# Rose-STL-Lab/spherical-dyffusion

Hardware: AMD Instinct MI355X
Metric: forecast-steps/sec (180x360, 63ch), 25-member ensemble DYffusion sampling, whole job (higher is better)
Workload: dtype f32 tensors; every GEMM-class kernel (1x1 convs, fused MLP, Legendre analysis/synthesis, dhconv) as 3-pass split-f16 MFMA with f32 accumulation; FFT / norms / pointwise in f32 (statistics f64); 1 GPU; 25-member ensemble x horizon-6 DYffusion sampling pass (6 forecaster + 10 interpolator SFNO forwards, dropout stream on, AR feedback), 180x360, 63 state + 2 forcing channels, embed 256, 8 blocks; horizon=6, relayed_members=0, parallelism=members of one initial condition sharded over GPUs, no data-path collective

## Files before the change

### include/sdy_amd.h

```cpp
#ifndef SDY_AMD_H
#define SDY_AMD_H

#include <stddef.h>
#include <stdint.h>

#ifdef __cplusplus
extern "C" {
#endif
#pragma GCC visibility push(default)

#define SDY_OK 0
#define SDY_ERR_ARG (-1)
#define SDY_ERR_UNSUPPORTED (-2)
#define SDY_ERR_ALIGN (-3)
#define SDY_ERR_WORKSPACE (-4)
#define SDY_ERR_NAME (-5)
#define SDY_ERR_SHAPE (-6)
#define SDY_ERR_STATE (-7)

#define SDY_GRID_EQUIANGULAR 0
#define SDY_GRID_LEGENDRE_GAUSS 1

int sdy_version(void);
const char* sdy_error_string(int code);
// ... 13 lines not shown

int sdy_sht_forward(const sdy_sht_plan* plan, const float* x, float* out_c64, int B, int C, float* ws,
                    size_t ws_floats, void* stream);
int sdy_sht_inverse(const sdy_sht_plan* plan, const float* in_c64, float* y, int B, int C, float* ws,
                    size_t ws_floats, void* stream);

int sdy_rfft_lon(const sdy_sht_plan* plan, const float* x, const float* a, const float* d, float* xn_out,
                 float* Xf, int B, int C, void* stream);
int sdy_legendre_fwd(const sdy_sht_plan* plan, const float* Xf, float* Cs, int B, int C, void* stream);
int sdy_legendre_inv(const sdy_sht_plan* plan, const float* Cs, float* Yf, int B, int C, void* stream);
int sdy_irfft_lon(const sdy_sht_plan* plan, const float* Yf, const float* bias, float* y, int B, int C,
                  void* stream);

int sdy_dhconv_pack_weight(const float* w_host, int Ci, int Co, int L, float* w_packed_dev, void* stream);
int sdy_dhconv(const float* Cs_in, const float* w_packed, float* Cs_out, int L, int mtr, int B, int Ci, int Co,
               void* stream);
size_t sdy_dhconv_h3_pack_bytes(int Ci, int Co, int L);
int sdy_dhconv_h3_pack_weight(const float* w_host, int Ci, int Co, int L, void* packed_dev, float* scale);
int sdy_dhconv_h3(const float* Cs_in, const void* packed, float scale, float* Cs_out, int L, int mtr, int B, int Ci,
                  int Co, void* stream);

int sdy_dhconv_frag_supported(int Ci, int Co);
size_t sdy_dhconv_frag_pack_bytes(int L);
int sdy_dhconv_frag_pack(const float* w_host, int L, void* packed_dev, float* scale);
int sdy_dhconv_frag(const float* Cs_in, const void* packed, float scale, float* Cs_out, int L, int mtr, int B,
                    void* stream);

int sdy_instnorm_coeffs(const float* x, int B, int C, int HW, const float* gamma, const float* beta,
                        const float* scale_shift, long ss_stride, float eps, float* a, float* d, void* stream);

typedef struct sdy_conv_args {
  const float* x;  long x_bstride;
  const float* wt; int ldw;
  float* out;      long out_bstride;
  int B, Cin, Cout, HW;
  const float* pa; const float* pd;
  const float* bias;
  const float* add; long add_bstride;
  int add_mode;
  int act;
  float drop_p;
  const float* keep_mask;
  uint64_t seed; uint32_t call; uint32_t stream_id; uint32_t batch_offset;
  int rows_per_call;
  const float* batch_scale;
  int kernel_tag;
  const void* w_h3;
  float w_h3_scale;
  const void* w_frag;
  float w_frag_scale;
  double* stats;
  int out_tiled;
  const unsigned char* x_rows;
} sdy_conv_args;
int sdy_conv1x1(const sdy_conv_args* args, void* stream);

int sdy_conv256_h3_supported(int Cin, int Cout);
size_t sdy_conv256_h3_pack_bytes(void);
size_t sdy_conv256_h3_pack_bytes_cin(int Cin);
int sdy_conv256_h3_pack(const float* w_host, void* packed_dev, float* scale);
int sdy_conv256_h3_pack_cin(const float* w_host, int Cin, void* packed_dev, float* scale);
size_t sdy_h3_pack_bytes(int Cout, int Cin);
int sdy_h3_pack_weight(const float* w_host, int Cout, int Cin, void* packed_dev, float* scale);

typedef struct sdy_mlp_args {
  const float* x;  long x_bstride;
  const float* pa; const float* pd;
  const void* w; float w1_scale; float w2_scale;
  const float* b1; const float* b2;
  float* out;      long out_bstride;
  const float* add; long add_bstride;
  const float* add_a; const float* add_d;
  int B, E, hidden, HW;
  float drop_p;
  uint64_t seed; uint32_t call; uint32_t stream_fc1; uint32_t stream_fc2; uint32_t batch_offset;
  int rows_per_call;
  const float* batch_scale;
  double* stats;
  int x_tiled;
  const float* keep_hidden;
  const float* keep_out;
  const unsigned char* out_rows;
  int add_by_launch_row;
} sdy_mlp_args;
int sdy_instnorm_from_stats(double* stats, int B, int C, int HW, const float* gamma, const float* beta,
                            const float* scale_shift, long ss_bstride, float eps, float* a_out, float* d_out, void* stream);
int sdy_mlp_h3_supported(int E, int hidden);
size_t sdy_mlp_h3_pack_bytes(int E, int hidden);
int sdy_mlp_h3_pack(const float* w1_host, const float* w2_host, int E, int hidden, void* packed_dev, float* scale1,
                    float* scale2);
int sdy_mlp_h3(const sdy_mlp_args* args, void* stream);

typedef struct sdy_pair_args {
  const float* x;  long x_bstride;
  const void* w; float w1_scale; float w2_scale;
  const float* b1;
  float* out;      long out_bstride;
  const float* add; long add_bstride;
  int B, Cin, hidden, Cout, HW;
  double* stats;
} sdy_pair_args;
int sdy_pair_h3_supported(int Cin, int hidden, int Cout);
size_t sdy_pair_h3_pack_bytes(int Cin, int hidden, int Cout);
int sdy_pair_h3_pack(const float* w1_host, const float* w2_host, int Cin, int hidden, int Cout, void* packed_dev,
                     float* scale1, float* scale2);
int sdy_pair_h3(const sdy_pair_args* args, void* stream);

typedef struct sdy_sfno_config {
  int nlat, nlon;
  int in_chans;
  int out_chans;
  int embed_dim;
  int num_layers;
  int mlp_hidden;
  int lmax, mmax;
  int data_grid;
  int with_time_emb;
  int time_dim;
  float dropout_mlp;
  float drop_path_rate;
  int big_skip, pos_embed;
  int gemm_mode;
} sdy_sfno_config;

typedef struct sdy_sfno sdy_sfno;
int sdy_sfno_create(const sdy_sfno_config* cfg, sdy_sfno** out);
void sdy_sfno_destroy(sdy_sfno* net);
int sdy_sfno_set_param(sdy_sfno* net, const char* name, const float* host, size_t numel);
int sdy_sfno_ready(const sdy_sfno* net);
const char* sdy_sfno_missing(const sdy_sfno* net);
size_t sdy_sfno_workspace_floats(const sdy_sfno* net, int B);
int sdy_sfno_max_batch(const sdy_sfno* net);

typedef struct sdy_sfno_fwd_args {
  const float* in[3]; int in_chans[3];
  const float* time;
  float* out;
  int B;
  int enable_dropout;
  uint64_t seed; uint32_t call; uint32_t batch_offset;
  int rows_per_call;
  const float* const* keep_masks;
  const float* drop_path_keep;
  float* ws; size_t ws_floats;
  int reuse_encoder;
  int shared_inputs;
  const float* gen_src;
  int gen_chans;
  int gen_pos;
  const float* gen_coef;
  const float* gen_noise;
} sdy_sfno_fwd_args;
int sdy_sfno_forward(sdy_sfno* net, const sdy_sfno_fwd_args* args, void* stream);

int sdy_sfno_time_embed(sdy_sfno* net, const float* time, int B, float* t_repr, float* ss, void* stream);

int sdy_cold_update(const float* x_s, const float* x_ip_next, const float* x_ip_s, float* out, size_t n,
                    void* stream);
int sdy_concat_channels(const float* const* src, const int* chans, int nsrc, float* out, int B, int HW,
                        void* stream);

#define SDY_MAX_VARS 96
typedef struct sdy_var_table {
  int nvars;
  const float* data[SDY_MAX_VARS];
  float mean[SDY_MAX_VARS];
  float std[SDY_MAX_VARS];
} sdy_var_table;
int sdy_norm_pack(const sdy_var_table* vars, int t, int T1, int B, int HW, float* out, void* stream);

typedef struct sdy_step_finish_args {
  int B, HW, T1, t;
  const float* gen; int n_out;
  const float* prev_in; float* next_in; int n_in;
  int n_entries;
  int out_idx[SDY_MAX_VARS];
  int in_idx[SDY_MAX_VARS];
  float* gen_norm_tl[SDY_MAX_VARS];
  float* gen_tl[SDY_MAX_VARS];
  float mean[SDY_MAX_VARS], std[SDY_MAX_VARS];
  int presc_entry;
  const float* presc_target;
  const float* presc_mask;
  int mask_value, interpolate;
  const float* ar_init;
} sdy_step_finish_args;
int sdy_step_finish(const sdy_step_finish_args* args, void* stream);
int sdy_init_timeline(const sdy_var_table* vars, int T1, int B, int HW, float* const* tl_norm, float* const* tl_denorm,
                      void* stream);
int sdy_lp_rel_terms(const float* gen, const sdy_var_table* targets, int t, int T1, int B, int HW, double* terms,
                     void* stream);

int sdy_ensemble_metrics(const float* pred, const float* truth, const float* weights, int M, long member_stride,
                         int n_planes, int HW, double* out, void* stream);

int sdy_ensemble_series(const float* pred, int M, long member_stride, long sample_stride, const float* truth,
                        long truth_sample_stride, const float* weights, int n_sample, int T, int HW, double* out,
                        void* stream);

int sdy_ensemble_series_grad(const float* pred, int M, long member_stride, long sample_stride, const float* truth,
                             long truth_sample_stride, const float* weights, int n_sample, int T, int nlat, int nlon,
                             double* out, void* stream);

#define SDY_DERIVED_MAX_LEVELS 16
typedef struct {
  const float* q[SDY_DERIVED_MAX_LEVELS];
  const float* ps;
  const float* lhf;
  const float* prate;
  const float* adv;
  long s0, s1;
  int n0, n1, T, HW, K;
  float ak[SDY_DERIVED_MAX_LEVELS + 1], bk[SDY_DERIVED_MAX_LEVELS + 1];
  float* dry;
  float* twp;
  float* resid;
} sdy_derived_args;
int sdy_derived_water(const sdy_derived_args* args, void* stream);

#define SDY_CORRECTOR_DRY_AIR 1
#define SDY_CORRECTOR_ZERO_ADV 2
typedef struct sdy_corrector_var {
  const float* base;
  long stride;
  int channel;
  float mean, std;
} sdy_corrector_var;
typedef struct sdy_corrector_out {
  float* base;
  long stride;
  int channel;
} sdy_corrector_out;
typedef struct sdy_corrector_args {
  int B, HW, K;
  int flags;
  int budget;
// ... 130 lines not shown
```

### spherical-dyffusion_amd/_lib.py

```python
from __future__ import annotations

import ctypes as C
import os

_HERE = os.path.dirname(os.path.abspath(__file__))
LIB_PATH = os.environ.get("SDY_AMD_LIB") or os.path.join(_HERE, "libsdy_amd.so")

SDY_GRID = {"equiangular": 0, "legendre-gauss": 1}


class SdyError(RuntimeError):
    pass


class SdyConvArgs(C.Structure):
    _fields_ = [
        ("x", C.c_void_p), ("x_bstride", C.c_long),
        ("wt", C.c_void_p), ("ldw", C.c_int),
        ("out", C.c_void_p), ("out_bstride", C.c_long),
        ("B", C.c_int), ("Cin", C.c_int), ("Cout", C.c_int), ("HW", C.c_int),
        ("pa", C.c_void_p), ("pd", C.c_void_p),
        ("bias", C.c_void_p),
        ("add", C.c_void_p), ("add_bstride", C.c_long),
        ("add_mode", C.c_int),
        ("act", C.c_int),
        ("drop_p", C.c_float),
        ("keep_mask", C.c_void_p),
        ("seed", C.c_uint64), ("call", C.c_uint32), ("stream_id", C.c_uint32), ("batch_offset", C.c_uint32),
        ("rows_per_call", C.c_int),
        ("batch_scale", C.c_void_p),
        ("kernel_tag", C.c_int),
        ("w_h3", C.c_void_p),
        ("w_h3_scale", C.c_float),
        ("w_frag", C.c_void_p),
        ("w_frag_scale", C.c_float),
        ("stats", C.c_void_p),
        ("out_tiled", C.c_int),
        ("x_rows", C.c_void_p),
    ]


class SdyMlpArgs(C.Structure):
    _fields_ = [
        ("x", C.c_void_p), ("x_bstride", C.c_long),
        ("pa", C.c_void_p), ("pd", C.c_void_p),
        ("w", C.c_void_p), ("w1_scale", C.c_float), ("w2_scale", C.c_float),
        ("b1", C.c_void_p), ("b2", C.c_void_p),
        ("out", C.c_void_p), ("out_bstride", C.c_long),
        ("add", C.c_void_p), ("add_bstride", C.c_long),
        ("add_a", C.c_void_p), ("add_d", C.c_void_p),
        ("B", C.c_int), ("E", C.c_int), ("hidden", C.c_int), ("HW", C.c_int),
        ("drop_p", C.c_float),
        ("seed", C.c_uint64), ("call", C.c_uint32), ("stream_fc1", C.c_uint32), ("stream_fc2", C.c_uint32),
        ("batch_offset", C.c_uint32),
        ("rows_per_call", C.c_int),
        ("batch_scale", C.c_void_p),
        ("stats", C.c_void_p),
        ("x_tiled", C.c_int),
        ("keep_hidden", C.c_void_p), ("keep_out", C.c_void_p),
        ("out_rows", C.c_void_p),
        ("add_by_launch_row", C.c_int),
    ]


class SdyPairArgs(C.Structure):
    _fields_ = [
        ("x", C.c_void_p), ("x_bstride", C.c_long),
        ("w", C.c_void_p), ("w1_scale", C.c_float), ("w2_scale", C.c_float),
        ("b1", C.c_void_p),
        ("out", C.c_void_p), ("out_bstride", C.c_long),
        ("add", C.c_void_p), ("add_bstride", C.c_long),
        ("B", C.c_int), ("Cin", C.c_int), ("hidden", C.c_int), ("Cout", C.c_int), ("HW", C.c_int),
        ("stats", C.c_void_p),
    ]


SDY_MAX_VARS = 96


class SdyVarTable(C.Structure):
    _fields_ = [("nvars", C.c_int), ("data", C.c_void_p * SDY_MAX_VARS), ("mean", C.c_float * SDY_MAX_VARS),
                ("std", C.c_float * SDY_MAX_VARS)]


class SdyStepFinishArgs(C.Structure):
    _fields_ = [
        ("B", C.c_int), ("HW", C.c_int), ("T1", C.c_int), ("t", C.c_int),
        ("gen", C.c_void_p), ("n_out", C.c_int),
        ("prev_in", C.c_void_p), ("next_in", C.c_void_p), ("n_in", C.c_int),
        ("n_entries", C.c_int),
        ("out_idx", C.c_int * SDY_MAX_VARS), ("in_idx", C.c_int * SDY_MAX_VARS),
        ("gen_norm_tl", C.c_void_p * SDY_MAX_VARS), ("gen_tl", C.c_void_p * SDY_MAX_VARS),
        ("mean", C.c_float * SDY_MAX_VARS), ("std", C.c_float * SDY_MAX_VARS),
        ("presc_entry", C.c_int),
        ("presc_target", C.c_void_p), ("presc_mask", C.c_void_p),
        ("mask_value", C.c_int), ("interpolate", C.c_int),
        ("ar_init", C.c_void_p),
    ]


class SdySfnoConfig(C.Structure):
    _fields_ = [
        ("nlat", C.c_int), ("nlon", C.c_int),
        ("in_chans", C.c_int), ("out_chans", C.c_int),
        ("embed_dim", C.c_int), ("num_layers", C.c_int), ("mlp_hidden", C.c_int),
        ("lmax", C.c_int), ("mmax", C.c_int),
        ("data_grid", C.c_int),
        ("with_time_emb", C.c_int), ("time_dim", C.c_int),
        ("dropout_mlp", C.c_float), ("drop_path_rate", C.c_float),
        ("big_skip", C.c_int), ("pos_embed", C.c_int),
        ("gemm_mode", C.c_int),
    ]


class SdySfnoFwdArgs(C.Structure):
    _fields_ = [
        ("in_", C.c_void_p * 3), ("in_chans", C.c_int * 3),
        ("time", C.c_void_p),
        ("out", C.c_void_p),
        ("B", C.c_int),
        ("enable_dropout", C.c_int),
        ("seed", C.c_uint64), ("call", C.c_uint32), ("batch_offset", C.c_uint32),
        ("rows_per_call", C.c_int),
        ("keep_masks", C.POINTER(C.c_void_p)),
        ("drop_path_keep", C.c_void_p),
        ("ws", C.c_void_p), ("ws_floats", C.c_size_t),
        ("reuse_encoder", C.c_int),
        ("shared_inputs", C.c_int),
        ("gen_src", C.c_void_p), ("gen_chans", C.c_int), ("gen_pos", C.c_int),
        ("gen_coef", C.c_void_p), ("gen_noise", C.c_void_p),
    ]


SDY_DERIVED_MAX_LEVELS = 16


class SdyDerivedArgs(C.Structure):
    _fields_ = [
        ("q", C.c_void_p * SDY_DERIVED_MAX_LEVELS), ("ps", C.c_void_p),
        ("lhf", C.c_void_p), ("prate", C.c_void_p), ("adv", C.c_void_p),
        ("s0", C.c_long), ("s1", C.c_long),
        ("n0", C.c_int), ("n1", C.c_int), ("T", C.c_int), ("HW", C.c_int), ("K", C.c_int),
        ("ak", C.c_float * (SDY_DERIVED_MAX_LEVELS + 1)), ("bk", C.c_float * (SDY_DERIVED_MAX_LEVELS + 1)),
        ("dry", C.c_void_p), ("twp", C.c_void_p), ("resid", C.c_void_p),
    ]


SDY_CORRECTOR_DRY_AIR = 1
SDY_CORRECTOR_ZERO_ADV = 2
SDY_CORRECTOR_BUDGET = {None: 0, "precipitation": 1, "evaporation": 2, "advection_and_precipitation": 3,
                        "advection_and_evaporation": 4}


class SdyCorrectorVar(C.Structure):
    _fields_ = [("base", C.c_void_p), ("stride", C.c_long), ("channel", C.c_int), ("mean", C.c_float), ("std", C.c_float)]


class SdyCorrectorOut(C.Structure):
    _fields_ = [("base", C.c_void_p), ("stride", C.c_long), ("channel", C.c_int)]


class SdyCorrectorArgs(C.Structure):
    _fields_ = [
        ("B", C.c_int), ("HW", C.c_int), ("K", C.c_int), ("flags", C.c_int), ("budget", C.c_int),
        ("ak", C.c_float * (SDY_DERIVED_MAX_LEVELS + 1)), ("bk", C.c_float * (SDY_DERIVED_MAX_LEVELS + 1)),
        ("area", C.c_void_p),
        ("gen_q", SdyCorrectorVar * SDY_DERIVED_MAX_LEVELS), ("in_q", SdyCorrectorVar * SDY_DERIVED_MAX_LEVELS),
        ("gen_ps", SdyCorrectorVar), ("in_ps", SdyCorrectorVar), ("gen_lhf", SdyCorrectorVar),
        ("gen_prate", SdyCorrectorVar), ("gen_adv", SdyCorrectorVar),
        ("out_ps", SdyCorrectorOut), ("out_lhf", SdyCorrectorOut), ("out_prate", SdyCorrectorOut),
        ("out_adv", SdyCorrectorOut),
        ("ws", C.c_void_p), ("ws_bytes", C.c_size_t),
    ]


class SdyDryAirVar(C.Structure):
    _fields_ = [("base", C.c_void_p), ("stride_b", C.c_long), ("stride_t", C.c_long), ("channel", C.c_int),
                ("mean", C.c_float), ("std", C.c_float)]


class SdyDryAirArgs(C.Structure):
    _fields_ = [
        ("B", C.c_int), ("T", C.c_int), ("HW", C.c_int), ("K", C.c_int), ("accumulate", C.c_int),
        ("ak", C.c_float * (SDY_DERIVED_MAX_LEVELS + 1)), ("bk", C.c_float * (SDY_DERIVED_MAX_LEVELS + 1)),
        ("area", C.c_void_p),
        ("q", SdyDryAirVar * SDY_DERIVED_MAX_LEVELS), ("ps", SdyDryAirVar),
        ("gm", C.c_void_p), ("absdiff", C.c_void_p), ("mean_absdiff", C.c_void_p),
        ("ws", C.c_void_p), ("ws_bytes", C.c_size_t),
    ]


SDY_HIST_MAX_BINS = 2048
SDY_HIST_FLAG_RANGE = 1


class SdyHistArgs(C.Structure):
    _fields_ = [
        ("nvars", C.c_int), ("data", C.c_void_p * SDY_MAX_VARS),
        ("s0", C.c_long * SDY_MAX_VARS), ("s1", C.c_long * SDY_MAX_VARS),
        ("n0", C.c_int), ("n1", C.c_int), ("T", C.c_int), ("HW", C.c_int),
        ("t_start", C.c_int), ("n_times", C.c_int), ("n_bins", C.c_int),
        ("state", C.c_void_p), ("counts", C.c_void_p),
    ]


class SdyCoarsenArgs(C.Structure):
    _fields_ = [
        ("nvars", C.c_int), ("data", C.c_void_p * SDY_MAX_VARS),
        ("s0", C.c_long * SDY_MAX_VARS), ("s1", C.c_long * SDY_MAX_VARS),
        ("out", C.c_void_p * SDY_MAX_VARS),
        ("n0", C.c_int), ("n1", C.c_int), ("T", C.c_int), ("HW", C.c_int),
# ... 1 lines not shown
    ]


class SdyVideoArgs(C.Structure):
    _fields_ = [
        ("nvars", C.c_int), ("gen", C.c_void_p * SDY_MAX_VARS), ("target", C.c_void_p * SDY_MAX_VARS),
        ("gs0", C.c_long), ("gs1", C.c_long), ("ts1", C.c_long),
        ("n0", C.c_int), ("n1", C.c_int), ("T", C.c_int), ("HW", C.c_int),
        ("t_start", C.c_int), ("n_timesteps", C.c_int),
        ("gen_mean", C.c_void_p), ("target_mean", C.c_void_p), ("gen_sq", C.c_void_p), ("target_sq", C.c_void_p),
        ("err_var", C.c_void_p), ("err_min", C.c_void_p), ("err_max", C.c_void_p),
    ]


class SdyZonalArgs(C.Structure):
    _fields_ = [
        ("nvars", C.c_int), ("gen", C.c_void_p * SDY_MAX_VARS), ("target", C.c_void_p * SDY_MAX_VARS),
        ("gs0", C.c_long), ("gs1", C.c_long), ("ts1", C.c_long),
        ("n0", C.c_int), ("n1", C.c_int), ("T", C.c_int), ("H", C.c_int), ("W", C.c_int),
        ("t_start", C.c_int), ("n_timesteps", C.c_int),
        ("gen_acc", C.c_void_p), ("target_acc", C.c_void_p),
    ]


SIGNATURES = {
    "sdy_version": (C.c_int, []),
    "sdy_error_string": (C.c_char_p, [C.c_int]),
    "sdy_abi_check": (C.c_int, [C.POINTER(C.c_size_t), C.c_int]),
    "sdy_sht_tables_host": (C.c_int, [C.c_int, C.c_int, C.c_int, C.c_int, C.c_int, C.c_void_p, C.c_void_p, C.c_void_p]),
    "sdy_sht_plan_create": (C.c_int, [C.c_int, C.c_int, C.c_int, C.c_int, C.c_int, C.POINTER(C.c_void_p)]),
    "sdy_sht_plan_create_ex": (C.c_int, [C.c_int, C.c_int, C.c_int, C.c_int, C.c_int, C.c_int, C.POINTER(C.c_void_p)]),
    "sdy_sht_plan_destroy": (None, [C.c_void_p]),
    "sdy_sht_plan_dims": (C.c_int, [C.c_void_p, C.POINTER(C.c_int * 6)]),
    "sdy_sht_plan_kernels": (C.c_int, [C.c_void_p, C.POINTER(C.c_int * 2)]),
    "sdy_sht_workspace_floats": (C.c_size_t, [C.c_void_p, C.c_int, C.c_int]),
    "sdy_sht_forward": (C.c_int, [C.c_void_p, C.c_void_p, C.c_void_p, C.c_int, C.c_int, C.c_void_p, C.c_size_t, C.c_void_p]),
    "sdy_sht_inverse": (C.c_int, [C.c_void_p, C.c_void_p, C.c_void_p, C.c_int, C.c_int, C.c_void_p, C.c_size_t, C.c_void_p]),
    "sdy_rfft_lon": (C.c_int, [C.c_void_p, C.c_void_p, C.c_void_p, C.c_void_p, C.c_void_p, C.c_void_p, C.c_int, C.c_int, C.c_void_p]),
    "sdy_legendre_fwd": (C.c_int, [C.c_void_p, C.c_void_p, C.c_void_p, C.c_int, C.c_int, C.c_void_p]),
    "sdy_legendre_inv": (C.c_int, [C.c_void_p, C.c_void_p, C.c_void_p, C.c_int, C.c_int, C.c_void_p]),
    "sdy_irfft_lon": (C.c_int, [C.c_void_p, C.c_void_p, C.c_void_p, C.c_void_p, C.c_int, C.c_int, C.c_void_p]),
    "sdy_dhconv_pack_weight": (C.c_int, [C.c_void_p, C.c_int, C.c_int, C.c_int, C.c_void_p, C.c_void_p]),
    "sdy_dhconv": (C.c_int, [C.c_void_p, C.c_void_p, C.c_void_p, C.c_int, C.c_int, C.c_int, C.c_int, C.c_int, C.c_void_p]),
    "sdy_dhconv_h3_pack_bytes": (C.c_size_t, [C.c_int, C.c_int, C.c_int]),
    "sdy_dhconv_h3_pack_weight": (C.c_int, [C.c_void_p, C.c_int, C.c_int, C.c_int, C.c_void_p, C.POINTER(C.c_float)]),
    "sdy_dhconv_h3": (C.c_int, [C.c_void_p, C.c_void_p, C.c_float, C.c_void_p, C.c_int, C.c_int, C.c_int, C.c_int, C.c_int,
                                C.c_void_p]),
    "sdy_dhconv_frag_supported": (C.c_int, [C.c_int, C.c_int]),
    "sdy_dhconv_frag_pack_bytes": (C.c_size_t, [C.c_int]),
    "sdy_dhconv_frag_pack": (C.c_int, [C.c_void_p, C.c_int, C.c_void_p, C.POINTER(C.c_float)]),
    "sdy_dhconv_frag": (C.c_int, [C.c_void_p, C.c_void_p, C.c_float, C.c_void_p, C.c_int, C.c_int, C.c_int, C.c_void_p]),
    "sdy_instnorm_coeffs": (C.c_int, [C.c_void_p, C.c_int, C.c_int, C.c_int, C.c_void_p, C.c_void_p, C.c_void_p, C.c_long,
                                      C.c_float, C.c_void_p, C.c_void_p, C.c_void_p]),
    "sdy_conv1x1": (C.c_int, [C.POINTER(SdyConvArgs), C.c_void_p]),
    "sdy_ensemble_metrics": (C.c_int, [C.c_void_p, C.c_void_p, C.c_void_p, C.c_int, C.c_long, C.c_int, C.c_int, C.c_void_p,
                                       C.c_void_p]),
    "sdy_instnorm_from_stats": (C.c_int, [C.c_void_p, C.c_int, C.c_int, C.c_int, C.c_void_p, C.c_void_p, C.c_void_p,
                                          C.c_long, C.c_float, C.c_void_p, C.c_void_p, C.c_void_p]),
    "sdy_mlp_h3_supported": (C.c_int, [C.c_int, C.c_int]),
    "sdy_mlp_h3_pack_bytes": (C.c_size_t, [C.c_int, C.c_int]),
    "sdy_mlp_h3_pack": (C.c_int, [C.c_void_p, C.c_void_p, C.c_int, C.c_int, C.c_void_p, C.POINTER(C.c_float),
                                  C.POINTER(C.c_float)]),
    "sdy_mlp_h3": (C.c_int, [C.POINTER(SdyMlpArgs), C.c_void_p]),
    "sdy_pair_h3_supported": (C.c_int, [C.c_int, C.c_int, C.c_int]),
    "sdy_pair_h3_pack_bytes": (C.c_size_t, [C.c_int, C.c_int, C.c_int]),
    "sdy_pair_h3_pack": (C.c_int, [C.c_void_p, C.c_void_p, C.c_int, C.c_int, C.c_int, C.c_void_p, C.POINTER(C.c_float),
                                   C.POINTER(C.c_float)]),
    "sdy_pair_h3": (C.c_int, [C.POINTER(SdyPairArgs), C.c_void_p]),
    "sdy_conv256_h3_supported": (C.c_int, [C.c_int, C.c_int]),
    "sdy_conv256_h3_pack_bytes": (C.c_size_t, []),
    "sdy_conv256_h3_pack_bytes_cin": (C.c_size_t, [C.c_int]),
    "sdy_conv256_h3_pack": (C.c_int, [C.c_void_p, C.c_void_p, C.POINTER(C.c_float)]),
    "sdy_conv256_h3_pack_cin": (C.c_int, [C.c_void_p, C.c_int, C.c_void_p, C.POINTER(C.c_float)]),
    "sdy_h3_pack_bytes": (C.c_size_t, [C.c_int, C.c_int]),
    "sdy_h3_pack_weight": (C.c_int, [C.c_void_p, C.c_int, C.c_int, C.c_void_p, C.POINTER(C.c_float)]),
    "sdy_sfno_create": (C.c_int, [C.POINTER(SdySfnoConfig), C.POINTER(C.c_void_p)]),
    "sdy_sfno_destroy": (None, [C.c_void_p]),
    "sdy_sfno_set_param": (C.c_int, [C.c_void_p, C.c_char_p, C.c_void_p, C.c_size_t]),
    "sdy_sfno_ready": (C.c_int, [C.c_void_p]),
    "sdy_sfno_missing": (C.c_char_p, [C.c_void_p]),
    "sdy_sfno_workspace_floats": (C.c_size_t, [C.c_void_p, C.c_int]),
    "sdy_sfno_max_batch": (C.c_int, [C.c_void_p]),
    "sdy_sfno_forward": (C.c_int, [C.c_void_p, C.POINTER(SdySfnoFwdArgs), C.c_void_p]),
    "sdy_sfno_time_embed": (C.c_int, [C.c_void_p, C.c_void_p, C.c_int, C.c_void_p, C.c_void_p, C.c_void_p]),
    "sdy_norm_pack": (C.c_int, [C.POINTER(SdyVarTable), C.c_int, C.c_int, C.c_int, C.c_int, C.c_void_p, C.c_void_p]),
    "sdy_step_finish": (C.c_int, [C.POINTER(SdyStepFinishArgs), C.c_void_p]),
    "sdy_init_timeline": (C.c_int, [C.POINTER(SdyVarTable), C.c_int, C.c_int, C.c_int, C.POINTER(C.c_void_p),
                                    C.POINTER(C.c_void_p), C.c_void_p]),
    "sdy_lp_rel_terms": (C.c_int, [C.c_void_p, C.POINTER(SdyVarTable), C.c_int, C.c_int, C.c_int, C.c_int, C.c_void_p,
                                   C.c_void_p]),
    "sdy_cold_update": (C.c_int, [C.c_void_p, C.c_void_p, C.c_void_p, C.c_void_p, C.c_size_t, C.c_void_p]),
    "sdy_concat_channels": (C.c_int, [C.POINTER(C.c_void_p), C.POINTER(C.c_int), C.c_int, C.c_void_p, C.c_int, C.c_int,
                                      C.c_void_p]),
    "sdy_time_mean_accumulate": (C.c_int, [C.c_void_p, C.c_int, C.c_long, C.c_int, C.c_long, C.c_int, C.c_int, C.c_int,
                                          C.c_float, C.c_void_p, C.c_void_p]),
    "sdy_status_flags": (C.c_int, [C.POINTER(C.c_uint), C.c_int, C.c_void_p]),
    "sdy_status_flags_async": (C.c_int, [C.c_void_p, C.c_int, C.c_void_p]),
    "sdy_range_headroom_enable": (C.c_int, [C.c_int]),
    "sdy_range_headroom": (C.c_int, [C.POINTER(C.c_float), C.c_int, C.c_void_p]),
    "sdy_dropout_stream_rounds": (C.c_int, []),
    "sdy_dropout_stream_words": (C.c_int, [C.c_uint32, C.c_uint32, C.c_uint32, C.c_uint32, C.c_uint32, C.c_uint32,
                                           C.POINTER(C.c_uint32)]),
    "sdy_cond_noise_fill": (C.c_int, [C.c_uint64, C.c_uint32, C.c_uint32, C.c_int, C.c_int, C.c_int, C.c_int, C.c_void_p,
                                      C.c_void_p]),
    "sdy_ensemble_series": (C.c_int, [C.c_void_p, C.c_int, C.c_long, C.c_long, C.c_void_p, C.c_long, C.c_void_p, C.c_int,
                                     C.c_int, C.c_int, C.c_void_p, C.c_void_p]),
    "sdy_ensemble_series_grad": (C.c_int, [C.c_void_p, C.c_int, C.c_long, C.c_long, C.c_void_p, C.c_long, C.c_void_p,
                                          C.c_int, C.c_int, C.c_int, C.c_int, C.c_void_p, C.c_void_p]),
    "sdy_derived_water": (C.c_int, [C.POINTER(SdyDerivedArgs), C.c_void_p]),
    "sdy_corrector": (C.c_int, [C.POINTER(SdyCorrectorArgs), C.c_void_p]),
    "sdy_corrector_host": (C.c_int, [C.POINTER(SdyCorrectorArgs)]),
    "sdy_corrector_workspace_bytes": (C.c_size_t, [C.c_int, C.c_int]),
    "sdy_corrector_args_bytes": (C.c_size_t, []),
    "sdy_dry_air_series": (C.c_int, [C.POINTER(SdyDryAirArgs), C.c_void_p]),
    "sdy_dry_air_series_host": (C.c_int, [C.POINTER(SdyDryAirArgs)]),
    "sdy_dry_air_workspace_bytes": (C.c_size_t, [C.c_int, C.c_int, C.c_int]),
    "sdy_dry_air_args_bytes": (C.c_size_t, []),
    "sdy_hist_add": (C.c_int, [C.POINTER(SdyHistArgs), C.c_void_p]),
    "sdy_hist_args_bytes": (C.c_size_t, []),
    "sdy_hist_state_bytes": (C.c_size_t, [C.c_int]),
    "sdy_hist_state_unpack_host": (C.c_int, [C.c_void_p, C.c_int, C.POINTER(C.c_float), C.POINTER(C.c_float),
                                             C.POINTER(C.c_int), C.POINTER(C.c_uint), C.POINTER(C.c_ulonglong)]),
    "sdy_hist_plan_host": (C.c_int, [C.c_float, C.c_float, C.c_int, C.c_float, C.c_float, C.c_int, C.POINTER(C.c_float),
                                     C.POINTER(C.c_float), C.POINTER(C.c_int), C.POINTER(C.c_int), C.POINTER(C.c_uint)]),
    "sdy_hist_edges_host": (C.c_int, [C.c_float, C.c_float, C.c_int, C.c_void_p]),
    "sdy_hist_bins_host": (C.c_int, [C.c_void_p, C.c_long, C.c_float, C.c_float, C.c_int, C.c_void_p]),
    "sdy_time_coarsen": (C.c_int, [C.POINTER(SdyCoarsenArgs), C.c_void_p]),
    "sdy_time_coarsen_host": (C.c_int, [C.POINTER(SdyCoarsenArgs)]),
    "sdy_coarsen_args_bytes": (C.c_size_t, []),
    "sdy_video_accumulate": (C.c_int, [C.POINTER(SdyVideoArgs), C.c_void_p]),
    "sdy_video_accumulate_host": (C.c_int, [C.POINTER(SdyVideoArgs)]),
    "sdy_video_args_bytes": (C.c_size_t, []),
    "sdy_zonal_accumulate": (C.c_int, [C.POINTER(SdyZonalArgs), C.c_void_p]),
    "sdy_zonal_accumulate_host": (C.c_int, [C.POINTER(SdyZonalArgs)]),
    "sdy_zonal_args_bytes": (C.c_size_t, []),
    "sdy_profile_enable": (C.c_int, [C.c_int]),
    "sdy_profile_stage_count": (C.c_int, []),
    "sdy_profile_stage_name": (C.c_char_p, [C.c_int]),
    "sdy_profile_read": (C.c_int, [C.POINTER(C.c_double), C.POINTER(C.c_long), C.c_int]),
    "sdy_profile_read_rows": (C.c_int, [C.POINTER(C.c_double), C.POINTER(C.c_long), C.POINTER(C.c_long), C.c_int]),
    "sdy_relay_pool_create": (C.c_int, [C.c_size_t, C.c_int, C.POINTER(C.c_void_p), C.POINTER(C.c_ubyte)]),
    "sdy_relay_pool_destroy": (C.c_int, [C.c_void_p]),
    "sdy_ipc_open": (C.c_int, [C.POINTER(C.c_ubyte), C.POINTER(C.c_void_p)]),
    "sdy_ipc_close": (C.c_int, [C.c_void_p]),
    "sdy_copy_nocu": (C.c_int, [C.c_void_p, C.c_void_p, C.c_size_t, C.c_void_p]),
}


def _load():
    import torch

    if not os.path.exists(LIB_PATH):
        raise ImportError(
            f"{LIB_PATH} not found: the HIP library is required (no CPU/PyTorch fallback exists). "
            "Build it with `make -C spherical-dyffusion_amd/csrc` or `__graft_entry__.build()`."
        )
    lib = C.CDLL(LIB_PATH)
    for name, (res, args) in SIGNATURES.items():
        fn = getattr(lib, name)
        fn.restype = res
        fn.argtypes = args
    structs = (SdyConvArgs, SdyMlpArgs, SdyPairArgs, SdySfnoConfig, SdySfnoFwdArgs, SdyVarTable, SdyStepFinishArgs)
    sizes = (C.c_size_t * len(structs))(*[C.sizeof(t) for t in structs])
    if lib.sdy_abi_check(sizes, len(structs)) != 0:
        raise ImportError(f"{LIB_PATH}: argument structures of the bindings and of the library differ in size "
                          f"({[C.sizeof(t) for t in structs]}): rebuild the library (make -C spherical-dyffusion_amd/csrc)")
# ... 45 lines not shown
```

### spherical-dyffusion_amd/csrc/capi.hip

```cpp
#include <cmath>
#include <cstdio>
#include <cstdlib>
#include <cstring>
#include <mutex>
#include <string>
#include <vector>

#include "common.h"
#include "fft.h"
#include "pointwise.h"

static inline int round_up(int v, int m) { return (v + m - 1) / m * m; }
static inline size_t round_up_sz(size_t v, size_t m) { return (v + m - 1) / m * m; }

template <class F>
static float h3_pack_host(std::vector<_Float16>& buf, int nb, int rows, int K, int rows_pad, int Kpad, F value) {
  float mx = 0.f;
  for (int b = 0; b < nb; ++b)
    for (int r = 0; r < rows; ++r)
      for (int k = 0; k < K; ++k) mx = std::fmax(mx, std::fabs(value(b, r, k)));
  const float s = sdy_h3_scale(mx);
  const size_t plane = (size_t)nb * rows_pad * Kpad;
  buf.assign(2 * plane, (_Float16)0.0f);
  for (int b = 0; b < nb; ++b)
// ... 492 lines not shown
  return sdy_cond_noise_launch(seed, call, batch_offset, rows_per_call, B, C, HW, out, (hipStream_t)stream);
}

namespace {

struct DevBuf {
  float* p = nullptr;
  size_t n = 0;
  bool set = false;
  void* h3 = nullptr;
  float h3_scale = 1.0f;
  void* frag = nullptr;
  float frag_scale = 1.0f;
};

struct BlockW {
  DevBuf n0w, n0b, n1w, n1b;
  DevBuf tw, tb;
  DevBuf fw;
  DevBuf fb;
  DevBuf skw, skb;
  DevBuf w1, b1, w2, b2;
  std::vector<float> w1_host, w2_host;
  void* mlp = nullptr;
  float mlp_s1 = 1.0f, mlp_s2 = 1.0f;
  std::vector<float> fw_host, skw_host, fb_host, skb_host;
  DevBuf fbs;
};

}

static int spec_ilv(const sdy_sfno_config& c) { return (c.gemm_mode == 1 && c.embed_dim % 16 == 0) ? 1 : 0; }

static bool skip_foldable(const sdy_sfno_config& c, int i) {
  const bool first = i == 0, last = i == c.num_layers - 1;
  return c.gemm_mode == 1 && c.data_grid != SDY_GRID_LEGENDRE_GAUSS && first != last;
}

enum DhKind { DH_FOLDED, DH_FRAG, DH_GEMM_H3, DH_GEMM_F32 };
static DhKind dhconv_kind(const sdy_sfno_config& c, int i) {
  if (c.gemm_mode != 1) return DH_GEMM_F32;
  if (!sdy_dhconv_frag_supported(c.embed_dim, c.embed_dim) || sw().no_dh_frag) return DH_GEMM_H3;
  return skip_foldable(c, i) && !sw().no_skip_fold ? DH_FOLDED : DH_FRAG;
}

namespace {
struct XfSide {
  const sdy_sht_plan* plan;
  bool polar;
  bool tiled;
  int ilv;
  const int* mcut;
};

struct BlockPath {
  XfSide in, out;
  bool scale_residual;
  bool fused_mlp;
  bool lazy_norm;
  bool cs_tiled;
  DhKind dh;
  enum Skip { SKIP_CONV, SKIP_GELU, SKIP_IN_FFT } skip;
  bool stats1;
  bool z_tiled;
  bool drop_skip;
};
}

struct sdy_sfno {
  sdy_sfno_config cfg;
  int HW, catC, decC, ldo;
  sdy_sht_plan* plan_data = nullptr;
  sdy_sht_plan* plan_lg = nullptr;
  DevBuf pos, e0w, e0b, e2w, d0w, d0b, d2w;
  struct Pair { std::vector<float> w1_host, w2_host; void* w = nullptr; float s1 = 1.0f, s2 = 1.0f; } enc, dec;
  DevBuf t1w, t1b, t3w, t3b, freq, wbt, bb;
  std::vector<BlockW> blk;
  std::vector<BlockPath> path;
  SdyTimeMlp tm;
  std::string missing;
  const float* enc_ws = nullptr;
  int enc_B = 0;
  bool enc_has_stats = false;
};

static int dev_alloc(DevBuf& b, size_t n) {
  if (b.p && b.n == n) return SDY_OK;
  if (b.p) (void)hipFree(b.p);
  b.p = nullptr;
  SDY_HIP_TRY(hipMalloc((void**)&b.p, n * sizeof(float)));
  b.n = n;
  return SDY_OK;
}
static int dev_upload(DevBuf& b, const float* host, size_t n) {
  SDY_TRY(dev_alloc(b, n));
  SDY_HIP_TRY(hipMemcpy(b.p, host, n * sizeof(float), hipMemcpyHostToDevice));
  b.set = true;
  return SDY_OK;
}
static int dev_upload_T(DevBuf& b, const float* host, int out, int in, int ld) {
  std::vector<float> t((size_t)in * ld, 0.0f);
  for (int o = 0; o < out; ++o)
    for (int i = 0; i < in; ++i) t[(size_t)i * ld + o] = host[(size_t)o * in + i];
  return dev_upload(b, t.data(), t.size());
}
static void dev_free(DevBuf& b) {
  if (b.p) (void)hipFree(b.p);
  if (b.h3) (void)hipFree(b.h3);
  if (b.frag) (void)hipFree(b.frag);
  b.p = nullptr;
  b.h3 = nullptr;
  b.frag = nullptr;
  b.set = false;
}
static int dev_upload_conv(DevBuf& b, const float* host, int out, int in, int ld, bool want_h3) {
  SDY_TRY(dev_upload_T(b, host, out, in, ld));
  if (want_h3) {
    if (b.h3) (void)hipFree(b.h3);
    b.h3 = nullptr;
    SDY_HIP_TRY(hipMalloc(&b.h3, sdy_h3_pack_bytes(out, in)));
    SDY_TRY(sdy_h3_pack_weight(host, out, in, b.h3, &b.h3_scale));
    if (sdy_conv256_h3_supported(in, out)) {
      if (b.frag) (void)hipFree(b.frag);
      b.frag = nullptr;
      SDY_HIP_TRY(hipMalloc(&b.frag, sdy_conv256_h3_pack_bytes_cin(in)));
      SDY_TRY(sdy_conv256_h3_pack_cin(host, in, b.frag, &b.frag_scale));
    }
  }
  return SDY_OK;
}

extern "C" int sdy_sfno_create(const sdy_sfno_config* c, sdy_sfno** out) {
  if (!c || !out) return SDY_ERR_ARG;
  if (c->nlat < 2 || c->nlon < 4 || c->in_chans < 1 || c->out_chans < 1 || c->embed_dim < 4 || c->num_layers < 1 ||
      c->num_layers > 32 || c->mlp_hidden < 4)
    return SDY_ERR_ARG;
  if ((c->embed_dim & 3) || (c->mlp_hidden & 3) || ((c->nlat * c->nlon) & 3)) return SDY_ERR_ALIGN;
  if (c->with_time_emb && (c->time_dim < 4 || (c->embed_dim & 1))) return SDY_ERR_ARG;
  if (c->dropout_mlp < 0.f || c->dropout_mlp >= 1.f || c->drop_path_rate < 0.f || c->drop_path_rate >= 1.f)
    return SDY_ERR_ARG;
  sdy_sfno* n = new sdy_sfno();
  n->cfg = *c;
  n->HW = c->nlat * c->nlon;
  n->catC = c->embed_dim + c->in_chans;
  n->decC = c->embed_dim + (c->big_skip ? c->in_chans : 0);
  n->ldo = round_up(c->out_chans, 4);
  n->blk.resize(c->num_layers);
  if (c->gemm_mode != 0 && c->gemm_mode != 1) { delete n; return SDY_ERR_ARG; }
  int r = sdy_sht_plan_create_ex(c->nlat, c->nlon, c->lmax, c->mmax, c->data_grid, c->gemm_mode, &n->plan_data);
  if (r != SDY_OK) { delete n; return r; }
  if (c->data_grid == SDY_GRID_LEGENDRE_GAUSS) {
    n->plan_lg = n->plan_data;
  } else {
    r = sdy_sht_plan_create_ex(c->nlat, c->nlon, c->lmax, c->mmax, SDY_GRID_LEGENDRE_GAUSS, c->gemm_mode, &n->plan_lg);
    if (r != SDY_OK) { sdy_sfno_destroy(n); return r; }
  }
  std::memset(&n->tm, 0, sizeof(n->tm));
  n->tm.num_layers = c->num_layers;
  for (int i = 0; i < c->num_layers; ++i) {
    const float rate = c->num_layers > 1 ? c->drop_path_rate * (float)i / (float)(c->num_layers - 1) : 0.0f;
    n->tm.dp_rate[i] = rate;
    n->tm.dp_thr[i] = sdy_drop_threshold(rate);
  }
  if (c->with_time_emb) {
    const int E = c->embed_dim, T = c->time_dim, L = c->num_layers, half = E / 2;
    std::vector<float> f(half);
    const float e = (float)(-std::log(10000.0) / (half - 1));
    for (int i = 0; i < half; ++i) f[i] = expf((float)i * e);
    r = dev_upload(n->freq, f.data(), half);
    if (r == SDY_OK) r = dev_alloc(n->wbt, (size_t)L * T * 2 * E);
    if (r == SDY_OK) r = dev_alloc(n->bb, (size_t)L * 2 * E);
    if (r != SDY_OK) { sdy_sfno_destroy(n); return r; }
  }
  *out = n;
  return SDY_OK;
}

extern "C" void sdy_sfno_destroy(sdy_sfno* n) {
  if (!n) return;
  if (n->plan_lg && n->plan_lg != n->plan_data) sdy_sht_plan_destroy(n->plan_lg);
  if (n->plan_data) sdy_sht_plan_destroy(n->plan_data);
  DevBuf* top[] = {&n->pos, &n->e0w, &n->e0b, &n->e2w, &n->d0w, &n->d0b, &n->d2w, &n->t1w, &n->t1b,
                   &n->t3w, &n->t3b, &n->freq, &n->wbt, &n->bb};
  for (DevBuf* b : top) dev_free(*b);
  for (BlockW& w : n->blk) {
    DevBuf* bs[] = {&w.n0w, &w.n0b, &w.n1w, &w.n1b, &w.fw, &w.fb, &w.skw, &w.skb, &w.w1, &w.b1, &w.w2, &w.b2, &w.fbs};
    for (DevBuf* b : bs) dev_free(*b);
    if (w.mlp) (void)hipFree(w.mlp);
  }
  if (n->enc.w) (void)hipFree(n->enc.w);
  if (n->dec.w) (void)hipFree(n->dec.w);
  delete n;
}

#define EXPECT_NUMEL(n_expected)                      \
  do {                                                \
    if (numel != (size_t)(n_expected)) return SDY_ERR_SHAPE; \
  } while (0)

extern "C" int sdy_sfno_set_param(sdy_sfno* n, const char* name_c, const float* host, size_t numel) {
  if (!n || !name_c || !host) return SDY_ERR_ARG;
  const sdy_sfno_config& c = n->cfg;
  const int E = c.embed_dim, T = c.time_dim, L = c.num_layers, H = c.mlp_hidden, Cin = c.in_chans;
  const std::string name(name_c);
  const bool h3 = c.gemm_mode == 1;
  n->enc_ws = nullptr;
  n->path.clear();
  if (name.find("trans") != std::string::npos && (name.find(".weights") != std::string::npos ||
                                                   name.find(".pct") != std::string::npos))
    return SDY_OK;
  if (name == "@time_freq") { EXPECT_NUMEL(E / 2); return dev_upload(n->freq, host, numel); }
  if (name == "@drop_path_rates") {
    EXPECT_NUMEL(L);
    for (int i = 0; i < L; ++i) {
      if (host[i] < 0.f || host[i] >= 1.f) return SDY_ERR_ARG;
      n->tm.dp_rate[i] = host[i];
      n->tm.dp_thr[i] = sdy_drop_threshold(host[i]);
    }
    return SDY_OK;
  }
  if (name == "pos_embed") { EXPECT_NUMEL((size_t)E * n->HW); return dev_upload(n->pos, host, numel); }
  auto pack_pair = [&](sdy_sfno::Pair& pr, int cin, int cout) -> int {
    if (!h3 || !sdy_pair_h3_supported(cin, E, cout) || pr.w1_host.empty() || pr.w2_host.empty()) return SDY_OK;
    if (!pr.w) SDY_HIP_TRY(hipMalloc(&pr.w, sdy_pair_h3_pack_bytes(cin, E, cout)));
    return sdy_pair_h3_pack(pr.w1_host.data(), pr.w2_host.data(), cin, E, cout, pr.w, &pr.s1, &pr.s2);
  };
  if (name == "encoder.0.weight") {
    EXPECT_NUMEL((size_t)E * Cin);
    n->enc.w1_host.assign(host, host + numel);
    SDY_TRY(pack_pair(n->enc, Cin, E));
    return dev_upload_conv(n->e0w, host, E, Cin, E, h3);
  }
  if (name == "encoder.0.bias") { EXPECT_NUMEL(E); return dev_upload(n->e0b, host, numel); }
  if (name == "encoder.2.weight") {
    EXPECT_NUMEL((size_t)E * E);
    n->enc.w2_host.assign(host, host + numel);
    SDY_TRY(pack_pair(n->enc, Cin, E));
    return dev_upload_conv(n->e2w, host, E, E, E, h3);
  }
  if (name == "decoder.0.weight") {
    EXPECT_NUMEL((size_t)E * n->decC);
    n->dec.w1_host.assign(host, host + numel);
    SDY_TRY(pack_pair(n->dec, n->decC, c.out_chans));
    return dev_upload_conv(n->d0w, host, E, n->decC, E, h3);
  }
  if (name == "decoder.0.bias") { EXPECT_NUMEL(E); return dev_upload(n->d0b, host, numel); }
  if (name == "decoder.2.weight") {
    EXPECT_NUMEL((size_t)c.out_chans * E);
    n->dec.w2_host.assign(host, host + numel);
    SDY_TRY(pack_pair(n->dec, n->decC, c.out_chans));
    return dev_upload_conv(n->d2w, host, c.out_chans, E, n->ldo, h3);
  }
  if (c.with_time_emb) {
    if (name == "time_emb_mlp.1.weight") { EXPECT_NUMEL((size_t)T * E); return dev_upload_T(n->t1w, host, T, E, T); }
    if (name == "time_emb_mlp.1.bias") { EXPECT_NUMEL(T); return dev_upload(n->t1b, host, numel); }
    if (name == "time_emb_mlp.3.weight") { EXPECT_NUMEL((size_t)T * T); return dev_upload_T(n->t3w, host, T, T, T); }
    if (name == "time_emb_mlp.3.bias") { EXPECT_NUMEL(T); return dev_upload(n->t3b, host, numel); }
  }
  if (name.rfind("blocks.", 0) == 0) {
    const size_t dot = name.find('.', 7);
    if (dot == std::string::npos) return SDY_ERR_NAME;
    const int i = std::atoi(name.substr(7, dot - 7).c_str());
    if (i < 0 || i >= L) return SDY_ERR_NAME;
    const std::string rest = name.substr(dot + 1);
    BlockW& w = n->blk[i];
    if (rest == "norm0.weight") { EXPECT_NUMEL(E); return dev_upload(w.n0w, host, numel); }
    if (rest == "norm0.bias") { EXPECT_NUMEL(E); return dev_upload(w.n0b, host, numel); }
    if (rest == "norm1.weight") { EXPECT_NUMEL(E); return dev_upload(w.n1w, host, numel); }
    if (rest == "norm1.bias") { EXPECT_NUMEL(E); return dev_upload(w.n1b, host, numel); }
    if (c.with_time_emb && rest == "time_mlp.1.weight") {
      EXPECT_NUMEL((size_t)2 * E * T);
      std::vector<float> t((size_t)T * 2 * E);
      for (int o = 0; o < 2 * E; ++o)
        for (int k = 0; k < T; ++k) t[(size_t)k * 2 * E + o] = host[(size_t)o * T + k];
      SDY_HIP_TRY(hipMemcpy(n->wbt.p + (size_t)i * T * 2 * E, t.data(), t.size() * sizeof(float), hipMemcpyHostToDevice));
      w.tw.set = true;
      return SDY_OK;
    }
    if (c.with_time_emb && rest == "time_mlp.1.bias") {
      EXPECT_NUMEL((size_t)2 * E);
      SDY_HIP_TRY(hipMemcpy(n->bb.p + (size_t)i * 2 * E, host, numel * sizeof(float), hipMemcpyHostToDevice));
      w.tb.set = true;
      return SDY_OK;
    }
    auto pack_folded = [&]() -> int {
      if (w.fw_host.empty() || w.skw_host.empty()) return SDY_OK;
      std::vector<float> sum(w.fw_host);
      for (int ii = 0; ii < E; ++ii)
        for (int oo = 0; oo < E; ++oo) {
// ... 71 lines not shown
      return SDY_OK;
    }
    if (rest == "mlp.fwd.2.bias" || rest == "mlp.fwd.3.bias") { EXPECT_NUMEL(E); return dev_upload(w.b2, host, numel); }
  }
  return SDY_ERR_NAME;
}

static BlockPath resolve_path(const sdy_sfno* n, int i) {
  const sdy_sfno_config& c = n->cfg;
  const BlockW& w = n->blk[i];
  const int E = c.embed_dim, ilv = spec_ilv(c);
  auto side = [&](const sdy_sht_plan* p) {
    const bool polar = plan_polar_ok(p, E), tiled = plan_tiled_ok(p, E, ilv);
    return XfSide{p, polar, tiled, tiled ? 2 : ilv, polar ? p->d_mcut : nullptr};
  };
  BlockPath b;
  b.in = side(i == 0 ? n->plan_data : n->plan_lg);
  b.out = side(i == c.num_layers - 1 ? n->plan_data : n->plan_lg);
  b.scale_residual = b.in.plan != b.out.plan;
  b.fused_mlp = w.mlp && !sw().no_fused_mlp;
  b.lazy_norm = b.fused_mlp && !b.scale_residual;
  b.dh = dhconv_kind(c, i);
  const bool dh_frag = b.dh == DH_FOLDED || b.dh == DH_FRAG;
  b.cs_tiled = b.in.tiled && b.out.tiled && dh_frag && b.in.plan->lmax == b.out.plan->lmax && b.in.plan->mtr == b.out.plan->mtr;
  b.stats1 = c.gemm_mode == 1 && w.skw.frag && sdy_conv256_h3_supported(E, E);
  b.z_tiled = b.stats1 && b.fused_mlp;
  b.skip = b.dh != DH_FOLDED ? BlockPath::SKIP_CONV : (b.out.tiled && b.z_tiled) ? BlockPath::SKIP_IN_FFT : BlockPath::SKIP_GELU;
  b.drop_skip = b.fused_mlp && b.z_tiled && b.cs_tiled && !sw().no_drop_skip;
  return b;
}

extern "C" int sdy_sfno_ready(const sdy_sfno* n_c) {
  sdy_sfno* n = const_cast<sdy_sfno*>(n_c);
  if (!n) return SDY_ERR_ARG;
  if (!n->path.empty()) return SDY_OK;
  const sdy_sfno_config& c = n->cfg;
  n->missing.clear();
  auto need = [&](const DevBuf& b, const std::string& nm) {
    if (!b.set && n->missing.empty()) n->missing = nm;
  };
  if (c.pos_embed) need(n->pos, "pos_embed");
  need(n->e0w, "encoder.0.weight"); need(n->e0b, "encoder.0.bias"); need(n->e2w, "encoder.2.weight");
  need(n->d0w, "decoder.0.weight"); need(n->d0b, "decoder.0.bias"); need(n->d2w, "decoder.2.weight");
  if (c.with_time_emb) {
    need(n->t1w, "time_emb_mlp.1.weight"); need(n->t1b, "time_emb_mlp.1.bias");
    need(n->t3w, "time_emb_mlp.3.weight"); need(n->t3b, "time_emb_mlp.3.bias");
  }
  for (int i = 0; i < c.num_layers; ++i) {
    const BlockW& w = n->blk[i];
    const std::string p = "blocks." + std::to_string(i) + ".";
    need(w.n0w, p + "norm0.weight"); need(w.n0b, p + "norm0.bias");
    need(w.n1w, p + "norm1.weight"); need(w.n1b, p + "norm1.bias");
    if (c.with_time_emb) { need(w.tw, p + "time_mlp.1.weight"); need(w.tb, p + "time_mlp.1.bias"); }
    need(w.fw, p + "filter.filter.weight"); need(w.fb, p + "filter.filter.bias");
    need(w.skw, p + "inner_skip.weight"); need(w.skb, p + "inner_skip.bias");
    need(w.w1, p + "mlp.fwd.0.weight"); need(w.b1, p + "mlp.fwd.0.bias");
    need(w.w2, p + "mlp.fwd.{2|3}.weight"); need(w.b2, p + "mlp.fwd.{2|3}.bias");
  }
  if (!n->missing.empty()) return SDY_ERR_STATE;
  if (c.with_time_emb) {
    n->tm.E = c.embed_dim; n->tm.T = c.time_dim;
    n->tm.freq = n->freq.p; n->tm.w1t = n->t1w.p; n->tm.b1 = n->t1b.p; n->tm.w2t = n->t3w.p; n->tm.b2 = n->t3b.p;
    n->tm.wbt = n->wbt.p; n->tm.bb = n->bb.p;
  } else {
    n->tm.E = 0;
  }
  std::vector<BlockPath> path;
  for (int i = 0; i < c.num_layers; ++i) {
    const BlockW& w = n->blk[i];
    const BlockPath b = resolve_path(n, i);
    const void* packed = b.dh == DH_GEMM_F32 ? (const void*)w.fw.p : b.dh == DH_GEMM_H3 ? w.fw.h3 : w.fw.frag;
    if (!packed) return SDY_ERR_STATE;
    if (b.dh == DH_FOLDED && !(b.scale_residual && w.fbs.set)) return SDY_ERR_STATE;
    path.push_back(b);
  }
  n->path = std::move(path);
  return SDY_OK;
}

extern "C" const char* sdy_sfno_missing(const sdy_sfno* n) { return n ? n->missing.c_str() : ""; }

namespace {
struct WsLayout {
  size_t cat, xa, xb, xe, xn, y, zt, hid, xf, cs, cs2, ca, cd, ca1, cd1, st0, st1, ste, ss, dp, trep, sp, total;
};
WsLayout ws_layout(const sdy_sfno* n, int B) {
  const sdy_sfno_config& c = n->cfg;
  const size_t HW = n->HW, E = c.embed_dim;
  WsLayout w;
  size_t off = 0;
  auto take = [&](size_t floats) { size_t o = off; off += round_up_sz(floats, 64); return o; };
  w.cat = take((size_t)B * n->catC * HW);
  const size_t img = (size_t)B * E * HW;
  w.xa = take(img); w.xb = take(img);
  w.xe = take(img);
  w.xn = take(img); w.y = take(img);
  w.zt = take((size_t)B * ((HW + 63) / 64) * E * 64);
  w.hid = take((size_t)B * c.mlp_hidden * HW);
  w.xf = take(xf_floats(n->plan_data, B, (int)E));
  w.cs = take(cs_floats(n->plan_data, B, (int)E)); w.cs2 = take(cs_floats(n->plan_data, B, (int)E));
  w.ca = take((size_t)B * E); w.cd = take((size_t)B * E); w.ca1 = take((size_t)B * E); w.cd1 = take((size_t)B * E);
  w.st1 = take((size_t)B * E * 4);
  w.st0 = take((size_t)B * E * 4);
  w.ste = take((size_t)B * E * 4);
  w.ss = take((size_t)B * c.num_layers * 2 * E);
  w.dp = take((size_t)B * c.num_layers);
  w.trep = take((size_t)2 * B * (c.with_time_emb ? c.time_dim : 1));
  w.sp = take((size_t)B * E * c.nlat * 4);
  w.total = off;
  return w;
}
}

extern "C" size_t sdy_sfno_workspace_floats(const sdy_sfno* n, int B) {
  if (!n || B <= 0) return 0;
  return ws_layout(n, B).total;
}

extern "C" int sdy_sfno_max_batch(const sdy_sfno* n) {
  if (!n) return 0;
  const sdy_sfno_config& c = n->cfg;
  const int mtr = c.mmax < c.lmax ? c.mmax : c.lmax;
  bool all_tiled = sdy_sfno_ready(n) == SDY_OK;
  for (const BlockPath& p : n->path) all_tiled = all_tiled && p.cs_tiled;
  long b;
  if (all_tiled) {
    b = ((1L << 32) - 1) / ((long)mtr * 8 * c.lmax * 64);
  } else {
    const long per_row = 192L * mtr * 2 * c.embed_dim * 4 + 2L * c.embed_dim * 4;
    b = ((1L << 32) - 1) / per_row;
  }
  if (b > SDY_MAP_MAX) b = SDY_MAP_MAX;
  return b < 1 ? 1 : (int)b;
}

extern "C" int sdy_sfno_time_embed(sdy_sfno* n, const float* time, int B, float* t_repr, float* ss, void* stream) {
  if (!n || !time || B <= 0) return SDY_ERR_ARG;
  SDY_TRY(sdy_sfno_ready(n));
  if (!n->cfg.with_time_emb) return SDY_ERR_UNSUPPORTED;
  if (!ss) return SDY_ERR_ARG;
  float* scratch = nullptr;
  SDY_HIP_TRY(hipMallocAsync(reinterpret_cast<void**>(&scratch), (size_t)2 * B * n->cfg.time_dim * sizeof(float), (hipStream_t)stream));
  const int rc = sdy_time_mlp_launch(n->tm, time, B, t_repr, ss, nullptr, nullptr, 0, 0, 0, 0, 0, (hipStream_t)stream, scratch);
  SDY_HIP_TRY(hipFreeAsync(scratch, (hipStream_t)stream));
  return rc;
}

namespace {
enum SdyStage {
  ST_CONCAT, ST_TIME_MLP, ST_ENC0, ST_ENC2, ST_NORM_COEFFS, ST_FFT_FWD, ST_LEG_FWD, ST_LEG_INV, ST_FFT_INV, ST_DHCONV,
  ST_SKIP_CONV, ST_MLP_FUSED, ST_MLP_FUSED_DROP, ST_FC1, ST_FC2, ST_DEC0, ST_DEC2, ST_ENC_PAIR, ST_DEC_PAIR, ST_DROP_COPY,
  ST_SKIP_GELU, ST_COUNT
};
const char* const kStageNames[ST_COUNT] = {
  "concat", "time_mlp", "encoder.0 conv", "encoder.2 conv", "instnorm coefficients", "rfft (lon)", "legendre analysis",
  "legendre synthesis", "irfft (lon)", "dhconv", "inner-skip conv", "mlp fused", "mlp fused (dropout)", "mlp fc1", "mlp fc2",
  "decoder.0 conv", "decoder.2 conv", "encoder (fused pair)", "decoder (fused pair)", "drop-path copy",
  "inner skip folded (gelu)"};
struct SdyProfiler {
  bool on = false;
  struct Rec { int stage; int rows; hipEvent_t e0, e1; bool closed; };
  std::vector<Rec> recs;
  std::vector<hipEvent_t> pool;
  std::mutex mu;
  int get_event(hipEvent_t* e) {
    if (!pool.empty()) { *e = pool.back(); pool.pop_back(); return SDY_OK; }
    SDY_HIP_TRY(hipEventCreate(e));
    return SDY_OK;
  }
  int begin(int stage, int rows, hipStream_t s, int* idx) {
    std::lock_guard<std::mutex> g(mu);
    Rec r{stage, rows, nullptr, nullptr, false};
    SDY_TRY(get_event(&r.e0));
    int rc = get_event(&r.e1);
    if (rc == SDY_OK) {
      hipError_t e = hipEventRecord(r.e0, s);
      if (e != hipSuccess) rc = (int)e;
    }
    if (rc != SDY_OK) {
      pool.push_back(r.e0);
      if (r.e1) pool.push_back(r.e1);
      return rc;
    }
    recs.push_back(r);
    *idx = (int)recs.size() - 1;
    return SDY_OK;
  }
  int end(int idx, hipStream_t s) {
    std::lock_guard<std::mutex> g(mu);
    if (idx < 0 || idx >= (int)recs.size()) return SDY_ERR_STATE;
    SDY_HIP_TRY(hipEventRecord(recs[idx].e1, s));
    recs[idx].closed = true;
    return SDY_OK;
  }
} g_prof;
}

#define SDY_STAGE_N(stage, rows, call)                                          \
  do {                                                                          \
    int prof_idx_ = -1;                                                         \
    if (g_prof.on) SDY_TRY(g_prof.begin((stage), (rows), stream, &prof_idx_));  \
    SDY_TRY(call);                                                              \
    if (prof_idx_ >= 0) (void)g_prof.end(prof_idx_, stream);                    \
  } while (0)
#define SDY_STAGE(stage, call) SDY_STAGE_N(stage, B, call)

extern "C" int sdy_profile_enable(int on) {
  g_prof.on = on != 0;
  return SDY_OK;
}
extern "C" int sdy_profile_stage_count(void) { return ST_COUNT; }
extern "C" const char* sdy_profile_stage_name(int stage) {
  return (stage >= 0 && stage < ST_COUNT) ? kStageNames[stage] : "";
}
extern "C" int sdy_profile_read(double* total_ms, long* launches, int n) {
  return sdy_profile_read_rows(total_ms, launches, nullptr, n);
}
extern "C" int sdy_profile_read_rows(double* total_ms, long* launches, long* rows, int n) {
  if (!total_ms || !launches || n < ST_COUNT) return SDY_ERR_ARG;
  for (int i = 0; i < n; ++i) { total_ms[i] = 0.0; launches[i] = 0; if (rows) rows[i] = 0; }
  std::lock_guard<std::mutex> g(g_prof.mu);
  int rc = SDY_OK;
  for (auto& r : g_prof.recs) {
    if (r.closed) {
      float ms = 0.f;
      hipError_t e = hipEventSynchronize(r.e1);
      if (e == hipSuccess) e = hipEventElapsedTime(&ms, r.e0, r.e1);
      if (e != hipSuccess) rc = (int)e;
      else { total_ms[r.stage] += ms; launches[r.stage] += 1; if (rows) rows[r.stage] += r.rows; }
    }
    g_prof.pool.push_back(r.e0);
    g_prof.pool.push_back(r.e1);
  }
  g_prof.recs.clear();
  return rc;
}

namespace {
struct SfnoCall {
  sdy_sfno* n;
  const sdy_sfno_config& c;
  const sdy_sfno_fwd_args* a;
  hipStream_t stream;
  const int B, E = c.embed_dim, HW = n->HW, ilv = spec_ilv(c);
  const int rpc = a->rows_per_call > 0 ? a->rows_per_call : B;
  const bool drop = a->enable_dropout != 0, reuse = a->reuse_encoder != 0, shared = a->shared_inputs != 0, gen = a->gen_src;
  const bool enc_once = shared && n->enc.w && n->path[0].scale_residual && n->path[0].in.tiled;
  const int Be = enc_once ? rpc : B;
  const float pm = (drop && c.dropout_mlp > 0.f) ? c.dropout_mlp : 0.f;
  const WsLayout w = ws_layout(n, B);
  float* const ws = a->ws;
  const long xbs = (long)E * HW, cat_bs = (long)n->catC * HW;
  const long zt_bs = (long)((HW + 63) / 64) * E * 64;
  float *cat = ws + w.cat, *xa = ws + w.xa, *xb = ws + w.xb, *xe = ws + w.xe, *xn = ws + w.xn, *y = ws + w.y, *zt = ws + w.zt;
  float *hid = ws + w.hid, *Xf = ws + w.xf, *Cs = ws + w.cs, *Cs2 = ws + w.cs2, *ss = ws + w.ss, *dp = ws + w.dp;
  float *ca = ws + w.ca, *cd = ws + w.cd, *ca1 = ws + w.ca1, *cd1 = ws + w.cd1, *trep = ws + w.trep;
  float* cat_in = cat + (size_t)(n->catC - c.in_chans) * HW;
  double *st0 = reinterpret_cast<double*>(ws + w.st0), *st1 = reinterpret_cast<double*>(ws + w.st1);
  double *ste = reinterpret_cast<double*>(ws + w.ste), *sp = reinterpret_cast<double*>(ws + w.sp);
  const float* srcs[4];
  int chans[4], ns = 0;
  float *cur = xe, *nxt = xa;
  double* cur_stats = nullptr;

  struct Blk {
    int i;
    const BlockPath& P;
    const BlockW& w;
    float* dst; long dst_bs;
    float* z; long z_bs;
    double* st_out;
    unsigned char perm[SDY_MAP_MAX];
    int Bp, nD, Bf;
    const unsigned char* rows;
  };

  SfnoCall(sdy_sfno* n_, const sdy_sfno_fwd_args* a_, hipStream_t s) : n(n_), c(n_->cfg), a(a_), stream(s), B(a_->B) {}

  int check() {
    if (c.with_time_emb && !a->time) return SDY_ERR_ARG;
    if (a->ws_floats < w.total) return SDY_ERR_WORKSPACE;
    if (reuse && (n->enc_ws != ws || n->enc_B != B)) return SDY_ERR_STATE;
    int ctot = 0;
    for (int i = 0; i < 3; ++i)
      if (a->in[i] && a->in_chans[i] > 0) { srcs[ns] = a->in[i]; chans[ns] = a->in_chans[i]; ctot += a->in_chans[i]; ++ns; }
    if (gen) {
      if (a->gen_chans <= 0 || !a->gen_coef || a->gen_pos < 0 || a->gen_pos > ns) return SDY_ERR_ARG;
      if (reuse || shared) return SDY_ERR_ARG;
      for (int i = ns; i > a->gen_pos; --i) { srcs[i] = srcs[i - 1]; chans[i] = chans[i - 1]; }
      srcs[a->gen_pos] = a->gen_src; chans[a->gen_pos] = a->gen_chans; ctot += a->gen_chans; ++ns;
    }
    if (ns == 0 || ctot != c.in_chans) return SDY_ERR_SHAPE;
    if (a->rows_per_call < 0 || (a->rows_per_call > 0 && B % a->rows_per_call)) return SDY_ERR_ARG;
    if (shared && (reuse || rpc >= B)) return SDY_ERR_ARG;
    return SDY_OK;
  }

  int inputs() {
    if (!reuse) n->enc_ws = nullptr;
    SDY_HIP_TRY(hipMemsetAsync(st1, 0, (size_t)B * E * 2 * sizeof(double), stream));
    SDY_HIP_TRY(hipMemsetAsync(st0, 0, (size_t)B * E * 2 * sizeof(double), stream));
    if (gen) {
      SdyConcatGen g;
      g.gen = a->gen_pos; g.coef = a->gen_coef; g.noise = a->gen_noise;
      g.seed = a->seed; g.call = a->call; g.batch_offset = a->batch_offset; g.rows_per_call = rpc;
      SDY_STAGE(ST_CONCAT, sdy_concat_gen_launch(srcs, chans, ns, g, cat_in, cat_bs, B, HW, stream));
    } else if (!reuse) {
      SDY_STAGE(ST_CONCAT, sdy_concat_launch(srcs, chans, ns, cat_in, cat_bs, B, HW, stream, shared ? rpc : 0));
    }
    return SDY_OK;
  }

  int time_mlp() {
    SDY_STAGE(ST_TIME_MLP, sdy_time_mlp_launch(n->tm, a->time, B, trep, ss, dp, a->drop_path_keep, drop ? 1 : 0, a->seed, a->call,
                                               a->batch_offset, rpc, stream, trep + (size_t)B * (c.with_time_emb ? c.time_dim : 1)));
    return SDY_OK;
  }

  sdy_conv_args conv_args(const DevBuf& wb, int rows) const {
    sdy_conv_args cv;
    std::memset(&cv, 0, sizeof(cv));
    cv.B = rows; cv.HW = HW; cv.seed = a->seed; cv.call = a->call; cv.batch_offset = a->batch_offset; cv.rows_per_call = rpc;
    cv.wt = wb.p;
    if (c.gemm_mode == 1) { cv.w_h3 = wb.h3; cv.w_h3_scale = wb.h3_scale; cv.w_frag = wb.frag; cv.w_frag_scale = wb.frag_scale; }
    return cv;
  }

  int encoder() {
    bool have_ste = false;
    if (reuse) {
      have_ste = n->enc_has_stats;
    } else if (n->enc.w) {
      sdy_pair_args pa{};
      pa.x = cat_in; pa.x_bstride = cat_bs; pa.w = n->enc.w; pa.w1_scale = n->enc.s1; pa.w2_scale = n->enc.s2;
      pa.b1 = n->e0b.p; pa.out = xe; pa.out_bstride = xbs;
      if (c.pos_embed) { pa.add = n->pos.p; pa.add_bstride = 0; }
      pa.B = Be; pa.Cin = c.in_chans; pa.hidden = E; pa.Cout = E; pa.HW = HW;
      SDY_HIP_TRY(hipMemsetAsync(ste, 0, (size_t)Be * E * 2 * sizeof(double), stream));
      pa.stats = ste; have_ste = true;
      SDY_STAGE_N(ST_ENC_PAIR, Be, sdy_pair_h3(&pa, stream));
    } else {
      sdy_conv_args cv = conv_args(n->e0w, B);
      cv.x = cat_in; cv.x_bstride = cat_bs; cv.ldw = E; cv.out = xa; cv.out_bstride = xbs;
      cv.Cin = c.in_chans; cv.Cout = E; cv.bias = n->e0b.p; cv.act = 1;
      SDY_STAGE(ST_ENC0, sdy_conv1x1(&cv, stream));
      cv = conv_args(n->e2w, B);
      cv.x = xa; cv.x_bstride = xbs; cv.ldw = E; cv.out = xe; cv.out_bstride = xbs; cv.Cin = E; cv.Cout = E;
      if (c.pos_embed) { cv.add = n->pos.p; cv.add_bstride = 0; cv.add_mode = 2; }
      if (cv.w_frag && sdy_conv256_h3_supported(E, E)) {
        SDY_HIP_TRY(hipMemsetAsync(ste, 0, (size_t)B * E * 2 * sizeof(double), stream));
        cv.stats = ste; have_ste = true;
      }
      SDY_STAGE(ST_ENC2, sdy_conv1x1(&cv, stream));
    }
    n->enc_ws = enc_once ? nullptr : ws; n->enc_B = B; n->enc_has_stats = have_ste;
    if (have_ste) {
      for (int b0 = 0; b0 < B; b0 += Be)
        SDY_HIP_TRY(hipMemcpyAsync(st0 + (size_t)b0 * E * 2, ste, (size_t)Be * E * 2 * sizeof(double), hipMemcpyDeviceToDevice,
                                   stream));
      cur_stats = st0;
    }
    return SDY_OK;
  }

  int block(int i) {
    const bool last = i == c.num_layers - 1;
    Blk k{i, n->path[i], n->blk[i], last ? cat : nxt, last ? cat_bs : xbs};
    k.z = k.P.z_tiled ? zt : y;
    k.z_bs = k.P.z_tiled ? zt_bs : xbs;
    k.st_out = (k.P.fused_mlp && !last) ? st0 : nullptr;
    SDY_TRY(norm0(k));
    drop_rows(k);
    SDY_TRY(spectral(k));
    if (k.Bp > 0) {
      SDY_TRY(inner_skip(k));
      SDY_TRY(mlp(k));
    }
    if (k.nD > 0) SDY_TRY(drop_copy(k));
    cur_stats = k.st_out;
    cur = k.dst;
    nxt = (k.dst == xa) ? xb : xa;
    return SDY_OK;
  }

  int norm0(const Blk& k) {
    const float* ssk = c.with_time_emb ? ss + (size_t)k.i * 2 * E : nullptr;
    const long ss_bs = (long)c.num_layers * 2 * E;
    if (cur_stats)
      SDY_STAGE(ST_NORM_COEFFS, sdy_instnorm_from_stats(cur_stats, B, E, HW, k.w.n0w.p, k.w.n0b.p, ssk, ss_bs, 1e-6f, ca, cd, stream));
    else
      SDY_STAGE(ST_NORM_COEFFS, sdy_instnorm_coeffs_launch(cur, B, E, HW, k.w.n0w.p, k.w.n0b.p, ssk, ss_bs, 1e-6f, ca, cd, stream));
    return SDY_OK;
  }

  void drop_rows(Blk& k) const {
    k.Bp = B;
    k.nD = 0;
    if (drop && !a->drop_path_keep && B <= SDY_MAP_MAX && n->tm.dp_rate[k.i] > 0.f && k.P.drop_skip) {
      unsigned char drp[SDY_MAP_MAX];
      k.Bp = 0;
      for (int b = 0; b < B; ++b) {
        const int bq = b / rpc;
        const philox4 wd = philox4x32((uint32_t)(b - bq * rpc) + a->batch_offset, 0xFFFFFFFFu, 0x1000u + (uint32_t)k.i,
                                      a->call + (uint32_t)bq, (uint32_t)(a->seed & 0xFFFFFFFFu), (uint32_t)(a->seed >> 32));
        if (wd.x >= n->tm.dp_thr[k.i]) k.perm[k.Bp++] = (unsigned char)b;
        else drp[k.nD++] = (unsigned char)b;
      }
      for (int j = 0; j < k.nD; ++j) k.perm[k.Bp + j] = drp[j];
    }
    k.rows = k.nD > 0 ? k.perm : nullptr;
    k.Bf = k.P.scale_residual ? B : k.Bp;
  }

  int spectral(const Blk& k) {
    const BlockPath& P = k.P;
    const sdy_sht_plan *pin = P.in.plan, *pout = P.out.plan;
    if (k.Bf > 0) {
      float* xn_out = (P.scale_residual || P.lazy_norm) ? nullptr : xn;
      SDY_STAGE_N(ST_FFT_FWD, k.Bf, sdy_fft_launch_fwd(pin->fft, cur, ca, cd, xn_out, Xf, k.Bf, E, pin->nlat, pin->mtr, P.in.ilv,
                                                       P.in.mcut, stream, k.rows, (k.i == 0 && enc_once) ? Be : 0));
      SDY_STAGE_N(ST_LEG_FWD, k.Bf, legendre_fwd_impl(pin, Xf, Cs, k.Bf, E, P.in.polar, stream, P.in.tiled, P.cs_tiled));
      if (P.scale_residual) {
        SDY_STAGE(ST_LEG_INV, legendre_inv_impl(pout, Cs, Xf, B, E, P.out.polar, stream, P.out.tiled, P.cs_tiled));
        SDY_STAGE(ST_FFT_INV, sdy_fft_launch_inv(pout->fft, Xf, nullptr, xn, B, E, pout->nlat, pout->mtr, P.out.ilv, P.out.mcut,
                                                 stream));
      }
    }
    if (k.Bp == 0) return SDY_OK;
    if (P.dh == DH_FOLDED || P.dh == DH_FRAG)
      SDY_STAGE_N(ST_DHCONV, k.Bp, sdy_dh_h3_launch(Cs, k.w.fw.frag, k.w.fw.frag_scale, Cs2, c.lmax, pin->mtr, k.Bp, ilv, stream,
                                                    P.cs_tiled ? 1 : 0, k.Bf));
    else if (P.dh == DH_GEMM_H3)
      SDY_STAGE(ST_DHCONV, sdy_dhconv_h3(Cs, k.w.fw.h3, k.w.fw.h3_scale, Cs2, c.lmax, pin->mtr, B, E, E, stream));
    else
      SDY_STAGE(ST_DHCONV, sdy_dhconv(Cs, k.w.fw.p, Cs2, c.lmax, pin->mtr, B, E, E, stream));
    SDY_STAGE_N(ST_LEG_INV, k.Bp, legendre_inv_impl(pout, Cs2, Xf, k.Bp, E, P.out.polar, stream, P.out.tiled, P.cs_tiled));
    const float* bias = P.dh == DH_FOLDED ? k.w.fbs.p : k.w.fb.p;
    if (P.skip == BlockPath::SKIP_IN_FFT)
      SDY_STAGE_N(ST_FFT_INV, k.Bp, sdy_fft360_launch_inv(pout->fft, Xf, bias, nullptr, k.Bp, E, pout->nlat, pout->mtr, P.out.ilv,
                                                          P.out.mcut, stream, zt, zt_bs, sp));
    else
      SDY_STAGE_N(ST_FFT_INV, k.Bp, sdy_fft_launch_inv(pout->fft, Xf, bias, y, k.Bp, E, pout->nlat, pout->mtr, P.out.ilv,
                                                       P.out.mcut, stream));
    return SDY_OK;
  }

  int inner_skip(const Blk& k) {
    const BlockPath& P = k.P;
    const BlockW& bw = k.w;
    if (P.skip == BlockPath::SKIP_IN_FFT) {
      SDY_STAGE_N(ST_NORM_COEFFS, k.Bp, sdy_instnorm_from_partials_launch(sp, P.out.plan->nlat, k.Bp, E, HW, bw.n1w.p, bw.n1b.p,
                                                                          1e-6f, ca1, cd1, stream));
      return SDY_OK;
    }
    if (P.skip == BlockPath::SKIP_GELU) {
      SDY_STAGE_N(ST_SKIP_GELU, k.Bp, sdy_gelu_stats_launch(y, xbs, k.z, k.z_bs, P.z_tiled ? 1 : 0, st1, k.Bp, E, HW, stream));
    } else {
      sdy_conv_args cv = conv_args(bw.skw, k.Bp);
      cv.x_rows = P.lazy_norm ? k.rows : nullptr;
      cv.x = P.lazy_norm ? cur : xn; cv.x_bstride = xbs;
      if (P.lazy_norm) { cv.pa = ca; cv.pd = cd; }
      cv.ldw = E; cv.out = k.z; cv.out_bstride = k.z_bs; cv.out_tiled = P.z_tiled ? 1 : 0;
      cv.Cin = E; cv.Cout = E; cv.bias = bw.skb.p; cv.add = y; cv.add_bstride = xbs; cv.add_mode = 1; cv.act = 1; cv.kernel_tag = 3;
      if (P.stats1) cv.stats = st1;
      SDY_STAGE_N(ST_SKIP_CONV, k.Bp, sdy_conv1x1(&cv, stream));
    }
    if (P.skip == BlockPath::SKIP_GELU || P.stats1)
      SDY_STAGE_N(ST_NORM_COEFFS, k.Bp, sdy_instnorm_from_stats(st1, k.Bp, E, HW, bw.n1w.p, bw.n1b.p, nullptr, 0, 1e-6f, ca1, cd1,
                                                                stream));
    else
      SDY_STAGE(ST_NORM_COEFFS, sdy_instnorm_coeffs_launch(y, B, E, HW, bw.n1w.p, bw.n1b.p, nullptr, 0, 1e-6f, ca1, cd1, stream));
    return SDY_OK;
  }

  int mlp(const Blk& k) {
    const BlockW& bw = k.w;
    const int i = k.i, Hd = c.mlp_hidden;
    const float* dps = (drop && n->tm.dp_rate[i] > 0.f) ? dp + (size_t)i * B : nullptr;
    const float* keep1 = (pm > 0.f && a->keep_masks) ? a->keep_masks[2 * i] : nullptr;
    const float* keep2 = (pm > 0.f && a->keep_masks) ? a->keep_masks[2 * i + 1] : nullptr;
    if (k.P.fused_mlp) {
      sdy_mlp_args ma;
      std::memset(&ma, 0, sizeof(ma));
      ma.x = k.z; ma.x_bstride = k.z_bs; ma.x_tiled = k.P.z_tiled ? 1 : 0; ma.pa = ca1; ma.pd = cd1;
      ma.w = bw.mlp; ma.w1_scale = bw.mlp_s1; ma.w2_scale = bw.mlp_s2; ma.b1 = bw.b1.p; ma.b2 = bw.b2.p;
      ma.out = k.dst; ma.out_bstride = k.dst_bs;
      if (k.P.lazy_norm) { ma.add = cur; ma.add_bstride = xbs; ma.add_a = ca; ma.add_d = cd; }
      else { ma.add = xn; ma.add_bstride = xbs; ma.add_by_launch_row = k.rows ? 1 : 0; }
      ma.B = k.Bp; ma.out_rows = k.rows; ma.E = E; ma.hidden = Hd; ma.HW = HW;
      ma.drop_p = pm; ma.seed = a->seed; ma.call = a->call; ma.stream_fc1 = 2u * i; ma.stream_fc2 = 2u * i + 1u;
      ma.batch_offset = a->batch_offset; ma.rows_per_call = rpc;
      ma.batch_scale = dps; ma.keep_hidden = keep1; ma.keep_out = keep2; ma.stats = k.st_out;
      SDY_STAGE_N(pm > 0.f ? ST_MLP_FUSED_DROP : ST_MLP_FUSED, k.Bp, sdy_mlp_h3(&ma, stream));
      return SDY_OK;
    }
    sdy_conv_args cv = conv_args(bw.w1, B);
    cv.x = y; cv.x_bstride = xbs; cv.ldw = Hd; cv.out = hid; cv.out_bstride = (long)Hd * HW;
    cv.Cin = E; cv.Cout = Hd; cv.pa = ca1; cv.pd = cd1; cv.bias = bw.b1.p; cv.act = 1; cv.kernel_tag = 1;
    cv.drop_p = pm; cv.stream_id = 2u * i; cv.keep_mask = keep1;
    SDY_STAGE(ST_FC1, sdy_conv1x1(&cv, stream));
    cv = conv_args(bw.w2, B);
    cv.x = hid; cv.x_bstride = (long)Hd * HW; cv.ldw = E; cv.out = k.dst; cv.out_bstride = k.dst_bs;
    cv.Cin = Hd; cv.Cout = E; cv.bias = bw.b2.p; cv.kernel_tag = 2;
    cv.drop_p = pm; cv.stream_id = 2u * i + 1u; cv.keep_mask = keep2; cv.batch_scale = dps;
    cv.add = xn; cv.add_bstride = xbs; cv.add_mode = 2;
    SDY_STAGE(ST_FC2, sdy_conv1x1(&cv, stream));
    return SDY_OK;
  }

  int drop_copy(const Blk& k) {
    if (k.P.lazy_norm)
      SDY_STAGE_N(ST_DROP_COPY, k.nD, sdy_affine_copy_stats_launch(cur, xbs, ca, cd, k.dst, k.dst_bs, k.st_out, E, HW,
                                                                   k.perm + k.Bp, k.nD, stream));
    else
      SDY_STAGE_N(ST_DROP_COPY, k.nD, sdy_affine_copy_stats_launch(xn, xbs, nullptr, nullptr, k.dst, k.dst_bs, k.st_out, E, HW,
                                                                   k.perm + k.Bp, k.nD, stream, k.Bp));
    return SDY_OK;
  }

  int decoder() {
    if (n->dec.w) {
      sdy_pair_args pa{};
      pa.x = cat; pa.x_bstride = cat_bs; pa.w = n->dec.w; pa.w1_scale = n->dec.s1; pa.w2_scale = n->dec.s2;
      pa.b1 = n->d0b.p; pa.out = a->out; pa.out_bstride = (long)c.out_chans * HW;
      pa.B = B; pa.Cin = n->decC; pa.hidden = E; pa.Cout = c.out_chans; pa.HW = HW;
      SDY_STAGE(ST_DEC_PAIR, sdy_pair_h3(&pa, stream));
      return SDY_OK;
    }
    sdy_conv_args cv = conv_args(n->d0w, B);
    cv.x = cat; cv.x_bstride = cat_bs; cv.ldw = E;
    cv.out = xa; cv.out_bstride = xbs; cv.Cin = n->decC; cv.Cout = E; cv.bias = n->d0b.p; cv.act = 1;
    SDY_STAGE(ST_DEC0, sdy_conv1x1(&cv, stream));
    cv = conv_args(n->d2w, B);
    cv.x = xa; cv.x_bstride = xbs; cv.ldw = n->ldo; cv.out = a->out; cv.out_bstride = (long)c.out_chans * HW;
    cv.Cin = E; cv.Cout = c.out_chans;
    SDY_STAGE(ST_DEC2, sdy_conv1x1(&cv, stream));
    return SDY_OK;
  }
};
}

extern "C" int sdy_sfno_forward(sdy_sfno* n, const sdy_sfno_fwd_args* a, void* stream) {
  if (!n || !a || !a->out || !a->ws || a->B <= 0) return SDY_ERR_ARG;
  SDY_TRY(sdy_sfno_ready(n));
  SfnoCall f(n, a, (hipStream_t)stream);
  SDY_TRY(f.check());
  SDY_TRY(f.inputs());
  SDY_TRY(f.time_mlp());
  SDY_TRY(f.encoder());
  for (int i = 0; i < n->cfg.num_layers; ++i) SDY_TRY(f.block(i));
  return f.decoder();
}
```

### spherical-dyffusion_amd/csrc/mlp_h3.hip

```cpp
#include <cstdlib>
#include <vector>
#include <cmath>
#include <type_traits>

#include "common.h"

typedef const sdy_f16x8 __attribute__((address_space(1)))* wptr_t;
typedef _Float16 f16x4 __attribute__((ext_vector_type(4)));

namespace {

constexpr int ME = 256;
constexpr int MH = 512;
constexpr int TN = 64;
constexpr int HC = 128;
constexpr int NCH = MH / HC;
constexpr int KS1 = ME / 16;
constexpr int KSC = HC / 16;
constexpr int RING = 16;
constexpr int NGROUPS = NCH * 2 * RING;
static_assert(KS1 == RING && 2 * KSC == RING, "ring slot = index inside a block");
constexpr float SX = SDY_ACT_SX;

struct MlpParams {
  const float* x; long x_bs;
  int x_tiled;
  const float* pa; const float* pd;
  const sdy_f16x8* w;
  const float* b1; const float* b2;
  float* out; long out_bs;
  const float* add; long add_bs;
  const float* add_a; const float* add_d;
  int HW, B;
  float s1, s2;
  uint32_t drop_thr; float drop_scale;
  uint32_t seed_lo, seed_hi, stream1, stream2, call, batch_offset;
  int rows_per_call;
  const float* batch_scale;
  double* stats;
  const float* keep_h; const float* keep_o;
  unsigned* flags;
  unsigned* head;
  unsigned long long* stamps;
  SdyImgMap omap;
  int add_local;
};

__device__ __forceinline__ int px_swz(int px) { return (px & 15) ^ (((px >> 4) & 1) * 3); }
__device__ __forceinline__ int xs_off(int px, int c) { return px * ME + (((c & 16) | ((c ^ px_swz(px)) & 15)) << 3); }
__device__ __forceinline__ int hs_off(int px, int c) { return px * HC + (((c ^ px_swz(px)) & 15) << 3); }

template <bool DROP, bool INJECT = false>
__global__ __launch_bounds__(256, 1) void mlp_h3_kernel(const MlpParams p) {
  extern __shared__ __attribute__((aligned(16))) unsigned char smem[];
  _Float16* Xs_hi = reinterpret_cast<_Float16*>(smem);
  _Float16* Xs_lo = Xs_hi + TN * ME;
  _Float16* Hs = Xs_lo + TN * ME;
  float* Cf = reinterpret_cast<float*>(Hs + 4 * TN * HC);
  float* Cb2 = Cf + 4 * ME;

  const int tid = threadIdx.x, lane = tid & 63;
  const int wave = __builtin_amdgcn_readfirstlane(tid >> 6);
  int h = lane >> 5, l31 = lane & 31;
  const int tpi = (p.HW + TN - 1) / TN;
  const int ntiles = tpi * p.B;
  const int t_per = (ntiles + (int)gridDim.x - 1) / (int)gridDim.x;
  const int t_begin = (int)blockIdx.x * t_per;
  const int t_end = (t_begin + t_per < ntiles) ? t_begin + t_per : ntiles;
  int z = 0, zo = 0, n0 = 0;
  bool full = true;

  sdy_f16x8 r_hi[RING], r_lo[RING];
  auto wbase_of = [&](int ln) { return (wptr_t)(p.w + (size_t)wave * (NGROUPS + RING) * SDY_GROUP + ln); };
  wptr_t wp = wbase_of(lane);
#pragma unroll
  for (int s = 0; s < RING; ++s) {
    r_hi[s] = wp[s * SDY_GROUP];
    r_lo[s] = wp[s * SDY_GROUP + 64];
  }
  wp += RING * SDY_GROUP;

  int q0 = tid & 15, o0 = tid >> 4;
  f32x4 xr[2][8];
  const float* pf_base = nullptr;
  const float* res_base = nullptr;
  unsigned pf_off = 0u;
  int pf_rs = 0;
  auto prefetch_setup = [&](int t) {
    const int zz = t / tpi, nn = (t - zz * tpi) * TN;
    const bool ok = nn + 4 * q0 < p.HW;
    pf_base = p.x + (long)zz * p.x_bs + (p.x_tiled ? (long)(t - zz * tpi) * (ME * TN) : 0L);
    pf_rs = p.x_tiled ? TN : p.HW;
    pf_off = p.x_tiled ? (unsigned)(8 * o0 * TN + 4 * q0) * 4u : (unsigned)(8 * o0 * p.HW + (ok ? nn + 4 * q0 : 0)) * 4u;
  };
  auto prefetch_piece = [&](int piece) {
    const int oc = piece >> 3, e = piece & 7;
    xr[oc][e] = sdy_ld16s(pf_base + (long)(8 * 16 * oc + e) * pf_rs, pf_off);
  };
  auto prefetch_x = [&](int t) {
    const int zz = t / tpi, nn = (t - zz * tpi) * TN;
    const bool ok = nn + 4 * q0 < p.HW;
    const float* xz = p.x + (long)zz * p.x_bs + (p.x_tiled ? (long)(t - zz * tpi) * (ME * TN) : 0L);
    const int rs = p.x_tiled ? TN : p.HW;
    const unsigned xo = p.x_tiled ? (unsigned)(8 * o0 * TN + 4 * q0) * 4u : (unsigned)(8 * o0 * p.HW + (ok ? nn + 4 * q0 : 0)) * 4u;
#pragma unroll
    for (int oc = 0; oc < 2; ++oc)
#pragma unroll
      for (int e = 0; e < 8; ++e) xr[oc][e] = sdy_ld16s(xz + (long)(8 * 16 * oc + e) * rs, xo);
  };
  auto load_coeffs = [&](int zz) {
    const int t = 64 * wave + (int)__builtin_amdgcn_mbcnt_hi(~0u, __builtin_amdgcn_mbcnt_lo(~0u, 0u));
    const long c = (long)zz * ME + t, co = (long)sdy_img(p.omap, zz) * ME + t;
    Cf[t] = p.pa ? p.pa[c] * SX : SX;
    Cf[ME + t] = p.pa ? p.pd[c] * SX : 0.0f;
    Cf[2 * ME + t] = p.add_a ? p.add_a[co] : 1.0f;
    Cf[3 * ME + t] = p.add_a ? p.add_d[co] : 0.0f;
  };
  Cb2[tid] = DROP ? p.b2[tid] * p.drop_scale : p.b2[tid];
  if (t_begin < t_end) load_coeffs(t_begin / tpi);
  __syncthreads();
  if (t_begin < t_end) prefetch_x(t_begin);
  double psum[16], psq[16];
#pragma unroll
  for (int i = 0; i < 16; ++i) { psum[i] = 0.0; psq[i] = 0.0; }

  for (int tile = t_begin; tile < t_end; ++tile) {
  asm volatile("" : "+v"(l31), "+v"(h), "+v"(q0), "+v"(o0));
  const int tile_it = tile - t_begin;
// ... 366 lines not shown
    };
    auto ldb1 = [&](int set, int t, int part) {
      const int j = part & 1;
      const int off = hs_off(32 * j + l31, 2 * t + h);
      if (part < 2) bh[set][j] = *reinterpret_cast<const sdy_f16x8*>(Hh + off);
      else bl[set][j] = *reinterpret_cast<const sdy_f16x8*>(Hl + off);
    };
    ldb(0, 0);
#pragma unroll
    for (int t = 0; t < KSC; ++t) {
      const int c = t & 1;
      if (!SDY_MLP_PINNED && t + 1 < KSC) ldb(c ^ 1, t + 1);
      __builtin_amdgcn_sched_barrier(0);
      Piece ps;
#pragma unroll
      for (int mi = 0; mi < 2; ++mi) {
        const int s = 2 * t + mi;
#pragma unroll
        for (int k = 0; k < 6; ++k) {
          const int j = k & 1;
          const sdy_f16x8 a = (k < 2) ? r_lo[s] : r_hi[s];
          const sdy_f16x8 b = (k >= 2 && k < 4) ? bl[c][j] : bh[c][j];
          if (SDY_H3_PASSES == 3 || k >= 4) oacc[mi][j] = __builtin_amdgcn_mfma_f32_32x32x16_f16(a, b, oacc[mi][j], 0, 0, 0);
          if (SDY_MLP_PINNED && mi == 0 && k < 4 && t + 1 < KSC) ldb1(c ^ 1, t + 1, k);
          if (SDY_MLP_PINNED && !CHAIN) __builtin_amdgcn_sched_barrier(0);
          if constexpr (CHAIN) {
            if (SDY_MLP_SCALAR_CHAIN) chain_slot(ps, 6 * mi + k, hc2 + 1, t & 1, t >> 1);
            else chain_stage(ps, 6 * mi + k, hc2 + 1, t & 1, t >> 1);
            __builtin_amdgcn_sched_barrier(0);
          }
        }
        r_hi[s] = wp[s * SDY_GROUP];
        r_lo[s] = wp[s * SDY_GROUP + 64];
        __builtin_amdgcn_sched_barrier(0);
      }
    }
    wp += RING * SDY_GROUP;
  };
  using T_ = std::integral_constant<bool, true>;
  using F_ = std::integral_constant<bool, false>;

  stamp(1);
  load_bias(0);
  fc1(0);
  stamp(2);
#pragma unroll
  for (int pc = 0; pc < 8; ++pc) chain_piece(0, pc & 1, pc >> 1);
  stamp(3);
  __syncthreads();
  stamp(4);
  load_bias(1);
  fc1(1);
  stamp(5);
#pragma unroll
  for (int mi = 0; mi < 2; ++mi)
#pragma unroll
    for (int j = 0; j < 2; ++j)
#pragma unroll
      for (int r = 0; r < 16; ++r) oacc[mi][j][r] = 0.0f;
#pragma unroll 1
  for (int hc = 1; hc < NCH; ++hc) {
    fc2(hc - 1, T_{});
    stamp(4 + 2 * hc);
    __syncthreads();
    if (hc < NCH - 1) {
      load_bias(hc + 1);
      fc1(hc + 1);
    }
    stamp(5 + 2 * hc);
  }
  {
    int ln = lane;
    asm volatile("" : "+v"(ln));
    wp = wbase_of(ln);
  }
  asm volatile("" : "+v"(wp));
  {
    const int nt = tile + 1;
    prefetch_setup(nt < t_end ? nt : tile);
  }
  fc2(NCH - 1, F_{});
  stamp(12);
  {
    res_base = p.add ? p.add + (long)(p.add_local ? z : zo) * p.add_bs : p.x + (long)z * p.x_bs;
  }

  {
    const float bscale = p.batch_scale ? p.batch_scale[zo] : 1.0f;
    const float s2e = do_drop ? p.s2 * p.drop_scale * p.drop_scale : p.s2;
    const uint32_t c1_base2 = (uint32_t)(((uint64_t)(zt + p.batch_offset) * (uint64_t)(ME >> 2)) & 0xFFFFFFFFu);
    float* Os = reinterpret_cast<float*>(smem);
#pragma unroll
    for (int mi = 0; mi < 2; ++mi) {
      const int row0 = 64 * wave + 32 * mi + 4 * h;
      f32x4 bv[4];
#pragma unroll
      for (int g4 = 0; g4 < 4; ++g4) bv[g4] = *reinterpret_cast<const f32x4*>(Cb2 + row0 + 8 * g4);
#pragma unroll
      for (int g4 = 0; g4 < 4; ++g4) {
        uint32_t words[4] = {0xFFFFFFFFu, 0xFFFFFFFFu, 0xFFFFFFFFu, 0xFFFFFFFFu};
        if (do_drop && !INJECT) {
          const philox4 w = philox4x32((uint32_t)(n0 + l31), c1_base2 + (uint32_t)((row0 + 8 * g4) >> 2), p.stream2,
                                          call_z, p.seed_lo, p.seed_hi);
          words[0] = w.x; words[1] = w.y; words[2] = w.z; words[3] = w.w;
        }
#pragma unroll
        for (int j = 0; j < 2; ++j) {
          const int px = 32 * j + l31;
#pragma unroll
          for (int r4 = 0; r4 < 4; r4 += 2) {
            sdy_gf2 o = sdy_gf2{oacc[mi][j][4 * g4 + r4], oacc[mi][j][4 * g4 + r4 + 1]} * s2e +
                        sdy_gf2{bv[g4][r4], bv[g4][r4 + 1]};
            if (do_drop) {
              if constexpr (INJECT) {
                const int pix = (n0 + px < p.HW) ? n0 + px : p.HW - 1;
                const float* km = p.keep_o + ((long)zo * ME + row0 + 8 * g4 + r4) * p.HW + pix;
                o = sdy_gf2{km[0] != 0.0f ? o.x : 0.0f, km[p.HW] != 0.0f ? o.y : 0.0f};
              } else {
                o = sdy_gf2{sdy_keep16(words[r4], j, p.drop_thr) ? o.x : 0.0f,
                            sdy_keep16(words[r4 + 1], j, p.drop_thr) ? o.y : 0.0f};
              }
            }
            o = o * bscale;
            Os[(row0 + 8 * g4 + r4) * TN + px] = o.x;
            Os[(row0 + 8 * g4 + r4 + 1) * TN + px] = o.y;
          }
        }
        {
          const int i0 = 2 * (4 * mi + g4);
          rres[i0] = sdy_ld16s(res_base + (long)(16 * i0) * p.HW, e_ro);
          rres[i0 + 1] = sdy_ld16s(res_base + (long)(16 * (i0 + 1)) * p.HW, e_ro);
          prefetch_piece(i0);
          prefetch_piece(i0 + 1);
        }
      }
    }
    stamp(13);
    __syncthreads();
    stamp(14);
    if (e_ok) {
      float* oz = p.out + (long)zo * p.out_bs;
      const float* os = Os + (tid >> 4) * TN + 4 * (tid & 15);
#pragma unroll
      for (int i = 0; i < 16; ++i) {
        const int row = (tid >> 4) + 16 * i;
        f32x4 v = *reinterpret_cast<const f32x4*>(os + 16 * i * TN);
        if (p.add) v += rres[i] * Cf[2 * ME + row] + Cf[3 * ME + row];
        sdy_st16s(oz + (long)(16 * i) * p.HW, e_ro, v);
        if (p.stats) {
          psum[i] += (double)sdy_quad_sum(v);
          psq[i] += (double)sdy_quad_sumsq(v);
        }
      }
    }
    if (p.stats) {
      const int nt = tile + 1;
      if (nt >= t_end || nt / tpi != z) {
#pragma unroll
        for (int i = 0; i < 16; ++i) {
          double s1 = psum[i], s2 = psq[i];
#pragma unroll
          for (int m = 1; m < 16; m <<= 1) {
            s1 += __shfl_xor(s1, m, 64);
            s2 += __shfl_xor(s2, m, 64);
          }
          if ((tid & 15) == 0) {
            double* st = p.stats + ((long)zo * ME + (tid >> 4) + 16 * i) * 2;
// ... 41 lines not shown
                               float* scale1, float* scale2) {
  if (!w1_host || !w2_host || !packed_dev || !scale1 || !scale2) return SDY_ERR_ARG;
  if (!sdy_mlp_h3_supported(E, hidden)) return SDY_ERR_UNSUPPORTED;
  const float s1 = sdy_h3_scale(sdy_h3_absmax(w1_host, (size_t)E * hidden));
  const float s2 = sdy_h3_scale(sdy_h3_absmax(w2_host, (size_t)E * hidden));
  const size_t gh = (size_t)SDY_GROUP * 8;
  std::vector<_Float16> buf((size_t)4 * (NGROUPS + RING) * gh, (_Float16)0.0f);
  for (int w = 0; w < 4; ++w) {
    _Float16* d = buf.data() + (size_t)w * (NGROUPS + RING) * gh;
    auto put_fc1 = [&](int hc) {
      for (int ks = 0; ks < KS1; ++ks, d += gh) {
        const float* blk = w1_host + (size_t)(128 * hc + 32 * w) * ME + 16 * ks;
        sdy_h3_put_group(d, s1, [&](int r, int k) { return blk[(size_t)r * ME + k]; });
      }
    };
    auto put_fc2 = [&](int hc) {
      for (int t = 0; t < KSC; ++t)
        for (int mi = 0; mi < 2; ++mi, d += gh) {
          const float* blk = w2_host + (size_t)(64 * w + 32 * mi) * MH + 16 * (KSC * hc + t);
          sdy_h3_put_group(d, s2, [&](int r, int k) { return blk[(size_t)r * MH + k]; });
        }
    };
    put_fc1(0);
    put_fc1(1);
    for (int hc = 1; hc < NCH; ++hc) {
      put_fc2(hc - 1);
      if (hc < NCH - 1) put_fc1(hc + 1);
    }
    put_fc2(NCH - 1);
  }
  SDY_HIP_TRY(hipMemcpy(packed_dev, buf.data(), buf.size() * sizeof(_Float16), hipMemcpyHostToDevice));
  *scale1 = s1;
  *scale2 = s2;
  return SDY_OK;
}

#endif

int sdy_mlp_h3_inject(const sdy_mlp_args* a, void* stream);

#ifdef SDY_MLP_INJECT_TU
int sdy_mlp_h3_inject(const sdy_mlp_args* a, void* stream) {
#else
extern "C" int sdy_mlp_h3(const sdy_mlp_args* a, void* stream) {
  if (a && (a->keep_hidden || a->keep_out)) {
    if (!a->keep_hidden || !a->keep_out || !(a->drop_p > 0.0f)) return SDY_ERR_ARG;
    return sdy_mlp_h3_inject(a, stream);
  }
#endif
  if (!a || !a->x || !a->w || !a->b1 || !a->b2 || !a->out) return SDY_ERR_ARG;
  if (a->B <= 0 || a->HW <= 0) return SDY_ERR_ARG;
  if (!sdy_mlp_h3_supported(a->E, a->hidden)) return SDY_ERR_UNSUPPORTED;
  if ((a->pa == nullptr) != (a->pd == nullptr) || (a->add_a == nullptr) != (a->add_d == nullptr)) return SDY_ERR_ARG;
  if ((a->HW & 3) || (a->x_bstride & 3) || (a->out_bstride & 3) || (a->add && (a->add_bstride & 3))) return SDY_ERR_ALIGN;
  if ((long)a->HW * ME * 4 >= (1L << 32)) return SDY_ERR_UNSUPPORTED;
  if (a->drop_p < 0.0f || a->drop_p >= 1.0f) return SDY_ERR_ARG;
  if (a->B > 65535) return SDY_ERR_UNSUPPORTED;
  MlpParams p{};
  p.x = a->x; p.x_bs = a->x_bstride; p.x_tiled = a->x_tiled; p.pa = a->pa; p.pd = a->pd;
  if (a->x_tiled && !a->add) return SDY_ERR_ARG;
  p.w = reinterpret_cast<const sdy_f16x8*>(a->w);
  p.b1 = a->b1; p.b2 = a->b2;
  p.out = a->out; p.out_bs = a->out_bstride; p.add = a->add; p.add_bs = a->add_bstride;
  p.add_a = a->add ? a->add_a : nullptr; p.add_d = a->add ? a->add_d : nullptr;
  p.HW = a->HW; p.B = a->B;
  p.s1 = 1.0f / (a->w1_scale * SX);
  p.s2 = 1.0f / (a->w2_scale * SX);
  if (a->drop_p > 0.0f) {
    p.drop_thr = sdy_drop_threshold16(a->drop_p);
    if (p.drop_thr == 0u) p.drop_thr = 1u;
    p.drop_scale = 1.0f / (1.0f - a->drop_p);
  }
  p.seed_lo = (uint32_t)(a->seed & 0xFFFFFFFFu); p.seed_hi = (uint32_t)(a->seed >> 32);
  p.stream1 = a->stream_fc1; p.stream2 = a->stream_fc2; p.call = a->call; p.batch_offset = a->batch_offset;
  if (a->rows_per_call < 0 || (!a->out_rows && a->rows_per_call > 0 && a->B % a->rows_per_call)) return SDY_ERR_ARG;
  if (a->out_rows && a->rows_per_call == 0) return SDY_ERR_ARG;
  p.rows_per_call = a->rows_per_call > 0 ? a->rows_per_call : a->B;
  p.batch_scale = a->batch_scale;
  p.stats = a->stats;
  p.keep_h = a->keep_hidden; p.keep_o = a->keep_out;
  if (a->out_rows && !a->add) return SDY_ERR_ARG;
  if (a->add_by_launch_row && (!a->out_rows || a->add_a)) return SDY_ERR_ARG;
  p.add_local = a->add_by_launch_row ? 1 : 0;
  SDY_TRY(sdy_img_map_fill(p.omap, a->out_rows, a->B));
  SDY_TRY(sdy_flags_ptr(&p.flags));
  SDY_TRY(sdy_headroom_ptr(SDY_RANGE_MLP, &p.head));
  p.stamps = nullptr;
#if SDY_STAMPS_ON && !defined(SDY_MLP_INJECT_TU)
  if (std::getenv("SDY_MLP_STAMPS")) {
    if (!g_stamps) SDY_HIP_TRY(hipMalloc(&g_stamps, 64 * sizeof(unsigned long long)));
    p.stamps = g_stamps;
  }
#endif
  int n_cu = 0;
  SDY_TRY(sdy_cu_count(&n_cu));
  const long ntiles = (long)((a->HW + TN - 1) / TN) * a->B;
  dim3 grid((unsigned)(ntiles < n_cu ? ntiles : n_cu));
  constexpr size_t smem = (size_t)(2 * TN * ME + 4 * TN * HC) * sizeof(_Float16) + 5 * ME * sizeof(float);
  static SdyOncePerDevice once;
  std::atomic<bool>* attr_done = nullptr;
  SDY_TRY(once.slot(&attr_done));
#ifdef SDY_MLP_INJECT_TU
  if (!*attr_done) {
    SDY_HIP_TRY(hipFuncSetAttribute(reinterpret_cast<const void*>(&mlp_h3_kernel<true, true>),
                                    hipFuncAttributeMaxDynamicSharedMemorySize, (int)smem));
    *attr_done = true;
  }
  hipLaunchKernelGGL((mlp_h3_kernel<true, true>), grid, dim3(256), smem, (hipStream_t)stream, p);
#else
  if (!*attr_done) {
    SDY_HIP_TRY(hipFuncSetAttribute(reinterpret_cast<const void*>(&mlp_h3_kernel<false>),
                                    hipFuncAttributeMaxDynamicSharedMemorySize, (int)smem));
    SDY_HIP_TRY(hipFuncSetAttribute(reinterpret_cast<const void*>(&mlp_h3_kernel<true>),
                                    hipFuncAttributeMaxDynamicSharedMemorySize, (int)smem));
    *attr_done = true;
  }
  if (p.drop_thr != 0u)
    hipLaunchKernelGGL(mlp_h3_kernel<true>, grid, dim3(256), smem, (hipStream_t)stream, p);
  else
    hipLaunchKernelGGL(mlp_h3_kernel<false>, grid, dim3(256), smem, (hipStream_t)stream, p);
#endif
  return sdy_launch_status();
}
```

### spherical-dyffusion_amd/csrc/pointwise.h

```cpp
#pragma once
#include <hip/hip_runtime.h>
#include <stdint.h>

struct SdyTimeMlp {
  int E;
  int T;
  int num_layers;
  const float* freq;
  const float* w1t;
  const float* b1;
  const float* w2t;
  const float* b2;
  const float* wbt;
  const float* bb;
  float dp_rate[32];
  uint32_t dp_thr[32];
};

int sdy_instnorm_coeffs_launch(const float* x, int B, int C, int HW, const float* gamma, const float* beta,
                               const float* ss, long ss_stride, float eps, float* a, float* d, hipStream_t stream);
int sdy_concat_launch(const float* const* src, const int* chans, int nsrc, float* out, long out_bstride, int B, int HW,
                      hipStream_t stream, int src_rows = 0);
struct SdyConcatGen {
  int gen;
  const float* coef;
  const float* noise;
  uint64_t seed;
  uint32_t call, batch_offset;
  int rows_per_call;
};
int sdy_concat_gen_launch(const float* const* src, const int* chans, int nsrc, const SdyConcatGen& g, float* out,
                          long out_bstride, int B, int HW, hipStream_t stream);
int sdy_cond_noise_launch(uint64_t seed, uint32_t call, uint32_t batch_offset, int rows_per_call, int B, int C, int HW, float* out,
                          hipStream_t stream);
int sdy_cold_update_launch(const float* xs, const float* xn, const float* xi, float* out, size_t n, hipStream_t stream);
int sdy_time_mlp_launch(const SdyTimeMlp& t, const float* time, int B, float* trep, float* ss, float* dp,
                        const float* dp_keep_in, int enable_dropout, uint64_t seed, uint32_t call,
                        uint32_t batch_offset, int rows_per_call, hipStream_t stream, float* scratch);
int sdy_spec_to_torch_launch(const float* Cs, float* out, int B, int C, int L, int mtr, int Mfull, hipStream_t stream);
int sdy_spec_zero_upper_launch(float* Cs, int L, int mtr, int N, hipStream_t stream);
int sdy_torch_to_spec_launch(const float* in, float* Cs, int B, int C, int L, int mtr, int Mfull, hipStream_t stream);
int sdy_instnorm_from_partials_launch(const double* part, int K, int B, int C, int HW, const float* gamma, const float* beta,
                                      float eps, float* a, float* d, hipStream_t stream);
int sdy_gelu_stats_launch(const float* y, long y_bs, float* out, long out_bs, int out_tiled, double* stats, int B, int C,
                          int HW, hipStream_t stream);
int sdy_affine_copy_stats_launch(const float* x, long x_bs, const float* a, const float* d, float* out, long out_bs,
                                 double* stats, int C, int HW, const unsigned char* rows, int n_rows, hipStream_t stream,
                                 int src_row0 = -1);
```

### spherical-dyffusion_amd/csrc/pointwise.hip

```cpp
#include <cmath>
#include <atomic>
#include <mutex>
#include <vector>
#include "common.h"
#include "pointwise.h"

namespace {

inline bool al16(const void* p) { return ((uintptr_t)p & 15) == 0; }

__global__ __launch_bounds__(256) void instnorm_coeffs_kernel(const float* __restrict__ x, int C, int HW,
                                                               const float* __restrict__ gamma,
                                                               const float* __restrict__ beta,
                                                               const float* __restrict__ ss, long ss_stride, float eps,
                                                               float* __restrict__ a_out, float* __restrict__ d_out,
                                                               unsigned* __restrict__ flags) {
  const int c = blockIdx.x, b = blockIdx.y;
  const float* px = x + ((long)b * C + c) * HW;
  double s = 0.0, s2 = 0.0;
  const int n4 = HW >> 2;
  const f32x4* p4 = reinterpret_cast<const f32x4*>(px);
  for (int i = threadIdx.x; i < n4; i += 256) {
    const f32x4 v = p4[i];
    s += (double)v.x + (double)v.y + (double)v.z + (double)v.w;
// ... 103 lines not shown
  const float a = gamma[c] * rstd;
  a_out[i] = a;
  d_out[i] = beta[c] - (float)mean * a;
}

__global__ __launch_bounds__(256) void affine_copy_stats_kernel(const float* __restrict__ x, long x_bs,
                                                                 const float* __restrict__ a, const float* __restrict__ d,
                                                                 float* __restrict__ out, long out_bs,
                                                                 double* __restrict__ stats, int C, int HW,
                                                                 const SdyImgMap rows, int src_row0) {
  const int c = blockIdx.x, b = sdy_img(rows, blockIdx.y), bs = src_row0 >= 0 ? src_row0 + (int)blockIdx.y : b;
  const f32x4* p4 = reinterpret_cast<const f32x4*>(x + (long)bs * x_bs + (long)c * HW);
  f32x4* o4 = reinterpret_cast<f32x4*>(out + (long)b * out_bs + (long)c * HW);
  const float av = a ? a[b * C + c] : 1.0f, dv = a ? d[b * C + c] : 0.0f;
  double s = 0.0, s2 = 0.0;
  const int n4 = HW >> 2;
  for (int i = threadIdx.x; i < n4; i += 256) {
    const f32x4 r = p4[i];
    f32x4 v;
#pragma unroll
    for (int e = 0; e < 4; ++e) v[e] = __builtin_fmaf(r[e], av, dv);
    o4[i] = v;
    s += (double)sdy_quad_sum(v);
    s2 += (double)sdy_quad_sumsq(v);
  }
  if (!stats) return;
#pragma unroll
  for (int off = 32; off > 0; off >>= 1) {
    s += __shfl_down(s, off, 64);
    s2 += __shfl_down(s2, off, 64);
  }
  __shared__ double sh[8];
  const int lane = threadIdx.x & 63, wave = threadIdx.x >> 6;
  if (lane == 0) {
    sh[wave] = s;
    sh[4 + wave] = s2;
  }
  __syncthreads();
  if (threadIdx.x == 0) {
    stats[((long)b * C + c) * 2] += (sh[0] + sh[1]) + (sh[2] + sh[3]);
    stats[((long)b * C + c) * 2 + 1] += (sh[4] + sh[5]) + (sh[6] + sh[7]);
  }
}

__global__ __launch_bounds__(256) void gelu_stats_kernel(const float* __restrict__ y, long y_bs, float* __restrict__ out,
                                                          long out_bs, int out_tiled, double* __restrict__ stats, int C,
                                                          int HW) {
  const int c = blockIdx.x, b = blockIdx.y;
  const f32x4* p4 = reinterpret_cast<const f32x4*>(y + (long)b * y_bs + (long)c * HW);
  float* ob = out + (long)b * out_bs + (out_tiled ? (long)c * 64 : (long)c * HW);
  const long tile_stride = (long)C * 64;
  double s = 0.0, s2 = 0.0;
  const int n4 = HW >> 2;
  for (int i = threadIdx.x; i < n4; i += 256) {
    const f32x4 r = p4[i];
    f32x4 v;
#pragma unroll
    for (int e = 0; e < 4; ++e) v[e] = gelu_erf_exact(r[e]);
    const int px = 4 * i;
    float* o = out_tiled ? ob + (long)(px >> 6) * tile_stride + (px & 63) : ob + px;
    *reinterpret_cast<f32x4*>(o) = v;
    s += (double)sdy_quad_sum(v);
    s2 += (double)sdy_quad_sumsq(v);
  }
  if (!stats) return;
#pragma unroll
  for (int off = 32; off > 0; off >>= 1) {
    s += __shfl_down(s, off, 64);
    s2 += __shfl_down(s2, off, 64);
  }
  __shared__ double sh[8];
  const int lane = threadIdx.x & 63, wave = threadIdx.x >> 6;
  if (lane == 0) {
    sh[wave] = s;
    sh[4 + wave] = s2;
  }
  __syncthreads();
  if (threadIdx.x == 0) {
    stats[((long)b * C + c) * 2] += (sh[0] + sh[1]) + (sh[2] + sh[3]);
    stats[((long)b * C + c) * 2 + 1] += (sh[4] + sh[5]) + (sh[6] + sh[7]);
  }
}

struct ConcatArgs {
  const float* src[4];
  int chans[4];
  int nsrc;
};
__global__ __launch_bounds__(256) void concat_kernel(const ConcatArgs a, float* __restrict__ out, long out_bstride,
                                                      int HW4, int src_rows) {
  const int i = blockIdx.x * 256 + threadIdx.x;
  if (i >= HW4) return;
  int c = blockIdx.y;
  const int b = blockIdx.z;
  const int bs = src_rows > 0 ? b % src_rows : b;
  int s = 0, coff = 0;
  while (s < a.nsrc - 1 && c >= a.chans[s]) {
    c -= a.chans[s];
    coff += a.chans[s];
    ++s;
  }
  const f32x4* src = reinterpret_cast<const f32x4*>(a.src[s] + ((long)bs * a.chans[s] + c) * HW4 * 4);
  f32x4* dst = reinterpret_cast<f32x4*>(out + (long)b * out_bstride + (long)(coff + c) * HW4 * 4);
  dst[i] = src[i];
}

struct ConcatGenArgs {
  ConcatArgs cat;
  int gen;
  const float* coef;
  const float* noise;
  uint32_t seed_lo, seed_hi, call, batch_offset;
  int rows_per_call;
};
__global__ __launch_bounds__(256) void concat_gen_kernel(const ConcatGenArgs g, float* __restrict__ out, long out_bstride,
                                                          int HW4) {
  const int i = blockIdx.x * 256 + threadIdx.x;
  if (i >= HW4) return;
  int c = blockIdx.y;
  const int b = blockIdx.z;
  int s = 0, coff = 0;
  while (s < g.cat.nsrc - 1 && c >= g.cat.chans[s]) {
    c -= g.cat.chans[s];
    coff += g.cat.chans[s];
    ++s;
  }
  const int C = g.cat.chans[s];
  const long plane = ((long)b * C + c) * HW4 * 4;
  const f32x4 x = reinterpret_cast<const f32x4*>(g.cat.src[s] + plane)[i];
  f32x4* dst = reinterpret_cast<f32x4*>(out + (long)b * out_bstride + (long)(coff + c) * HW4 * 4);
  if (s != g.gen) {
    dst[i] = x;
    return;
  }
  const float a = g.coef[2 * b], sc = g.coef[2 * b + 1];
  f32x4 v;
  if (sc == 0.0f) {
    v.x = __fmul_rn(a, x.x); v.y = __fmul_rn(a, x.y); v.z = __fmul_rn(a, x.z); v.w = __fmul_rn(a, x.w);
  } else {
    f32x4 e;
    if (g.noise) {
      e = reinterpret_cast<const f32x4*>(g.noise + plane)[i];
    } else {
      const int bq = b / g.rows_per_call;
      e = sdy_cond_noise4((uint32_t)i, (uint32_t)(b - bq * g.rows_per_call) + g.batch_offset, (uint32_t)C, (uint32_t)c,
                          g.call + (uint32_t)bq, g.seed_lo, g.seed_hi);
    }
    v.x = __fadd_rn(__fmul_rn(a, x.x), __fmul_rn(sc, e.x));
    v.y = __fadd_rn(__fmul_rn(a, x.y), __fmul_rn(sc, e.y));
    v.z = __fadd_rn(__fmul_rn(a, x.z), __fmul_rn(sc, e.z));
    v.w = __fadd_rn(__fmul_rn(a, x.w), __fmul_rn(sc, e.w));
  }
  dst[i] = v;
}

__global__ __launch_bounds__(256) void cond_noise_kernel(float* __restrict__ out, int HW4, uint32_t seed_lo, uint32_t seed_hi,
                                                          uint32_t call, uint32_t batch_offset, int rows_per_call) {
  const int i = blockIdx.x * 256 + threadIdx.x;
  if (i >= HW4) return;
  const int c = blockIdx.y, C = gridDim.y, b = blockIdx.z;
  const int bq = b / rows_per_call;
  reinterpret_cast<f32x4*>(out + ((long)b * C + c) * HW4 * 4)[i] =
      sdy_cond_noise4((uint32_t)i, (uint32_t)(b - bq * rows_per_call) + batch_offset, (uint32_t)C, (uint32_t)c,
                      call + (uint32_t)bq, seed_lo, seed_hi);
}

// ... 579 lines not shown
  if (!words[dev]) {
    SDY_HIP_TRY(hipMalloc(&words[dev], 64));
    SDY_HIP_TRY(hipMemset(words[dev], 0, 64));
  }
  *flags = words[dev];
  return SDY_OK;
}
int sdy_gelu_table_ptr(const float** table_dev) {
  static float* tabs[SDY_MAX_DEVICES] = {};
  static std::mutex mu;
  int dev = 0;
  SDY_TRY(sdy_current_device(&dev));
  std::lock_guard<std::mutex> g(mu);
  if (!tabs[dev]) {
    std::vector<float> h((size_t)SDY_GELU_NODES * 4);
    const double hstep = 1.0 / 32.0, sx = (double)SDY_GELU_SX / (double)SDY_GELU_WS, inv_sqrt_2pi = 0.39894228040143267794;
    for (int n = 0; n < SDY_GELU_NODES; ++n) {
      const double x = -6.0 + n * hstep;
      const double Phi = 0.5 * std::erfc(-x * 0.70710678118654752440), phi = inv_sqrt_2pi * std::exp(-0.5 * x * x);
      double c0 = sx * Phi, c1 = sx * phi * hstep, c2 = -sx * x * phi * hstep * hstep / 2.0,
             c3 = sx * (x * x - 1.0) * phi * hstep * hstep * hstep / 6.0;
      if (n == 0) { c0 = 0.0; c1 = c2 = c3 = 0.0; }
      if (n == SDY_GELU_NODES - 1) { c0 = sx; c1 = c2 = c3 = 0.0; }
      h[4 * n] = (float)c0; h[4 * n + 1] = (float)c1; h[4 * n + 2] = (float)c2; h[4 * n + 3] = (float)c3;
    }
    float* d = nullptr;
    SDY_HIP_TRY(hipMalloc(&d, h.size() * sizeof(float)));
    SDY_HIP_TRY(hipMemcpy(d, h.data(), h.size() * sizeof(float), hipMemcpyHostToDevice));
    tabs[dev] = d;
  }
  *table_dev = tabs[dev];
  return SDY_OK;
}

static std::atomic<bool> g_headroom_on{false};
int sdy_headroom_ptr(int slot, unsigned** word) {
  *word = nullptr;
  if (!g_headroom_on.load(std::memory_order_relaxed) || slot < 0 || slot >= SDY_RANGE_SLOTS) return SDY_OK;
  unsigned* d = nullptr;
  SDY_TRY(sdy_flags_ptr(&d));
  *word = d + 1 + slot;
  return SDY_OK;
}
extern "C" int sdy_range_headroom_enable(int on) {
  g_headroom_on.store(on != 0);
  return SDY_OK;
}
extern "C" int sdy_range_headroom(float* max_staged, int reset, void* stream) {
  if (!max_staged) return SDY_ERR_ARG;
  unsigned* d = nullptr;
  SDY_TRY(sdy_flags_ptr(&d));
  SDY_HIP_TRY(hipMemcpyAsync(max_staged, d + 1, SDY_RANGE_SLOTS * sizeof(float), hipMemcpyDeviceToHost, (hipStream_t)stream));
  if (reset) SDY_HIP_TRY(hipMemsetAsync(d + 1, 0, SDY_RANGE_SLOTS * sizeof(unsigned), (hipStream_t)stream));
  SDY_HIP_TRY(hipStreamSynchronize((hipStream_t)stream));
  return SDY_OK;
}
extern "C" int sdy_dropout_stream_rounds(void) { return SDY_PHILOX_ROUNDS; }
extern "C" int sdy_dropout_stream_words(uint32_t c0, uint32_t c1, uint32_t c2, uint32_t c3, uint32_t key_lo, uint32_t key_hi,
                                        uint32_t* out4) {
  if (!out4) return SDY_ERR_ARG;
  const philox4 w = philox4x32(c0, c1, c2, c3, key_lo, key_hi);
  out4[0] = w.x; out4[1] = w.y; out4[2] = w.z; out4[3] = w.w;
  return SDY_OK;
}

extern "C" int sdy_status_flags(unsigned* flags, int reset, void* stream) {
  if (!flags) return SDY_ERR_ARG;
  unsigned* d = nullptr;
  SDY_TRY(sdy_flags_ptr(&d));
  SDY_HIP_TRY(hipMemcpyAsync(flags, d, sizeof(unsigned), hipMemcpyDeviceToHost, (hipStream_t)stream));
  if (reset) SDY_HIP_TRY(hipMemsetAsync(d, 0, sizeof(unsigned), (hipStream_t)stream));
  SDY_HIP_TRY(hipStreamSynchronize((hipStream_t)stream));
  return SDY_OK;
}
extern "C" int sdy_status_flags_async(unsigned* flags_host, int reset, void* stream) {
  if (!flags_host) return SDY_ERR_ARG;
  unsigned* d = nullptr;
  SDY_TRY(sdy_flags_ptr(&d));
  SDY_HIP_TRY(hipMemcpyAsync(flags_host, d, sizeof(unsigned), hipMemcpyDeviceToHost, (hipStream_t)stream));
  if (reset) SDY_HIP_TRY(hipMemsetAsync(d, 0, sizeof(unsigned), (hipStream_t)stream));
  return SDY_OK;
}

int sdy_instnorm_coeffs_launch(const float* x, int B, int C, int HW, const float* gamma, const float* beta,
                               const float* ss, long ss_stride, float eps, float* a, float* d, hipStream_t stream) {
  if (!x || !gamma || !beta || !a || !d || B <= 0 || C <= 0 || HW <= 0) return SDY_ERR_ARG;
  if (HW & 3) return SDY_ERR_ALIGN;
  unsigned* flags = nullptr;
  SDY_TRY(sdy_flags_ptr(&flags));
  hipLaunchKernelGGL(instnorm_coeffs_kernel, dim3(C, B), dim3(256), 0, stream, x, C, HW, gamma, beta, ss, ss_stride,
                     eps, a, d, flags);
  return sdy_launch_status();
}

extern "C" int sdy_instnorm_from_stats(double* stats, int B, int C, int HW, const float* gamma, const float* beta,
                                       const float* ss, long ss_stride, float eps, float* a, float* d, void* stream) {
  if (!stats || !gamma || !beta || !a || !d || B <= 0 || C <= 0 || HW <= 0) return SDY_ERR_ARG;
  const int BC = B * C;
  unsigned* flags = nullptr;
  SDY_TRY(sdy_flags_ptr(&flags));
  hipLaunchKernelGGL(instnorm_from_stats_kernel, dim3((BC + 255) / 256), dim3(256), 0, (hipStream_t)stream, stats, BC, C, HW,
                     gamma, beta, ss, ss_stride, eps, a, d, flags);
  return sdy_launch_status();
}

int sdy_instnorm_from_partials_launch(const double* part, int K, int B, int C, int HW, const float* gamma, const float* beta,
                                      float eps, float* a, float* d, hipStream_t stream) {
  if (!part || !gamma || !beta || !a || !d || K <= 0 || B <= 0 || C <= 0 || HW <= 0) return SDY_ERR_ARG;
  const int BC = B * C;
  unsigned* flags = nullptr;
  SDY_TRY(sdy_flags_ptr(&flags));
  hipLaunchKernelGGL(instnorm_from_partials_kernel, dim3((BC + 255) / 256), dim3(256), 0, stream, part, K, BC, C, HW, gamma, beta, eps,
                     a, d, flags);
  return sdy_launch_status();
}

int sdy_gelu_stats_launch(const float* y, long y_bs, float* out, long out_bs, int out_tiled, double* stats, int B, int C,
                          int HW, hipStream_t stream) {
  if (!y || !out || B <= 0 || C <= 0 || HW <= 0) return SDY_ERR_ARG;
  if ((HW & 3) || (y_bs & 3) || (out_bs & 3)) return SDY_ERR_ALIGN;
  hipLaunchKernelGGL(gelu_stats_kernel, dim3(C, B), dim3(256), 0, stream, y, y_bs, out, out_bs, out_tiled, stats, C, HW);
  return sdy_launch_status();
}

int sdy_affine_copy_stats_launch(const float* x, long x_bs, const float* a, const float* d, float* out, long out_bs,
                                 double* stats, int C, int HW, const unsigned char* rows, int n_rows, hipStream_t stream,
                                 int src_row0) {
  if (!x || (a == nullptr) != (d == nullptr) || !out || !rows || C <= 0 || HW <= 0 || n_rows <= 0) return SDY_ERR_ARG;
  if ((HW & 3) || (x_bs & 3) || (out_bs & 3)) return SDY_ERR_ALIGN;
  SdyImgMap m;
  SDY_TRY(sdy_img_map_fill(m, rows, n_rows));
  hipLaunchKernelGGL(affine_copy_stats_kernel, dim3(C, n_rows), dim3(256), 0, stream, x, x_bs, a, d, out, out_bs, stats, C, HW, m,
                     src_row0);
  return sdy_launch_status();
}

int sdy_concat_launch(const float* const* src, const int* chans, int nsrc, float* out, long out_bstride, int B, int HW,
                      hipStream_t stream, int src_rows) {
  if (!src || !chans || !out || nsrc < 1 || nsrc > 4 || B <= 0 || HW <= 0) return SDY_ERR_ARG;
  if ((HW & 3) || (out_bstride & 3) || !al16(out)) return SDY_ERR_ALIGN;
  ConcatArgs a;
  int total = 0;
  for (int i = 0; i < 4; ++i) {
    a.src[i] = i < nsrc ? src[i] : nullptr;
    a.chans[i] = i < nsrc ? chans[i] : 0;
    if (i < nsrc) {
      if (!src[i] || chans[i] <= 0) return SDY_ERR_ARG;
      total += chans[i];
    }
  }
  for (int i = 0; i < nsrc; ++i)
    if (!al16(src[i])) return SDY_ERR_ALIGN;
  a.nsrc = nsrc;
  const int HW4 = HW / 4;
  hipLaunchKernelGGL(concat_kernel, dim3((HW4 + 255) / 256, total, B), dim3(256), 0, stream, a, out, out_bstride, HW4, src_rows);
  return sdy_launch_status();
}

int sdy_concat_gen_launch(const float* const* src, const int* chans, int nsrc, const SdyConcatGen& gen, float* out,
                          long out_bstride, int B, int HW, hipStream_t stream) {
  if (!src || !chans || !out || nsrc < 1 || nsrc > 4 || B <= 0 || HW <= 0) return SDY_ERR_ARG;
  if (gen.gen < 0 || gen.gen >= nsrc || !gen.coef || gen.rows_per_call <= 0 || B % gen.rows_per_call) return SDY_ERR_ARG;
  if ((HW & 3) || (out_bstride & 3) || !al16(out) || !al16(gen.noise)) return SDY_ERR_ALIGN;
  ConcatGenArgs g;
  int total = 0;
  for (int i = 0; i < 4; ++i) {
// ... 84 lines not shown
```

### spherical-dyffusion_amd/csrc/tables.cpp

```cpp
#include <cmath>
#include <cstring>
#include <vector>

#include "../../include/sdy_amd.h"

namespace {

const long double PI_L = 3.141592653589793238462643383279502884L;

void leggauss(int n, std::vector<double>& x, std::vector<double>& w) {
  x.assign(n, 0.0);
  w.assign(n, 0.0);
  for (int i = 0; i < (n + 1) / 2; ++i) {
    long double z = cosl(PI_L * (i + 0.75L) / (n + 0.5L));
    long double pp = 0.0L;
    for (int it = 0; it < 100; ++it) {
      long double p1 = 1.0L, p2 = 0.0L;
      for (int j = 1; j <= n; ++j) {
        long double p3 = p2;
        p2 = p1;
        p1 = ((2.0L * j - 1.0L) * z * p2 - (j - 1.0L) * p3) / j;
      }
      pp = n * (z * p1 - p2) / (z * z - 1.0L);
      long double z1 = z;
// ... 18 lines not shown
    x[i] = std::cos(t);
  }
  if (n == 2) {
    w[0] = w[1] = 1.0;
    return;
  }
  const int n1 = n - 1;
  std::vector<long double> Nn;
  for (int k = 1; k < n1; k += 2) Nn.push_back((long double)k);
  const int l = (int)Nn.size();
  const int m = n1 - l;
  std::vector<long double> v0(l + 1 + m, 0.0L);
  for (int i = 0; i < l; ++i) v0[i] = 2.0L / Nn[i] / (Nn[i] - 2.0L);
  v0[l] = 1.0L / Nn[l - 1];
  std::vector<long double> v(n1);
  const int len = l + 1 + m;
  for (int i = 0; i < n1; ++i) v[i] = 0.0L - v0[i] - v0[len - 1 - i];
  std::vector<long double> g(n1, -1.0L);
  g[l] += n1;
  g[m] += n1;
  const long double den = (long double)n1 * n1 - 1.0L + (n1 % 2);
  for (int i = 0; i < n1; ++i) g[i] /= den;
  for (int j = 0; j < n1; ++j) {
    long double acc = 0.0L;
    for (int k = 0; k < n1; ++k) {
      long long jk = ((long long)j * k) % n1;
      acc += (v[k] + g[k]) * cosl(2.0L * PI_L * jk / n1);
    }
    w[j] = (double)(acc / n1);
  }
  w[n1] = w[0];
}

}

extern "C" int sdy_sht_tables_host(int nlat, int nlon, int lmax, int mmax, int grid, double* pct, double* wq,
                                   double* theta_out) {
  if (nlat < 2 || nlon < 2 || lmax < 1 || mmax < 1) return SDY_ERR_ARG;
  std::vector<double> cost, w;
  if (grid == SDY_GRID_LEGENDRE_GAUSS)
    leggauss(nlat, cost, w);
  else if (grid == SDY_GRID_EQUIANGULAR)
    clenshaw_curtiss(nlat, cost, w);
  else
    return SDY_ERR_ARG;
  std::vector<double> theta(nlat), x(nlat);
  for (int k = 0; k < nlat; ++k) theta[k] = std::acos(cost[nlat - 1 - k]);
  for (int k = 0; k < nlat; ++k) x[k] = std::cos(theta[k]);
  if (theta_out) std::memcpy(theta_out, theta.data(), sizeof(double) * nlat);
  if (wq) std::memcpy(wq, w.data(), sizeof(double) * nlat);
  if (!pct) return SDY_OK;

  const int nmax = mmax > lmax ? mmax : lmax;
  const size_t K = (size_t)nlat;
  std::vector<double> vdm((size_t)nmax * nmax * K, 0.0);
  auto V = [&](int m, int l) { return vdm.data() + ((size_t)m * nmax + l) * K; };
  const double v00 = 1.0 / std::sqrt(4.0 * M_PI);
  for (size_t k = 0; k < K; ++k) V(0, 0)[k] = v00;
  for (int l = 1; l < nmax; ++l) {
    const double a = std::sqrt(2.0 * l + 1.0);
    for (size_t k = 0; k < K; ++k) {
      V(l - 1, l)[k] = a * x[k] * V(l - 1, l - 1)[k];
      V(l, l)[k] = std::sqrt((2.0 * l + 1.0) * (1.0 + x[k]) * (1.0 - x[k]) / 2.0 / l) * V(l - 1, l - 1)[k];
    }
  }
  for (int l = 2; l < nmax; ++l) {
    for (int m = 0; m < l - 1; ++m) {
      const double a = std::sqrt((2.0 * l - 1.0) / (l - m) * (2.0 * l + 1.0) / (l + m));
      const double b = std::sqrt((double)(l + m - 1) / (l - m) * (2.0 * l + 1.0) / (2.0 * l - 3.0) * (l - m - 1) / (l + m));
      for (size_t k = 0; k < K; ++k) V(m, l)[k] = x[k] * a * V(m, l - 1)[k] - b * V(m, l - 2)[k];
    }
  }
  for (int m = 0; m < mmax; ++m) {
    const double sgn = (m & 1) ? -1.0 : 1.0;
    for (int l = 0; l < lmax; ++l) {
      const double* src = V(m, l);
      double* dst = pct + ((size_t)m * lmax + l) * K;
      for (size_t k = 0; k < K; ++k) dst[k] = sgn * src[k];
    }
  }
  return SDY_OK;
}

int sdy_factor_radices(int n, int* radices, int* nstages) {
  int cnt = 0;
  const int cand[4] = {4, 2, 3, 5};
  for (int ci = 0; ci < 4; ++ci) {
    while (n % cand[ci] == 0 && n > 1) {
      if (cnt >= 10) return SDY_ERR_UNSUPPORTED;
      radices[cnt++] = cand[ci];
      n /= cand[ci];
    }
  }
  if (n != 1) return SDY_ERR_UNSUPPORTED;
  *nstages = cnt;
  return SDY_OK;
}
```

### spherical-dyffusion_amd/dyffusion.py

```python
from __future__ import annotations

from types import SimpleNamespace
from typing import Any, Dict, List, Optional, Sequence, Union

import numpy as np
import torch
from torch import Tensor

from . import ops

FORWARD_CONDITIONING = ("data", "none", "data+noise-v1", "data+noise-v2")


class DYffusion(torch.nn.Module):
    def __init__(
        self,
        model,
        interpolator,
        timesteps: int,
        forward_conditioning: str = "none",
        dynamic_cond_from_t: str = "h",
        schedule: str = "before_t1_only",
        additional_interpolation_steps: int = 0,
        additional_interpolation_steps_factor: int = 0,
        interpolate_before_t1: bool = True,
        sampling_type: str = "cold",
        sampling_schedule: Union[List[float], str, None] = None,
        use_cold_sampling_for_intermediate_steps: bool = True,
        use_cold_sampling_for_last_step: bool = True,
        use_cold_sampling_for_init_of_ar_step: Optional[bool] = None,
        time_encoding: str = "dynamics",
        refine_intermediate_predictions: bool = False,
        prediction_timesteps: Optional[Sequence[float]] = None,
        enable_interpolator_dropout: Union[bool, str] = True,
        interpolator_use_ema: bool = False,
        log_every_t: Union[str, int, None] = None,
        hack_for_imprecise_interpolation: bool = False,
        fuse_interpolator_pair_max_batch: int = 8,
        reuse_interpolator_encoder: bool = True,
        **unused,
    ):
        super().__init__()
        if schedule != "before_t1_only":
            raise NotImplementedError(f"schedule={schedule!r}: only 'before_t1_only' (the shipped config) is in scope")
        if forward_conditioning not in FORWARD_CONDITIONING:
            raise ValueError(f"Invalid value for forward_conditioning: {forward_conditioning!r}, "
                             f"must be one of {list(FORWARD_CONDITIONING)}")
        if time_encoding not in ("dynamics", "discrete"):
            raise ValueError(f"Invalid time_encoding: {time_encoding}")
        if enable_interpolator_dropout not in [True, False, "always", "except_dynamical_steps"]:
            raise ValueError(f"invalid enable_interpolator_dropout={enable_interpolator_dropout!r}")
        assert additional_interpolation_steps_factor == 0, \
            "additional_interpolation_steps_factor must be 0 when using before_t1_only schedule"
        assert interpolate_before_t1, "interpolate_before_t1 must be True when using before_t1_only schedule"
        assert timesteps > 1, f"horizon must be > 1, but got {timesteps}. Please use datamodule.horizon with > 1"
        self.model = model
        self.interpolator = interpolator
        if use_cold_sampling_for_init_of_ar_step is None:
            use_cold_sampling_for_init_of_ar_step = use_cold_sampling_for_last_step
        self.use_cold_sampling_for_init_of_ar_step = use_cold_sampling_for_init_of_ar_step
        self.hparams = SimpleNamespace(
            timesteps=timesteps, forward_conditioning=forward_conditioning, dynamic_cond_from_t=dynamic_cond_from_t,
            schedule=schedule, additional_interpolation_steps=additional_interpolation_steps,
            sampling_type=sampling_type, time_encoding=time_encoding,
            use_cold_sampling_for_intermediate_steps=use_cold_sampling_for_intermediate_steps,
            use_cold_sampling_for_last_step=use_cold_sampling_for_last_step,
            refine_intermediate_predictions=refine_intermediate_predictions,
            prediction_timesteps=prediction_timesteps, interpolator_use_ema=interpolator_use_ema,
            log_every_t=log_every_t, hack_for_imprecise_interpolation=hack_for_imprecise_interpolation,
        )
        self.additional_diffusion_steps = additional_interpolation_steps
        self.num_timesteps = timesteps + self.additional_diffusion_steps
        d_to_i = {d: self.diffusion_step_to_interpolation_step(d) for d in range(1, self.num_timesteps)}
        self.dynamical_steps = {d: i for d, i in d_to_i.items() if float(i).is_integer()}
        self.i_to_diffusion_step = {i: d for d, i in d_to_i.items()}
        self.artificial_interpolation_steps = {d: i for d, i in d_to_i.items() if not float(i).is_integer()}
        self.enable_interpolator_dropout = enable_interpolator_dropout
        self.fuse_interpolator_pair_max_batch = int(fuse_interpolator_pair_max_batch)
        import os
        self.reuse_interpolator_encoder = bool(reuse_interpolator_encoder) and os.environ.get("SDY_NO_ENCODER_REUSE") is None
        self.share_pair_inputs = os.environ.get("SDY_NO_SHARED_INPUTS") is None
        self.full_sampling_schedule = list(range(0, self.num_timesteps))
        self.sampling_schedule = sampling_schedule or self.full_sampling_schedule
        self.interpolator_window = getattr(interpolator, "window", 1)
        self.interpolator_horizon = getattr(interpolator, "true_horizon", timesteps)
        last = self.diffusion_step_to_interpolation_step(self.num_timesteps - 1)
        if self.interpolator_horizon != last + 1:
            raise ValueError(f"interpolator horizon {self.interpolator_horizon} must be equal to the "
                             f"last interpolation step+1=i_N=i_{self.num_timesteps - 1}={last + 1}")

    @property
    def diffusion_steps(self) -> List[int]:
        return list(range(0, self.num_timesteps))

    def diffusion_step_to_interpolation_step(self, diffusion_step):
        assert 0 <= diffusion_step <= self.num_timesteps - 1, \
            f"diffusion_step must be in [0, num_timesteps-1]=[0, {self.num_timesteps - 1}], but got {diffusion_step}"
        k = self.additional_diffusion_steps
        if diffusion_step >= k + 1:
            return diffusion_step - k
        return diffusion_step / (k + 1)

    @property
    def valid_time_range_for_backbone_model(self) -> List[float]:
        if self.hparams.time_encoding == "discrete":
            return self.diffusion_steps
        return [self.diffusion_step_to_interpolation_step(d) for d in self.diffusion_steps]

    @property
    def sampling_schedule(self):
        return self._sampling_schedule

    def _named_schedule(self, name: str) -> List[float]:
        import math
        import re

        artificial = sorted(self.artificial_interpolation_steps)
        first_data_step = min(self.dynamical_steps) if self.dynamical_steps else self.num_timesteps - 1
        m = re.fullmatch(r"only_dynamics(?:_plus(_discrete)?(\d+)(_discrete)?)?", name)
        if m:
            extra: List[float] = []
            if m.group(2) is not None:
                n = int(m.group(2)) + 1
                extra = [first_data_step * i / n for i in range(n)]
                if m.group(1) or m.group(3):
                    extra = [float(math.floor(v)) for v in extra]
        elif (m := re.fullmatch(r"every(\d+)(?:th|nd|rd|st)?", name)):
            stride = int(m.group(1))
            assert 1 <= stride <= self.num_timesteps, f"Invalid sampling schedule: {name}"
            extra = artificial[::stride]
        elif (m := re.fullmatch(r"first(\d*\.?\d+)(?:v2)?", name)):
            amount = float(m.group(1))
            if amount < 1:
                assert amount > 0, f"Invalid sampling schedule: {name}, must end with number/float > 0"
                count = math.ceil(amount * len(artificial))
            else:
                assert amount.is_integer(), f"If first_n >= 1, it must be an integer, but got {amount}"
                assert amount <= self.num_timesteps, f"Invalid sampling schedule: {name}"
                count = int(amount)
            extra = artificial[:count]
        else:
            raise ValueError(f"Invalid sampling schedule: ``{name}``. ")
        return sorted({0, *self.dynamical_steps, *extra})

    @sampling_schedule.setter
    def sampling_schedule(self, schedule):
        if isinstance(schedule, str):
            schedule = self._named_schedule(schedule)
        steps = [int(v) if float(v).is_integer() else float(v) for v in schedule]
        if not steps or steps[0] != 0:
            steps = [0] + steps
        assert 1 <= steps[-1] <= self.num_timesteps, \
            f"Invalid sampling schedule: {steps}, must end with number/float <= {self.num_timesteps}"
        assert all(b > a for a, b in zip(steps, steps[1:])), \
            f"Invalid sampling schedule not monotonically increasing: {steps}"
        self._sampling_schedule = steps

    @staticmethod
    def _time_tensor(value: float, like: Tensor) -> Tensor:
        return torch.full((like.shape[0],), float(value), dtype=torch.float32, device=like.device)

    @staticmethod
    def _check_time_range(net, value: float) -> None:
        lo, hi = getattr(net, "min_time", None), getattr(net, "max_time", None)
        if lo is not None and hi is not None:
            assert lo <= value <= hi, f"time must be in [{lo}, {hi}], but time is {value}"

    def q_sample(self, x0, x_end, t, interpolation_time=None, is_artificial_step: bool = True, _keep_packed=None,
                 **kwargs) -> Tensor:
        assert t is None or interpolation_time is None, "Either t or interpolation_time must be None."
        i_n = interpolation_time if t is None else self.diffusion_step_to_interpolation_step(t)
        dyn = kwargs.pop("dynamical_condition", None)
        if dyn is not None:
            kwargs["condition"] = self.interpolator.get_dynamical_condition(dyn, i_n)
        time = self._time_tensor(i_n, x0)
        self._check_time_range(getattr(self.interpolator, "model", None), float(i_n))
        do_enable = bool(
            self.enable_interpolator_dropout in [True, "always"]
            or (self.enable_interpolator_dropout == "except_dynamical_steps" and is_artificial_step)
        )
        kwargs.pop("num_predictions", None)
        with self.interpolator.inference_dropout_scope(condition=do_enable):
            return self._interpolate(initial_condition=x_end, x_last=x0, t=time, t_host=i_n, _keep_packed=_keep_packed, **kwargs)

    def _interpolate(self, initial_condition: Tensor, x_last: Tensor, t: Tensor, t_host=None, num_predictions: int = 1,
                     _packed_inputs: Optional[Tensor] = None, _keep_packed=None, **kwargs) -> Tensor:
        if t_host is not None:
            assert 0 < t_host < self.interpolator_horizon, \
                f"interpolate time must be in (0, {self.interpolator_horizon}), got {t_host}"
        hack = self.hparams.hack_for_imprecise_interpolation
        if _packed_inputs is None:
            pieces = [initial_condition] + ([initial_condition[:, :1]] if hack else []) + [x_last]
            inputs = ops.concat_channels(pieces)
        else:
            inputs = _packed_inputs
        if _keep_packed is not None:
            _keep_packed.append(inputs)
        out = self.interpolator.predict_packed(inputs, time=t, **kwargs)["preds"]
        if hack:
            out = ops.concat_channels([initial_condition[:, :1], out])
        return out

    def _can_reuse_encoder(self, kwargs) -> bool:
        net = getattr(self.interpolator, "model", None)
        return (self.reuse_interpolator_encoder and kwargs.get("dynamical_condition") is None
                and hasattr(net, "batch_offset") and getattr(net, "mask_injector", None) is None)

    def q_sample_two(self, x0, x_end, t_first, t_second, is_artificial_step: bool = True, **kwargs):
        packed = []
        first = self.q_sample(x0=x0, x_end=x_end, t=t_first, is_artificial_step=is_artificial_step, _keep_packed=packed,
                              **dict(kwargs))
        second = self.q_sample(x0=x0, x_end=x_end, t=t_second, is_artificial_step=is_artificial_step,
                               _packed_inputs=packed[0], reuse_encoder=True, **dict(kwargs))
        return first, second

    def _can_stack_calls(self) -> bool:
        net = getattr(self.interpolator, "model", None)
        return hasattr(net, "batch_offset") and getattr(net, "mask_injector", None) is None

    def q_sample_pair(self, x0, x_end, t_first, t_second, is_artificial_step: bool = True, **kwargs):
        B = x0.shape[0]
        i_a, i_b = (self.diffusion_step_to_interpolation_step(t) for t in (t_first, t_second))
        for i_n in (i_a, i_b):
            assert 0 < i_n < self.interpolator_horizon, f"interpolate time must be in (0, {self.interpolator_horizon}), got {i_n}"
            self._check_time_range(getattr(self.interpolator, "model", None), float(i_n))
        kwargs.pop("num_predictions", None)
        dyn = kwargs.pop("dynamical_condition", None)
        two = lambda v: torch.cat([v, v], dim=0)
        time = torch.cat([self._time_tensor(i_a, x0), self._time_tensor(i_b, x0)])
        hack = self.hparams.hack_for_imprecise_interpolation
        inputs = ops.concat_channels([x_end] + ([x_end[:, :1]] if hack else []) + [x0])
        share = dyn is None and self.share_pair_inputs and \
            getattr(getattr(self.interpolator, "model", None), "supports_shared_inputs", False)
        if not share:
            kwargs = {k: (two(v) if torch.is_tensor(v) and v.dim() > 0 and v.shape[0] == B else v) for k, v in kwargs.items()}
            if dyn is not None:
                kwargs["condition"] = torch.cat([self.interpolator.get_dynamical_condition(dyn, i_a),
                                                 self.interpolator.get_dynamical_condition(dyn, i_b)], dim=0)
            inputs = two(inputs)
        else:
            kwargs["shared_inputs"] = True
        do_enable = bool(
            self.enable_interpolator_dropout in [True, "always"]
            or (self.enable_interpolator_dropout == "except_dynamical_steps" and is_artificial_step)
        )
        with self.interpolator.inference_dropout_scope(condition=do_enable):
            out = self.interpolator.predict_packed(inputs, time=time, rows_per_call=B, **kwargs)["preds"]
        if hack:
            out = ops.concat_channels([two(x_end[:, :1]), out])
        return out[:B], out[B:]

    def forward_condition_coefs(self, t):
        mode = self.hparams.forward_conditioning
        if mode == "none":
            return None
        if mode == "data":
            return 1.0, 0.0
        f = np.float32(t) / np.float32(self.num_timesteps - 1)
        g = np.float32(1.0) - f
        return (float(f), float(g)) if mode == "data+noise-v1" else (float(g), float(f))

    def predict_x_last(self, initial_condition: Tensor, x_t: Tensor, t, **kwargs) -> Tensor:
        assert 0 <= t <= self.num_timesteps - 1, f"Invalid timestep: {t}. {self.num_timesteps=}"
        coefs = self.forward_condition_coefs(t)
        if coefs is not None:
            kwargs["forward_condition"] = (initial_condition,) + coefs
        dyn = kwargs.pop("dynamical_condition", None)
        cond = None
        if dyn is not None:
            assert dyn.shape[1] == self.num_timesteps + 1, f"{dyn.shape}[1] != {self.num_timesteps + 1}"
            sel = self.hparams.dynamic_cond_from_t
            if sel == "0":
                cond = dyn[:, 0]
            elif sel == "h":
                cond = dyn[:, -1]
            elif sel == "t":
                cond = dyn[:, int(t)]
            else:
                raise ValueError(f"Invalid dynamic_cond_from_t: {sel}")
        time_v = t if self.hparams.time_encoding == "discrete" else self.diffusion_step_to_interpolation_step(t)
        time = self._time_tensor(time_v, x_t)
        self._check_time_range(self.model, float(time_v))
        return self.model.predict_forward(x_t, time=time, condition=cond, **kwargs)

    def _drop_carried_channel(self, x: Tensor) -> Tensor:
        return x[:, 1:] if self.hparams.hack_for_imprecise_interpolation else x

    def sample_loop(self, initial_condition, log_every_t=None, num_predictions: int = None, verbose=True, **kwargs):
        hp = self.hparams
        if hp.sampling_type not in ("cold", "naive"):
            raise ValueError(f"unknown sampling type {hp.sampling_type}")
        assert len(initial_condition.shape) == 4, f"condition.shape: {initial_condition.shape} (should be 4D)"
        sched, last = self.sampling_schedule, self.num_timesteps - 1
        cold = hp.sampling_type == "cold"
        preds: Dict[str, Tensor] = {}
        x_s, x_hat, k = initial_condition, None, 0
        for pos, s in enumerate(sched):
            s_next = sched[pos + 1] if pos + 1 < len(sched) else sched[-1] + 1
            final = s == last
            x_hat = self.predict_x_last(initial_condition=initial_condition, x_t=x_s, t=s, **dict(kwargs))
            x_at_s = None
            i_next = self.diffusion_step_to_interpolation_step(s_next) if not final else None
            lands_on_data = final or float(i_next).is_integer()
            ipol = dict(x0=x_hat, x_end=initial_condition, is_artificial_step=not lands_on_data)
            if final:
                assert s_next > last, f"Invalid s_next: {s_next} (should be <= {last})"
                x_next = ops.concat_channels([initial_condition[:, :1], x_hat]) if hp.hack_for_imprecise_interpolation \
                    else x_hat
            else:
                assert s_next <= last, f"Invalid s_next: {s_next} (should be <= {last})"
                if cold and s > 0 and x_s.shape[0] <= self.fuse_interpolator_pair_max_batch and self._can_stack_calls():
                    x_next, x_at_s = self.q_sample_pair(x_hat, initial_condition, s_next, s,
                                                        is_artificial_step=not lands_on_data, **dict(kwargs))
                elif cold and s > 0 and self._can_reuse_encoder(kwargs):
                    x_next, x_at_s = self.q_sample_two(x_hat, initial_condition, s_next, s,
                                                       is_artificial_step=not lands_on_data, **dict(kwargs))
                else:
                    x_next = self.q_sample(**ipol, t=s_next, **dict(kwargs))
            if not cold:
                x_s = x_next
            elif final and not hp.use_cold_sampling_for_last_step:
                if self.use_cold_sampling_for_init_of_ar_step:
                    ar_init = ops.cold_update(x_s, x_hat, self.q_sample(**ipol, t=s, **dict(kwargs)))
                    preds["preds_autoregressive_init"] = self._drop_carried_channel(ar_init)
# ... 28 lines not shown
```

### spherical-dyffusion_amd/sfno.py

```python
from __future__ import annotations

import ctypes as C
import math
from contextlib import contextmanager
from typing import Dict, Optional

import torch
from torch import nn

from . import _lib
from ._lib import SdySfnoConfig, SdySfnoFwdArgs, aligned, check, current_stream, lib, ptr


class SphericalFourierNeuralOperatorNet(nn.Module):
    def __init__(
        self,
        num_input_channels: int,
        num_output_channels: int,
        num_conditional_channels: int = 0,
        spatial_shape_in=(180, 360),
        spectral_transform: str = "sht",
        filter_type: str = "linear",
        operator_type: str = "dhconv",
        scale_factor: int = 1,
# ... 1 lines not shown
        num_layers: int = 8,
        use_mlp: bool = True,
        mlp_ratio: float = 2.0,
        activation_function: str = "gelu",
        encoder_layers: int = 1,
        pos_embed: bool = True,
        dropout_mlp: float = 0.0,
        drop_path_rate: float = 0.0,
        normalization_layer: str = "instance_norm",
        hard_thresholding_fraction: float = 1.0,
        big_skip: bool = True,
        factorization=None,
        separable: bool = False,
        with_time_emb: bool = False,
        time_dim_mult: int = 2,
        time_rescale: bool = False,
        time_scale_shift_before_filter: bool = True,
        data_grid: str = "equiangular",
        seed: int = 0,
        gemm_mode: Optional[str] = None,
        **other,
    ):
        super().__init__()
        unsupported = []
        inert = {"params", "dropout_filter", "num_blocks", "sparsity_threshold", "use_complex_kernels", "rank",
                 "complex_network", "complex_activation", "spectral_layers", "checkpointing", "verbose", "name",
                 "loss_function", "loss_function_weights", "datamodule_config", "num_output_channels_raw",
                 "spatial_shape_out"}
        if float(other.get("pos_emb_dropout", 0.0) or 0.0) > 0.0:
            unsupported.append(f"pos_emb_dropout={other['pos_emb_dropout']}")
        if other.get("debug_mode", False):
            unsupported.append("debug_mode=True")
        if other.get("params"):
            unsupported.append("params=<non-empty> (modulus-style parameter object)")
        unknown = sorted(set(other) - inert - {"pos_emb_dropout", "debug_mode"})
        if unknown:
            raise TypeError(f"SphericalFourierNeuralOperatorNet: unexpected keyword arguments {unknown}")
        if spectral_transform != "sht": unsupported.append(f"spectral_transform={spectral_transform}")
        if filter_type != "linear": unsupported.append(f"filter_type={filter_type}")
        if operator_type != "dhconv": unsupported.append(f"operator_type={operator_type}")
        if scale_factor != 1: unsupported.append(f"scale_factor={scale_factor}")
        if not use_mlp: unsupported.append("use_mlp=False")
        if activation_function != "gelu": unsupported.append(f"activation_function={activation_function}")
        if encoder_layers != 1: unsupported.append(f"encoder_layers={encoder_layers}")
        if normalization_layer != "instance_norm": unsupported.append(f"normalization_layer={normalization_layer}")
        if factorization is not None or separable: unsupported.append("factorized/separable weights")
        if time_rescale: unsupported.append("time_rescale=True")
        if with_time_emb and not time_scale_shift_before_filter: unsupported.append("time_scale_shift_before_filter=False")
        if unsupported:
            raise NotImplementedError("outside the hot-path scope (SURVEY.md section 8): " + ", ".join(unsupported))

        self.num_input_channels = num_input_channels
        self.num_output_channels = num_output_channels
        self.num_conditional_channels = num_conditional_channels
        self.img_shape = tuple(spatial_shape_in)
        self.in_chans = num_input_channels + num_conditional_channels
        self.out_chans = num_output_channels
        self.embed_dim = embed_dim
        self.num_layers = num_layers
        self.mlp_hidden = int(embed_dim * mlp_ratio)
        self.dropout_mlp = float(dropout_mlp)
        self.drop_path_rate = float(drop_path_rate)
        self.big_skip = bool(big_skip)
        self.use_pos_embed = bool(pos_embed)
        self.with_time_emb = bool(with_time_emb)
        self.time_dim = embed_dim * time_dim_mult if with_time_emb else 0
        self.data_grid = data_grid
        nlat, nlon = self.img_shape
        self.h, self.w = nlat // scale_factor, nlon // scale_factor
        self.modes_lat = int(self.h * hard_thresholding_fraction)
        self.modes_lon = int((self.w // 2 + 1) * hard_thresholding_fraction)
        self.min_time: Optional[float] = None
        self.max_time: Optional[float] = None
        self.inference_dropout = False
        self.seed = int(seed)
        self.gemm_mode = gemm_mode or _lib.default_gemm_mode()
        if self.gemm_mode not in ("f32", "h3"):
            raise ValueError(f"gemm_mode must be 'f32' or 'h3', got {self.gemm_mode!r}")
        self.batch_offset = 0
        self._call = 0
        self.mask_injector = None
        self.noise_injector = None
        self.supports_shared_inputs = True

        E, T, H, Cin, L = embed_dim, self.time_dim, self.mlp_hidden, self.in_chans, self.modes_lat
        P = lambda *s: nn.Parameter(torch.zeros(*s), requires_grad=False)
        self._params: Dict[str, nn.Parameter] = {}

        def reg(name, *shape):
            p = P(*shape)
            self.register_parameter(name.replace(".", "__"), p)
            self._params[name] = p
            return p

        reg("encoder.0.weight", E, Cin, 1, 1); reg("encoder.0.bias", E); reg("encoder.2.weight", E, E, 1, 1)
        if self.use_pos_embed:
            reg("pos_embed", 1, E, nlat, nlon)
        if with_time_emb:
            reg("time_emb_mlp.1.weight", T, E); reg("time_emb_mlp.1.bias", T)
            reg("time_emb_mlp.3.weight", T, T); reg("time_emb_mlp.3.bias", T)
        self._fc2 = "mlp.fwd.3" if self.dropout_mlp > 0.0 else "mlp.fwd.2"
        for i in range(num_layers):
            p = f"blocks.{i}."
            reg(p + "norm0.weight", E); reg(p + "norm0.bias", E)
            if with_time_emb:
                reg(p + "time_mlp.1.weight", 2 * E, T); reg(p + "time_mlp.1.bias", 2 * E)
            reg(p + "filter.filter.weight", E, E, L, 2); reg(p + "filter.filter.bias", 1, E, 1, 1)
            reg(p + "inner_skip.weight", E, E, 1, 1); reg(p + "inner_skip.bias", E)
            reg(p + "norm1.weight", E); reg(p + "norm1.bias", E)
            reg(p + "mlp.fwd.0.weight", H, E, 1, 1); reg(p + "mlp.fwd.0.bias", H)
            reg(p + self._fc2 + ".weight", E, H, 1, 1); reg(p + self._fc2 + ".bias", E)
        dec_in = E + (Cin if big_skip else 0)
        reg("decoder.0.weight", E, dec_in, 1, 1); reg("decoder.0.bias", E); reg("decoder.2.weight", self.out_chans, E, 1, 1)
        for i in range(num_layers):
            for nme in ("norm0", "norm1"):
                self._params[f"blocks.{i}.{nme}.weight"].data.fill_(1.0)

        self._native: Dict[int, C.c_void_p] = {}
        self._native_dirty = True
        self._ws: Dict[Optional[int], torch.Tensor] = {}

    def state_dict(self, *args, destination=None, prefix="", keep_vars=False):
        out = destination if destination is not None else {}
        for k, v in self._params.items():
            out[prefix + k] = v if keep_vars else v.detach()
        return out

    def load_state_dict(self, state_dict, strict: bool = True):
        missing, unexpected = [], []
        for k, p in self._params.items():
            if k in state_dict:
                v = state_dict[k]
                if tuple(v.shape) != tuple(p.shape):
                    raise RuntimeError(f"size mismatch for {k}: checkpoint {tuple(v.shape)} vs model {tuple(p.shape)}")
                p.data.copy_(v.detach().to(torch.float32))
            else:
                missing.append(k)
        for k in state_dict:
            if k not in self._params:
                spec = self._persisted_sht_table(k)
                if spec is not None:
                    self._check_persisted_sht_table(k, state_dict[k], *spec)
                    continue
                unexpected.append(k)
        if strict and (missing or unexpected):
            raise RuntimeError(f"load_state_dict: missing={missing[:5]}... unexpected={unexpected[:5]}...")
        self._native_dirty = True
        return missing, unexpected

    def _persisted_sht_table(self, key: str):
        leaf = key.rsplit(".", 1)[-1]
        if leaf not in ("weights", "pct"):
            return None
        owner = key[: -len(leaf) - 1]
        lg, dg = "legendre-gauss", self.data_grid
        fixed = {"trans_down": ("weights", dg), "itrans_up": ("pct", dg), "trans": ("weights", lg), "itrans": ("pct", lg)}
        if owner in fixed:
            return fixed[owner] if fixed[owner][0] == leaf else None
        parts = owner.split(".")
        if len(parts) == 5 and parts[0] == "blocks" and parts[1].isdigit() and parts[2:4] == ["filter", "filter"]:
            i = int(parts[1])
            if parts[4] == "forward_transform" and leaf == "weights":
                return "weights", (dg if i == 0 else lg)
            if parts[4] == "inverse_transform" and leaf == "pct":
                return "pct", (dg if i == self.num_layers - 1 else lg)
        return None
# ... 29 lines not shown
            raise _lib.SdyError(f"persisted SHT table {key} ({kind}, {grid}) differs from the table this library computes: "
                                f"max |diff| {diff:.3e} (table scale {scale:.3e}) at (m={m}, l={l}, k={k}).  The checkpoint "
                                f"was trained with different Legendre tables (torch-harmonics version / norm / csphase); "
                                f"results would not match the reference.")

    def set_min_max_time(self, min_time: float, max_time: float):
        self.min_time, self.max_time = float(min_time), float(max_time)

    def enable_inference_dropout(self):
        self.inference_dropout = True

    def disable_inference_dropout(self):
        self.inference_dropout = False

    @contextmanager
    def inference_dropout_scope(self, condition: bool, context=None):
        assert isinstance(condition, bool), f"Condition must be a boolean, got {condition}"
        if condition:
            self.enable_inference_dropout()
        try:
            yield None
        finally:
            if condition:
                self.disable_inference_dropout()

    def _cfg(self) -> SdySfnoConfig:
        c = SdySfnoConfig()
        c.nlat, c.nlon = self.img_shape
        c.in_chans, c.out_chans = self.in_chans, self.out_chans
        c.embed_dim, c.num_layers, c.mlp_hidden = self.embed_dim, self.num_layers, self.mlp_hidden
        c.lmax, c.mmax = self.modes_lat, self.modes_lon
        c.data_grid = _lib.SDY_GRID[self.data_grid]
        c.with_time_emb, c.time_dim = int(self.with_time_emb), self.time_dim
        c.dropout_mlp, c.drop_path_rate = self.dropout_mlp, self.drop_path_rate
        c.big_skip, c.pos_embed = int(self.big_skip), int(self.use_pos_embed)
        c.gemm_mode = 1 if self.gemm_mode == "h3" else 0
        return c

    def _get_native(self, device: torch.device) -> C.c_void_p:
        idx = device.index if device.index is not None else torch.cuda.current_device()
        if self._native_dirty:
            for h in self._native.values():
                lib.sdy_sfno_destroy(h)
            self._native.clear()
            self._native_dirty = False
        if idx not in self._native:
            with torch.cuda.device(idx):
                h = C.c_void_p()
                cfg = self._cfg()
                check(lib.sdy_sfno_create(C.byref(cfg), C.byref(h)), "sdy_sfno_create")
                for name, p in self._params.items():
                    t = p.detach().to("cpu", torch.float32).contiguous()
                    check(lib.sdy_sfno_set_param(h, name.encode(), ptr(t), t.numel()), f"sdy_sfno_set_param({name})")
                if self.with_time_emb:
                    half = self.embed_dim // 2
                    f = torch.exp(torch.arange(half, dtype=torch.float32) * -(math.log(10000) / (half - 1))).contiguous()
                    check(lib.sdy_sfno_set_param(h, b"@time_freq", ptr(f), half))
                dpr = torch.linspace(0, self.drop_path_rate, self.num_layers).to(torch.float32).contiguous()
                check(lib.sdy_sfno_set_param(h, b"@drop_path_rates", ptr(dpr), self.num_layers))
                rc = lib.sdy_sfno_ready(h)
                if rc != 0:
                    raise _lib.SdyError(f"native SFNO not ready, missing {lib.sdy_sfno_missing(h).decode()}")
                self._native[idx] = h
        return self._native[idx]

    def _workspace(self, h, device, B):
        n = int(lib.sdy_sfno_workspace_floats(h, B))
        ws = self._ws.get(device.index)
        if ws is None or ws.numel() < n:
            self._ws.pop(device.index, None)
            del ws
            self._ws[device.index] = torch.empty(n, dtype=torch.float32, device=device)
        return self._ws[device.index]

    def __del__(self):
        try:
            for h in self._native.values():
                lib.sdy_sfno_destroy(h)
        except Exception:
            pass

    def forward(self, inputs, time=None, condition=None, static_condition=None, return_time_emb: bool = False,
                keep_masks=None, drop_path_keep=None, rows_per_call: Optional[int] = None, reuse_encoder: bool = False,
                shared_inputs: bool = False, forward_condition=None, **kwargs):
        if return_time_emb:
            raise NotImplementedError("return_time_emb is a training-path feature")
        if not inputs.is_cuda:
            raise RuntimeError("sdy_amd SFNO runs on the GPU only (no CPU fallback); move inputs to cuda")
        dev = inputs.device
        gen = None
        if forward_condition is not None:
            if reuse_encoder or shared_inputs:
                raise ValueError("forward_condition changes with every call: no reuse_encoder / shared_inputs")
            gen = self._forward_condition(forward_condition, inputs.shape[0], dev)
        if self.num_conditional_channels > 0:
            if condition is None and static_condition is None and gen is None:
                raise ValueError(f"condition and static_condition are both None but num_conditional_channels is "
                                 f"{self.num_conditional_channels}")
        else:
            assert condition is None and gen is None, "condition is not None but num_conditional_channels is 0"
            assert static_condition is None, "static_condition is not None but num_conditional_channels is 0"
        pieces = [aligned(t.to(torch.float32).contiguous()) for t in (inputs, condition, static_condition) if t is not None]
        B = B_in = inputs.shape[0]
        if shared_inputs:
            assert rows_per_call == B_in and self.with_time_emb and torch.is_tensor(time) and time.numel() % B_in == 0 \
                and time.numel() > B_in, "shared_inputs: rows_per_call = the inputs' rows, one time per stacked row"
            B = time.numel()
        nlat, nlon = self.img_shape
        for t in pieces:
            assert t.shape[0] == B_in and tuple(t.shape[-2:]) == (nlat, nlon), f"bad input shape {tuple(t.shape)}"
        n_gen = 0 if gen is None else gen[0].shape[1]
        if sum(t.shape[1] for t in pieces) + n_gen != self.in_chans:
            raise RuntimeError(f"inputs.shape: {tuple(inputs.shape)}, expected {self.in_chans} channels in total, got "
                               f"{[t.shape[1] for t in pieces[:1]] + ([n_gen] if gen else []) + [t.shape[1] for t in pieces[1:]]}")
        tt = None
        if self.with_time_emb:
            assert self.min_time is not None and self.max_time is not None, \
                "min_time and max_time must be set before using time embedding"
            assert time is not None, "time is required when with_time_emb=True"
            tt = torch.as_tensor(time, dtype=torch.float32, device=dev).reshape(-1).contiguous()
            if tt.numel() == 1 and B > 1:
                tt = tt.expand(B).contiguous()
            assert tt.numel() == B
            if isinstance(time, (int, float)) or not torch.is_tensor(time) or not time.is_cuda:
                tv = torch.as_tensor(time, dtype=torch.float32).reshape(-1)
                assert (self.min_time <= tv).all() and (tv <= self.max_time).all(), \
                    f"time must be in [{self.min_time}, {self.max_time}], but time is {tv}"

        h = self._get_native(dev)
        max_b = int(lib.sdy_sfno_max_batch(h))
        if B > max_b:
            if rows_per_call not in (None, B) or shared_inputs or keep_masks is not None or drop_path_keep is not None or \
                    (self.mask_injector is not None and self.inference_dropout) or \
                    (gen is not None and self.noise_injector is not None):
                raise _lib.SdyError(f"batch {B} > {max_b} rows per native call cannot be split with stacked calls / injected masks")
            n_chunks = -(-B // max_b)
            step = -(-B // n_chunks)
            out = torch.empty(B, self.out_chans, nlat, nlon, dtype=torch.float32, device=dev)
            for r0 in range(0, B, step):
                r1 = min(B, r0 + step)
                self._native_call(h, dev, [t[r0:r1] for t in pieces], None if tt is None else tt[r0:r1], out[r0:r1],
                                  self._call, self.batch_offset + r0,
                                  gen=None if gen is None else (gen[0][r0:r1], gen[1][r0:r1], None))
            self._call += 1
            return out
        out = torch.empty(B, self.out_chans, nlat, nlon, dtype=torch.float32, device=dev)
        n_calls = 1
        if rows_per_call is not None:
            assert rows_per_call >= 1 and B % rows_per_call == 0, f"rows_per_call={rows_per_call} must divide the batch {B}"
            assert keep_masks is None and drop_path_keep is None and self.mask_injector is None, \
                "injected masks address one call per forward"
            n_calls = B // int(rows_per_call)
        if keep_masks is None and drop_path_keep is None and self.mask_injector is not None and self.inference_dropout:
            keep_masks, drop_path_keep = self.mask_injector(self._call)
        if gen is not None and self.noise_injector is not None:
            assert n_calls == 1, "injected noise addresses one call per forward"
            eps = self.noise_injector(self._call)
            if eps is not None:
                eps = aligned(eps.to(dev, torch.float32).contiguous())
                assert eps.shape == gen[0].shape, f"injected noise {tuple(eps.shape)} != {tuple(gen[0].shape)}"
            gen = (gen[0], gen[1], eps)
        self._native_call(h, dev, pieces, tt, out, self._call, self.batch_offset, rows_per_call, keep_masks, drop_path_keep,
                          reuse_encoder=bool(reuse_encoder), shared_inputs=bool(shared_inputs), gen=gen)
        self._call += n_calls
        return out

    def _forward_condition(self, fc, B: int, dev):
        x0, a, s = fc
        x0 = aligned(x0.to(torch.float32).contiguous())
        nlat, nlon = self.img_shape
        assert x0.shape[0] == B and tuple(x0.shape[-2:]) == (nlat, nlon), f"bad forward_condition shape {tuple(x0.shape)}"

        def col(v):
            t = torch.as_tensor(v, dtype=torch.float32).reshape(-1).to(dev)
            return t.expand(B) if t.numel() == 1 else t.reshape(B)
        return x0, torch.stack([col(a), col(s)], dim=1).contiguous(), None

    def _native_call(self, h, dev, pieces, tt, out, call: int, batch_offset: int, rows_per_call: Optional[int] = None,
                     keep_masks=None, drop_path_keep=None, reuse_encoder: bool = False, shared_inputs: bool = False,
                     gen=None) -> None:
        B = out.shape[0]
        ws = self._workspace(h, dev, B)
        a = SdySfnoFwdArgs()
        for i in range(3):
            a.in_[i] = ptr(pieces[i]) if i < len(pieces) else None
            a.in_chans[i] = pieces[i].shape[1] if i < len(pieces) else 0
        a.time, a.out, a.B = ptr(tt), ptr(out), B
        a.enable_dropout = int(self.inference_dropout)
        a.seed, a.call, a.batch_offset = self.seed, call & 0xFFFFFFFF, batch_offset
        if rows_per_call is not None:
            a.rows_per_call = int(rows_per_call)
        keep = []
        if keep_masks is not None:
            arr = (C.c_void_p * (2 * self.num_layers))()
            for j, m in enumerate(keep_masks):
                if m is not None:
                    mm = m.to(dev, torch.float32).contiguous()
                    keep.append(mm)
                    arr[j] = ptr(mm)
            a.keep_masks = C.cast(arr, C.POINTER(C.c_void_p))
            keep.append(arr)
        if drop_path_keep is not None:
            dk = drop_path_keep.to(dev, torch.float32).contiguous()
            assert dk.shape == (self.num_layers, B)
            keep.append(dk)
            a.drop_path_keep = ptr(dk)
        a.ws, a.ws_floats = ptr(ws), ws.numel()
        a.reuse_encoder = int(reuse_encoder)
        a.shared_inputs = int(shared_inputs)
        if gen is not None:
            keep.append(gen)
            a.gen_src, a.gen_chans, a.gen_pos = ptr(gen[0]), gen[0].shape[1], 1
            a.gen_coef, a.gen_noise = ptr(gen[1]), ptr(gen[2])
        with torch.cuda.device(dev):
            check(lib.sdy_sfno_forward(h, C.byref(a), current_stream()), "sdy_sfno_forward")

    def predict_forward(self, *inputs, metadata=None, **kwargs):
        return self(*inputs, **kwargs)

    def time_embedding(self, time: torch.Tensor):
        dev = time.device
        h = self._get_native(dev)
        B = time.numel()
        tt = time.to(torch.float32).contiguous()
        trep = torch.empty(B, self.time_dim, dtype=torch.float32, device=dev)
        ss = torch.empty(B, self.num_layers, 2 * self.embed_dim, dtype=torch.float32, device=dev)
        with torch.cuda.device(dev):
            check(lib.sdy_sfno_time_embed(h, ptr(tt), B, ptr(trep), ptr(ss), current_stream()), "sdy_sfno_time_embed")
        return trep, ss
```

Baseline: 166.6 member-forecast-steps/s.

## Share block-0 spectral transform across interpolator time pair via time-affine in coefficient space

When two interpolator calls share encoder inputs and differ only in time embedding, block 0's instance-norm, FFT, Legendre analysis/synthesis is computed once on the shared rows. The per-time scale/shift is then applied in spectral coefficient space, with the shift folded into the l=0 mode through a host-computed constant c00. The residual add uses a modulo row map into the shared roundtrip image. This is gated on an exact-roundtrip check of the constant field and on several path conditions. It saves one SHT roundtrip per paired call but adds a workspace, a new kernel, and reliance on linearity of the transform.

```diff
diff --git a/include/sdy_amd.h b/include/sdy_amd.h
--- a/include/sdy_amd.h
+++ b/include/sdy_amd.h
@@ -119,6 +119,7 @@
   const float* keep_out;
   const unsigned char* out_rows;
   int add_by_launch_row;
+  int add_src_rows;
 } sdy_mlp_args;
 int sdy_instnorm_from_stats(double* stats, int B, int C, int HW, const float* gamma, const float* beta,
                             const float* scale_shift, long ss_bstride, float eps, float* a_out, float* d_out, void* stream);
@@ -182,6 +183,7 @@
   float* ws; size_t ws_floats;
   int reuse_encoder;
   int shared_inputs;
+  int share_block0;
   const float* gen_src;
   int gen_chans;
   int gen_pos;
@@ -189,6 +191,7 @@
   const float* gen_noise;
 } sdy_sfno_fwd_args;
 int sdy_sfno_forward(sdy_sfno* net, const sdy_sfno_fwd_args* args, void* stream);
+int sdy_sht_ones_roundtrip_host(int nlat, int nlon, int lmax, int mmax, int grid_in, int grid_out, double* c00, double* p1_err);
 
 int sdy_sfno_time_embed(sdy_sfno* net, const float* time, int B, float* t_repr, float* ss, void* stream);
 
diff --git a/spherical-dyffusion_amd/_lib.py b/spherical-dyffusion_amd/_lib.py
--- a/spherical-dyffusion_amd/_lib.py
+++ b/spherical-dyffusion_amd/_lib.py
@@ -60,6 +60,7 @@
         ("keep_hidden", C.c_void_p), ("keep_out", C.c_void_p),
         ("out_rows", C.c_void_p),
         ("add_by_launch_row", C.c_int),
+        ("add_src_rows", C.c_int),
     ]
 
 
@@ -127,6 +128,7 @@
         ("ws", C.c_void_p), ("ws_floats", C.c_size_t),
         ("reuse_encoder", C.c_int),
         ("shared_inputs", C.c_int),
+        ("share_block0", C.c_int),
         ("gen_src", C.c_void_p), ("gen_chans", C.c_int), ("gen_pos", C.c_int),
         ("gen_coef", C.c_void_p), ("gen_noise", C.c_void_p),
     ]
@@ -294,6 +296,8 @@
     "sdy_sfno_workspace_floats": (C.c_size_t, [C.c_void_p, C.c_int]),
     "sdy_sfno_max_batch": (C.c_int, [C.c_void_p]),
     "sdy_sfno_forward": (C.c_int, [C.c_void_p, C.POINTER(SdySfnoFwdArgs), C.c_void_p]),
+    "sdy_sht_ones_roundtrip_host": (C.c_int, [C.c_int, C.c_int, C.c_int, C.c_int, C.c_int, C.c_int, C.POINTER(C.c_double),
+                                              C.POINTER(C.c_double)]),
     "sdy_sfno_time_embed": (C.c_int, [C.c_void_p, C.c_void_p, C.c_int, C.c_void_p, C.c_void_p, C.c_void_p]),
     "sdy_norm_pack": (C.c_int, [C.POINTER(SdyVarTable), C.c_int, C.c_int, C.c_int, C.c_int, C.c_void_p, C.c_void_p]),
     "sdy_step_finish": (C.c_int, [C.POINTER(SdyStepFinishArgs), C.c_void_p]),
diff --git a/spherical-dyffusion_amd/csrc/capi.hip b/spherical-dyffusion_amd/csrc/capi.hip
--- a/spherical-dyffusion_amd/csrc/capi.hip
+++ b/spherical-dyffusion_amd/csrc/capi.hip
@@ -598,6 +598,9 @@
   const float* enc_ws = nullptr;
   int enc_B = 0;
   bool enc_has_stats = false;
+  const float* b0_ws = nullptr;
+  int b0_B = 0;
+  double c00 = 0.0, p1_err = 1.0;
 };
 
 static int dev_alloc(DevBuf& b, size_t n) {
@@ -671,6 +674,10 @@
     r = sdy_sht_plan_create_ex(c->nlat, c->nlon, c->lmax, c->mmax, SDY_GRID_LEGENDRE_GAUSS, c->gemm_mode, &n->plan_lg);
     if (r != SDY_OK) { sdy_sfno_destroy(n); return r; }
   }
+  if (n->plan_lg != n->plan_data) {
+    r = sdy_sht_ones_roundtrip_host(c->nlat, c->nlon, c->lmax, c->mmax, c->data_grid, SDY_GRID_LEGENDRE_GAUSS, &n->c00, &n->p1_err);
+    if (r != SDY_OK) { sdy_sfno_destroy(n); return r; }
+  }
   std::memset(&n->tm, 0, sizeof(n->tm));
   n->tm.num_layers = c->num_layers;
   for (int i = 0; i < c->num_layers; ++i) {
@@ -721,6 +728,7 @@
   const std::string name(name_c);
   const bool h3 = c.gemm_mode == 1;
   n->enc_ws = nullptr;
+  n->b0_ws = nullptr;
   n->path.clear();
   if (name.find("trans") != std::string::npos && (name.find(".weights") != std::string::npos ||
                                                    name.find(".pct") != std::string::npos))
@@ -958,7 +966,7 @@
 
 namespace {
 struct WsLayout {
-  size_t cat, xa, xb, xe, xn, y, zt, hid, xf, cs, cs2, ca, cd, ca1, cd1, st0, st1, ste, ss, dp, trep, sp, total;
+  size_t cat, xa, xb, xe, xn, y, zt, hid, xf, cs, cs2, ca, cd, ca1, cd1, st0, st1, ste, ss, dp, trep, sp, cs0, r0, ta, td, total;
 };
 WsLayout ws_layout(const sdy_sfno* n, int B) {
   const sdy_sfno_config& c = n->cfg;
@@ -983,6 +991,8 @@
   w.dp = take((size_t)B * c.num_layers);
   w.trep = take((size_t)2 * B * (c.with_time_emb ? c.time_dim : 1));
   w.sp = take((size_t)B * E * c.nlat * 4);
+  w.cs0 = take(cs_floats(n->plan_data, B, (int)E)); w.r0 = take(img);
+  w.ta = take((size_t)B * E); w.td = take((size_t)B * E);
   w.total = off;
   return w;
 }
@@ -1026,13 +1036,13 @@
 enum SdyStage {
   ST_CONCAT, ST_TIME_MLP, ST_ENC0, ST_ENC2, ST_NORM_COEFFS, ST_FFT_FWD, ST_LEG_FWD, ST_LEG_INV, ST_FFT_INV, ST_DHCONV,
   ST_SKIP_CONV, ST_MLP_FUSED, ST_MLP_FUSED_DROP, ST_FC1, ST_FC2, ST_DEC0, ST_DEC2, ST_ENC_PAIR, ST_DEC_PAIR, ST_DROP_COPY,
-  ST_SKIP_GELU, ST_COUNT
+  ST_SKIP_GELU, ST_B0_AFFINE, ST_COUNT
 };
 const char* const kStageNames[ST_COUNT] = {
   "concat", "time_mlp", "encoder.0 conv", "encoder.2 conv", "instnorm coefficients", "rfft (lon)", "legendre analysis",
   "legendre synthesis", "irfft (lon)", "dhconv", "inner-skip conv", "mlp fused", "mlp fused (dropout)", "mlp fc1", "mlp fc2",
   "decoder.0 conv", "decoder.2 conv", "encoder (fused pair)", "decoder (fused pair)", "drop-path copy",
-  "inner skip folded (gelu)"};
+  "inner skip folded (gelu)", "block-0 time affine"};
 struct SdyProfiler {
   bool on = false;
   struct Rec { int stage; int rows; hipEvent_t e0, e1; bool closed; };
@@ -1123,6 +1133,8 @@
   const bool drop = a->enable_dropout != 0, reuse = a->reuse_encoder != 0, shared = a->shared_inputs != 0, gen = a->gen_src;
   const bool enc_once = shared && n->enc.w && n->path[0].scale_residual && n->path[0].in.tiled;
   const int Be = enc_once ? rpc : B;
+  bool b0share = false, b0skip = false;
+  const int Bs = shared ? rpc : B;
   const float pm = (drop && c.dropout_mlp > 0.f) ? c.dropout_mlp : 0.f;
   const WsLayout w = ws_layout(n, B);
   float* const ws = a->ws;
@@ -1169,11 +1181,19 @@
     if (ns == 0 || ctot != c.in_chans) return SDY_ERR_SHAPE;
     if (a->rows_per_call < 0 || (a->rows_per_call > 0 && B % a->rows_per_call)) return SDY_ERR_ARG;
     if (shared && (reuse || rpc >= B)) return SDY_ERR_ARG;
-    return SDY_OK;
+    b0share = b0_share_ok();
+    b0skip = b0share && reuse && n->b0_ws == ws && n->b0_B == B;
+    return SDY_OK;
+  }
+
+  bool b0_share_ok() const {
+    const BlockPath& P = n->path[0];
+    return a->share_block0 && !gen && c.with_time_emb && c.num_layers > 1 && n->enc.w && P.scale_residual && P.in.tiled &&
+           P.cs_tiled && P.dh == DH_FOLDED && P.fused_mlp && n->tm.dp_rate[0] == 0.f && n->p1_err <= 1e-6;
   }
 
   int inputs() {
-    if (!reuse) n->enc_ws = nullptr;
+    if (!reuse) n->enc_ws = n->b0_ws = nullptr;
     SDY_HIP_TRY(hipMemsetAsync(st1, 0, (size_t)B * E * 2 * sizeof(double), stream));
     SDY_HIP_TRY(hipMemsetAsync(st0, 0, (size_t)B * E * 2 * sizeof(double), stream));
     if (gen) {
@@ -1230,8 +1250,9 @@
       SDY_STAGE(ST_ENC2, sdy_conv1x1(&cv, stream));
     }
     n->enc_ws = enc_once ? nullptr : ws; n->enc_B = B; n->enc_has_stats = have_ste;
-    if (have_ste) {
-      for (int b0 = 0; b0 < B; b0 += Be)
+    if (have_ste && b0skip) {
+    } else if (have_ste) {
+      for (int b0 = 0; b0 < (b0share ? Bs : B); b0 += Be)
         SDY_HIP_TRY(hipMemcpyAsync(st0 + (size_t)b0 * E * 2, ste, (size_t)Be * E * 2 * sizeof(double), hipMemcpyDeviceToDevice,
                                    stream));
       cur_stats = st0;
@@ -1245,8 +1266,10 @@
     k.z = k.P.z_tiled ? zt : y;
     k.z_bs = k.P.z_tiled ? zt_bs : xbs;
     k.st_out = (k.P.fused_mlp && !last) ? st0 : nullptr;
-    SDY_TRY(norm0(k));
+    const bool b0 = i == 0 && b0share;
+    if (!b0) SDY_TRY(norm0(k));
     drop_rows(k);
+    if (b0) SDY_TRY(block0_shared(k));
     SDY_TRY(spectral(k));
     if (k.Bp > 0) {
       SDY_TRY(inner_skip(k));
@@ -1288,10 +1311,31 @@
     k.Bf = k.P.scale_residual ? B : k.Bp;
   }
 
+  int block0_shared(const Blk& k) {
+    const BlockPath& P = k.P;
+    const sdy_sht_plan *pin = P.in.plan, *pout = P.out.plan;
+    float *Cs0 = ws + w.cs0, *R0 = ws + w.r0;
+    if (!b0skip) {
+      if (!cur_stats) return SDY_ERR_STATE;
+      SDY_STAGE_N(ST_NORM_COEFFS, Bs, sdy_instnorm_from_stats(cur_stats, Bs, E, HW, k.w.n0w.p, k.w.n0b.p, nullptr, 0, 1e-6f, ca, cd,
+                                                              stream));
+      SDY_STAGE_N(ST_FFT_FWD, Bs, sdy_fft_launch_fwd(pin->fft, cur, ca, cd, nullptr, Xf, Bs, E, pin->nlat, pin->mtr, P.in.ilv,
+                                                     P.in.mcut, stream, nullptr, 0));
+      SDY_STAGE_N(ST_LEG_FWD, Bs, legendre_fwd_impl(pin, Xf, Cs0, Bs, E, P.in.polar, stream, P.in.tiled, P.cs_tiled));
+      SDY_STAGE_N(ST_LEG_INV, Bs, legendre_inv_impl(pout, Cs0, Xf, Bs, E, P.out.polar, stream, P.out.tiled, P.cs_tiled));
+      SDY_STAGE_N(ST_FFT_INV, Bs, sdy_fft_launch_inv(pout->fft, Xf, nullptr, R0, Bs, E, pout->nlat, pout->mtr, P.out.ilv,
+                                                     P.out.mcut, stream));
+      n->b0_ws = shared ? nullptr : ws; n->b0_B = B;
+    }
+    SDY_STAGE(ST_B0_AFFINE, sdy_cs_time_affine_launch(Cs0, Bs, Cs, B, c.lmax, pin->mtr, ss, (long)c.num_layers * 2 * E,
+                                                      (float)n->c00, ws + w.ta, ws + w.td, stream));
+    return SDY_OK;
+  }
+
   int spectral(const Blk& k) {
     const BlockPath& P = k.P;
     const sdy_sht_plan *pin = P.in.plan, *pout = P.out.plan;
-    if (k.Bf > 0) {
+    if (k.Bf > 0 && !(k.i == 0 && b0share)) {
       float* xn_out = (P.scale_residual || P.lazy_norm) ? nullptr : xn;
       SDY_STAGE_N(ST_FFT_FWD, k.Bf, sdy_fft_launch_fwd(pin->fft, cur, ca, cd, xn_out, Xf, k.Bf, E, pin->nlat, pin->mtr, P.in.ilv,
                                                        P.in.mcut, stream, k.rows, (k.i == 0 && enc_once) ? Be : 0));
@@ -1361,7 +1405,9 @@
       ma.x = k.z; ma.x_bstride = k.z_bs; ma.x_tiled = k.P.z_tiled ? 1 : 0; ma.pa = ca1; ma.pd = cd1;
       ma.w = bw.mlp; ma.w1_scale = bw.mlp_s1; ma.w2_scale = bw.mlp_s2; ma.b1 = bw.b1.p; ma.b2 = bw.b2.p;
       ma.out = k.dst; ma.out_bstride = k.dst_bs;
-      if (k.P.lazy_norm) { ma.add = cur; ma.add_bstride = xbs; ma.add_a = ca; ma.add_d = cd; }
+      if (k.i == 0 && b0share) {
+        ma.add = ws + w.r0; ma.add_bstride = xbs; ma.add_a = ws + w.ta; ma.add_d = ws + w.td; ma.add_src_rows = shared ? Bs : 0;
+      } else if (k.P.lazy_norm) { ma.add = cur; ma.add_bstride = xbs; ma.add_a = ca; ma.add_d = cd; }
       else { ma.add = xn; ma.add_bstride = xbs; ma.add_by_launch_row = k.rows ? 1 : 0; }
       ma.B = k.Bp; ma.out_rows = k.rows; ma.E = E; ma.hidden = Hd; ma.HW = HW;
       ma.drop_p = pm; ma.seed = a->seed; ma.call = a->call; ma.stream_fc1 = 2u * i; ma.stream_fc2 = 2u * i + 1u;
diff --git a/spherical-dyffusion_amd/csrc/mlp_h3.hip b/spherical-dyffusion_amd/csrc/mlp_h3.hip
--- a/spherical-dyffusion_amd/csrc/mlp_h3.hip
+++ b/spherical-dyffusion_amd/csrc/mlp_h3.hip
@@ -44,6 +44,7 @@
   unsigned long long* stamps;
   SdyImgMap omap;
   int add_local;
+  int add_mod;
 };
 
 __device__ __forceinline__ int px_swz(int px) { return (px & 15) ^ (((px >> 4) & 1) * 3); }
@@ -576,7 +577,7 @@
   fc2(NCH - 1, F_{});
   stamp(12);
   {
-    res_base = p.add ? p.add + (long)(p.add_local ? z : zo) * p.add_bs : p.x + (long)z * p.x_bs;
+    res_base = p.add ? p.add + (long)(p.add_local ? z : zo % p.add_mod) * p.add_bs : p.x + (long)z * p.x_bs;
   }
 
   {
@@ -784,6 +785,8 @@
   if (a->out_rows && !a->add) return SDY_ERR_ARG;
   if (a->add_by_launch_row && (!a->out_rows || a->add_a)) return SDY_ERR_ARG;
   p.add_local = a->add_by_launch_row ? 1 : 0;
+  if (a->add_src_rows < 0 || (a->add_src_rows > 0 && (!a->add || a->add_by_launch_row))) return SDY_ERR_ARG;
+  p.add_mod = a->add_src_rows > 0 ? a->add_src_rows : 0x7fffffff;
   SDY_TRY(sdy_img_map_fill(p.omap, a->out_rows, a->B));
   SDY_TRY(sdy_flags_ptr(&p.flags));
   SDY_TRY(sdy_headroom_ptr(SDY_RANGE_MLP, &p.head));
diff --git a/spherical-dyffusion_amd/csrc/pointwise.h b/spherical-dyffusion_amd/csrc/pointwise.h
--- a/spherical-dyffusion_amd/csrc/pointwise.h
+++ b/spherical-dyffusion_amd/csrc/pointwise.h
@@ -47,3 +47,5 @@
 int sdy_affine_copy_stats_launch(const float* x, long x_bs, const float* a, const float* d, float* out, long out_bs,
                                  double* stats, int C, int HW, const unsigned char* rows, int n_rows, hipStream_t stream,
                                  int src_row0 = -1);
+int sdy_cs_time_affine_launch(const float* Cs_in, int src_rows, float* Cs_out, int B, int L, int mtr, const float* ss,
+                              long ss_stride, float c00, float* add_a, float* add_d, hipStream_t stream);
diff --git a/spherical-dyffusion_amd/csrc/pointwise.hip b/spherical-dyffusion_amd/csrc/pointwise.hip
--- a/spherical-dyffusion_amd/csrc/pointwise.hip
+++ b/spherical-dyffusion_amd/csrc/pointwise.hip
@@ -209,6 +209,31 @@
   }
 }
 
+__global__ __launch_bounds__(256) void cs_time_affine_kernel(const float* __restrict__ in, int src_rows, float* __restrict__ out,
+                                                             int B, int L, const float* __restrict__ ss, long ss_stride, float c00,
+                                                             float* __restrict__ add_a, float* __restrict__ add_d) {
+  constexpr int C = 256;
+  const int piece = blockIdx.x, b = blockIdx.y, m = blockIdx.z;
+  const int bs = b % src_rows;
+  const float* ssb = ss + (long)b * ss_stride;
+  if (m == 0 && piece == 0) {
+    add_a[(long)b * C + threadIdx.x] = ssb[threadIdx.x] + 1.0f;
+    add_d[(long)b * C + threadIdx.x] = ssb[C + threadIdx.x];
+  }
+  const int q = threadIdx.x & 15, lr = threadIdx.x >> 4;
+  const int j = 4 * q;
+  const int c = 16 * (2 * piece + (j >> 5)) + (j & 15);
+  const bool re = ((j >> 4) & 1) == 0;
+  const f32x4 sc = *reinterpret_cast<const f32x4*>(ssb + c) + 1.0f;
+  const f32x4* src = reinterpret_cast<const f32x4*>(in + ((long)(m * src_rows + bs) * 8 + piece) * L * 64) + q;
+  f32x4* dst = reinterpret_cast<f32x4*>(out + ((long)(m * B + b) * 8 + piece) * L * 64) + q;
+  for (int l = m + lr; l < L; l += 16) {
+    f32x4 v = src[l * 16] * sc;
+    if (l == 0 && re) v += *reinterpret_cast<const f32x4*>(ssb + C + c) * c00;
+    dst[l * 16] = v;
+  }
+}
+
 struct ConcatArgs {
   const float* src[4];
   int chans[4];
@@ -954,6 +979,16 @@
   return SDY_OK;
 }
 
+int sdy_cs_time_affine_launch(const float* Cs_in, int src_rows, float* Cs_out, int B, int L, int mtr, const float* ss,
+                              long ss_stride, float c00, float* add_a, float* add_d, hipStream_t stream) {
+  if (!Cs_in || !Cs_out || !ss || !add_a || !add_d || B <= 0 || L <= 0 || mtr <= 0 || src_rows <= 0 || src_rows > B)
+    return SDY_ERR_ARG;
+  if (B > 65535 || mtr > 65535 || (ss_stride & 3) || ss_stride < 512) return SDY_ERR_ARG;
+  hipLaunchKernelGGL(cs_time_affine_kernel, dim3(8, B, mtr), dim3(256), 0, stream, Cs_in, src_rows, Cs_out, B, L, ss, ss_stride,
+                     c00, add_a, add_d);
+  return sdy_launch_status();
+}
+
 int sdy_instnorm_coeffs_launch(const float* x, int B, int C, int HW, const float* gamma, const float* beta,
                                const float* ss, long ss_stride, float eps, float* a, float* d, hipStream_t stream) {
   if (!x || !gamma || !beta || !a || !d || B <= 0 || C <= 0 || HW <= 0) return SDY_ERR_ARG;
diff --git a/spherical-dyffusion_amd/csrc/tables.cpp b/spherical-dyffusion_amd/csrc/tables.cpp
--- a/spherical-dyffusion_amd/csrc/tables.cpp
+++ b/spherical-dyffusion_amd/csrc/tables.cpp
@@ -124,6 +124,31 @@
   return SDY_OK;
 }
 
+extern "C" int sdy_sht_ones_roundtrip_host(int nlat, int nlon, int lmax, int mmax, int grid_in, int grid_out, double* c00,
+                                           double* p1_err) {
+  if (!c00 || !p1_err) return SDY_ERR_ARG;
+  (void)mmax;
+  std::vector<double> pin((size_t)lmax * nlat), pout((size_t)lmax * nlat), w(nlat);
+  int r = sdy_sht_tables_host(nlat, nlon, lmax, 1, grid_in, pin.data(), w.data(), nullptr);
+  if (r == SDY_OK) r = sdy_sht_tables_host(nlat, nlon, lmax, 1, grid_out, pout.data(), nullptr, nullptr);
+  if (r != SDY_OK) return r;
+  std::vector<double> c(lmax, 0.0);
+  for (int l = 0; l < lmax; ++l) {
+    double acc = 0.0;
+    for (int k = 0; k < nlat; ++k) acc += pin[(size_t)l * nlat + k] * w[k];
+    c[l] = 2.0 * M_PI * acc;
+  }
+  double err = 0.0;
+  for (int k = 0; k < nlat; ++k) {
+    double acc = 0.0;
+    for (int l = 0; l < lmax; ++l) acc += c[l] * pout[(size_t)l * nlat + k];
+    err = std::fmax(err, std::fabs(acc - 1.0));
+  }
+  *c00 = c[0];
+  *p1_err = err;
+  return SDY_OK;
+}
+
 int sdy_factor_radices(int n, int* radices, int* nstages) {
   int cnt = 0;
   const int cand[4] = {4, 2, 3, 5};
diff --git a/spherical-dyffusion_amd/dyffusion.py b/spherical-dyffusion_amd/dyffusion.py
--- a/spherical-dyffusion_amd/dyffusion.py
+++ b/spherical-dyffusion_amd/dyffusion.py
@@ -80,6 +80,7 @@
         import os
         self.reuse_interpolator_encoder = bool(reuse_interpolator_encoder) and os.environ.get("SDY_NO_ENCODER_REUSE") is None
         self.share_pair_inputs = os.environ.get("SDY_NO_SHARED_INPUTS") is None
+        self.share_pair_block0 = os.environ.get("SDY_NO_BLOCK0_SHARE") is None
         self.full_sampling_schedule = list(range(0, self.num_timesteps))
         self.sampling_schedule = sampling_schedule or self.full_sampling_schedule
         self.interpolator_window = getattr(interpolator, "window", 1)
@@ -208,11 +209,16 @@
 
     def q_sample_two(self, x0, x_end, t_first, t_second, is_artificial_step: bool = True, **kwargs):
         packed = []
+        if self._can_share_block0():
+            kwargs = dict(kwargs, share_block0=True)
         first = self.q_sample(x0=x0, x_end=x_end, t=t_first, is_artificial_step=is_artificial_step, _keep_packed=packed,
                               **dict(kwargs))
         second = self.q_sample(x0=x0, x_end=x_end, t=t_second, is_artificial_step=is_artificial_step,
                                _packed_inputs=packed[0], reuse_encoder=True, **dict(kwargs))
         return first, second
+
+    def _can_share_block0(self) -> bool:
+        return self.share_pair_block0 and bool(getattr(getattr(self.interpolator, "model", None), "supports_block0_share", False))
 
     def _can_stack_calls(self) -> bool:
         net = getattr(self.interpolator, "model", None)
@@ -240,6 +246,8 @@
             inputs = two(inputs)
         else:
             kwargs["shared_inputs"] = True
+            if self._can_share_block0():
+                kwargs["share_block0"] = True
         do_enable = bool(
             self.enable_interpolator_dropout in [True, "always"]
             or (self.enable_interpolator_dropout == "except_dynamical_steps" and is_artificial_step)
diff --git a/spherical-dyffusion_amd/sfno.py b/spherical-dyffusion_amd/sfno.py
--- a/spherical-dyffusion_amd/sfno.py
+++ b/spherical-dyffusion_amd/sfno.py
@@ -107,6 +107,7 @@
         self.mask_injector = None
         self.noise_injector = None
         self.supports_shared_inputs = True
+        self.supports_block0_share = True
 
         E, T, H, Cin, L = embed_dim, self.time_dim, self.mlp_hidden, self.in_chans, self.modes_lat
         P = lambda *s: nn.Parameter(torch.zeros(*s), requires_grad=False)
@@ -302,7 +303,7 @@
 
     def forward(self, inputs, time=None, condition=None, static_condition=None, return_time_emb: bool = False,
                 keep_masks=None, drop_path_keep=None, rows_per_call: Optional[int] = None, reuse_encoder: bool = False,
-                shared_inputs: bool = False, forward_condition=None, **kwargs):
+                shared_inputs: bool = False, forward_condition=None, share_block0: bool = False, **kwargs):
         if return_time_emb:
             raise NotImplementedError("return_time_emb is a training-path feature")
         if not inputs.is_cuda:
@@ -381,7 +382,8 @@
                 assert eps.shape == gen[0].shape, f"injected noise {tuple(eps.shape)} != {tuple(gen[0].shape)}"
             gen = (gen[0], gen[1], eps)
         self._native_call(h, dev, pieces, tt, out, self._call, self.batch_offset, rows_per_call, keep_masks, drop_path_keep,
-                          reuse_encoder=bool(reuse_encoder), shared_inputs=bool(shared_inputs), gen=gen)
+                          reuse_encoder=bool(reuse_encoder), shared_inputs=bool(shared_inputs), gen=gen,
+                          share_block0=bool(share_block0) and gen is None)
         self._call += n_calls
         return out
 
@@ -398,7 +400,7 @@
 
     def _native_call(self, h, dev, pieces, tt, out, call: int, batch_offset: int, rows_per_call: Optional[int] = None,
                      keep_masks=None, drop_path_keep=None, reuse_encoder: bool = False, shared_inputs: bool = False,
-                     gen=None) -> None:
+                     gen=None, share_block0: bool = False) -> None:
         B = out.shape[0]
         ws = self._workspace(h, dev, B)
         a = SdySfnoFwdArgs()
@@ -428,6 +430,7 @@
         a.ws, a.ws_floats = ptr(ws), ws.numel()
         a.reuse_encoder = int(reuse_encoder)
         a.shared_inputs = int(shared_inputs)
+        a.share_block0 = int(share_block0)
         if gen is not None:
             keep.append(gen)
             a.gen_src, a.gen_chans, a.gen_pos = ptr(gen[0]), gen[0].shape[1], 1
```

Measured after the change: 167.8 member-forecast-steps/s (median of 6 runs). About the same (+0.7%).
